# WGLab/NanoCaller

Hardware: AMD Instinct MI355X
Metric: candidate sites/sec (pileup+CNN) (higher is better)
Workload: dtype f32 (f16x3 split MFMA, f32 accumulate)

## Files before the change

### include/nanocaller_hip.h

```cpp
#ifndef NANOCALLER_HIP_H
#define NANOCALLER_HIP_H

#include <stddef.h>
#include <stdint.h>

#ifdef __cplusplus
extern "C" {
#endif

#define NC_ABI_VERSION 11

typedef struct nc_ctx nc_ctx;

enum nc_status {
    NC_OK = 0,
    NC_ERR_ARG = -1,
    NC_ERR_CAPACITY = -2,
    NC_ERR_NOMEM = -3,
    NC_ERR_HIP = -4,
    NC_ERR_STATE = -5,
    NC_ERR_SELFTEST = -6,
    NC_ERR_UNSUPPORTED = -7
};

// ... 19 lines not shown
int nc_d2h_async(nc_ctx *ctx, void *stream, void *host, const void *dev, size_t bytes);
int nc_last_kernel_ms(nc_ctx *ctx, int which, float *ms);
int nc_enable_timing(nc_ctx *ctx, int on);
int nc_timing_sums(nc_ctx *ctx, double *sum_ms, int64_t *count);

typedef struct {
    int32_t start;
    int32_t end;
    int64_t base_flag;
} nc_tile_entry;

typedef struct {
    int64_t codes_len;
    const uint8_t *codes;
    int32_t tile_size;
    int32_t tile_pos0;
    int32_t n_tiles;
    const int32_t *tile_off;
    const nc_tile_entry *tile_ent;
    int64_t n_entries;
} nc_readpack;

int nc_pack_plan(int32_t n_reads, const int32_t *start, const int32_t *end, const uint8_t *keep,
                 int32_t tile_size, int32_t pos_lo, int32_t pos_hi,
                 int64_t *codes_len, int32_t *tile_pos0, int32_t *n_tiles, int64_t *n_entries);
int nc_pack_fill(int32_t n_reads, const int32_t *start, const int32_t *end, const int64_t *off,
                 const uint8_t *codes_in, const uint8_t *strand, const uint8_t *keep,
                 int32_t tile_size, int32_t tile_pos0, int32_t n_tiles,
                 uint8_t *codes_out, int64_t codes_len, int32_t *tile_off, nc_tile_entry *tile_ent,
                 int64_t n_entries);

typedef struct nc_wire nc_wire;
typedef struct {
    int32_t n_reads;
    const int32_t *rd_start;
    const int32_t *rd_end;
    const int64_t *slot_off;
    int64_t codes_len;
    int64_t n_blocks;
    const uint32_t *blk_off;
    const int32_t *blk_read;
    const uint16_t *events;
    int64_t n_events;
    const uint32_t *blk_ev;
    const uint8_t *ev_bytes;
    int64_t n_ev_bytes;
} nc_wire_arrays;
int nc_wire_build(int32_t n_reads, const int32_t *start, const int32_t *end, const int64_t *off, const uint8_t *codes_in,
                  const uint8_t *keep, const uint8_t *ref_wire, int32_t ref_pos0, int64_t ref_len, nc_wire **out);
int nc_wire_view(const nc_wire *w, nc_wire_arrays *view);
int nc_wire_free(nc_wire *w);
int nc_wire_ref_unpack(nc_ctx *ctx, const uint8_t *d_ref_nib, int64_t ref_len, uint8_t *d_ref_wire);
int nc_wire_ins_unpack(nc_ctx *ctx, const uint8_t *d_packed, int64_t n_bases, const int32_t *d_other_idx, int32_t n_other, uint8_t *d_ins_bases);
int nc_wire_build_del(int32_t n_reads, const int32_t *start, const int32_t *end, const int64_t *off, const uint8_t *codes_in,
                      const uint8_t *keep, const uint8_t *ref_wire, int32_t ref_pos0, int64_t ref_len, const int32_t *ev_off,
                      const int32_t *ev_pos, const int32_t *ev_len, nc_wire **out);
int nc_wire_apply_deletions(nc_ctx *ctx, int32_t n_reads, const int32_t *d_rd_start, const int32_t *d_rd_end, const int64_t *d_slot_off,
                            const int32_t *d_ev_off, const int32_t *d_ev_pos, const int32_t *d_ev_len, uint8_t *d_codes);
int nc_wire_expand(nc_ctx *ctx, int32_t n_reads, const int32_t *d_rd_start, const int32_t *d_rd_end, const int64_t *d_slot_off,
                   const uint8_t *d_ref_wire, int32_t ref_pos0, int64_t ref_len, const uint32_t *d_blk_off,
                   const int32_t *d_blk_read, const uint16_t *d_events, int64_t n_blocks, uint8_t *d_codes, int64_t codes_len,
                   uint8_t *d_ref_code);
int nc_wire_build2(int32_t n_reads, const int32_t *start, const int32_t *end, const int64_t *off, const uint8_t *codes_in,
                   const uint8_t *keep, const uint8_t *ref_wire, int32_t ref_pos0, int64_t ref_len, const int32_t *ev_off,
                   const int32_t *ev_pos, const int32_t *ev_len, int32_t flags, nc_wire **out);
int nc_wire_expand2(nc_ctx *ctx, int32_t n_reads, const int32_t *d_rd_start, const int32_t *d_rd_end, const int64_t *d_slot_off,
                    const uint8_t *d_ref_wire, int32_t ref_pos0, int64_t ref_len, const uint32_t *d_blk_off,
                    const int32_t *d_blk_read, const uint8_t *d_ev_bytes, int64_t n_blocks, uint8_t *d_codes, int64_t codes_len,
                    uint8_t *d_ref_code, const uint32_t *d_blk_ev, const int32_t *d_ev_off, const int32_t *d_ev_pos,
                    const int32_t *d_ev_len);
int nc_wire_expand_del(nc_ctx *ctx, int32_t n_reads, const int32_t *d_rd_start, const int32_t *d_rd_end, const int64_t *d_slot_off,
                       const uint8_t *d_ref_wire, int32_t ref_pos0, int64_t ref_len, const uint32_t *d_blk_off,
                       const int32_t *d_blk_read, const uint16_t *d_events, int64_t n_blocks, uint8_t *d_codes, int64_t codes_len,
                       uint8_t *d_ref_code, const uint32_t *d_blk_ev, const int32_t *d_ev_off, const int32_t *d_ev_pos,
                       const int32_t *d_ev_len);

int nc_indel_events_pack(int32_t n_reads, const int32_t *rd_start, const int32_t *ev_off, const int32_t *ev_pos, const int32_t *ev_len,
                         uint16_t *d16, int8_t *l8, int32_t *read_ins_off, int64_t big_cap, int32_t *big_idx, int32_t *big_pos,
                         int32_t *big_len, int64_t *n_big);
int nc_indel_events_expand(nc_ctx *ctx, int32_t n_reads, const int32_t *d_rd_start, const int32_t *d_ev_off, const uint16_t *d_d16,
                           const int8_t *d_l8, int32_t n_big, const int32_t *d_big_idx, const int32_t *d_big_pos, const int32_t *d_big_len,
                           const int32_t *d_read_ins_off, int32_t *d_ev_pos, int32_t *d_ev_len, int32_t *d_ins_off);
int nc_indel_events_pack8(int32_t n_reads, const int32_t *rd_start, const int32_t *ev_off, const int32_t *ev_pos, const int32_t *ev_len,
                          uint8_t *b8, uint16_t *d16x, int64_t esc_cap, int32_t *read_esc_off, int32_t *read_ins_off, int64_t big_cap,
                          int32_t *big_idx, int32_t *big_pos, int32_t *big_len, int64_t *n_esc, int64_t *n_big);
int nc_indel_events_expand8(nc_ctx *ctx, int32_t n_reads, const int32_t *d_rd_start, const int32_t *d_ev_off, const uint8_t *d_b8,
                            const uint16_t *d_d16x, const int32_t *d_read_esc_off, int32_t n_big, const int32_t *d_big_idx,
                            const int32_t *d_big_pos, const int32_t *d_big_len, const int32_t *d_read_ins_off, int32_t *d_ev_pos,
                            int32_t *d_ev_len, int32_t *d_ins_off);

int nc_inflate_device(nc_ctx *ctx, int32_t n_blocks, const uint8_t *d_comp, const int64_t *d_coff, const int32_t *d_clen, uint8_t *d_out,
                      const int64_t *d_ooff, const int32_t *d_isize, int32_t *d_status, uint32_t *d_tok, int32_t *d_ntok);
int nc_inflate_device_phase(nc_ctx *ctx, int32_t phase, int32_t n_blocks, const uint8_t *d_comp, const int64_t *d_coff, const int32_t *d_clen,
                            uint8_t *d_out, const int64_t *d_ooff, const int32_t *d_isize, int32_t *d_status, uint32_t *d_tok, int32_t *d_ntok);
int nc_bgzf_crc_device(nc_ctx *ctx, int32_t n_blocks, const uint8_t *d_comp, const int64_t *d_coff, const int32_t *d_clen, const uint8_t *d_out,
                       const int64_t *d_ooff, const int32_t *d_isize, int32_t *d_status);

int nc_bam_retag_sizes(nc_ctx *ctx, const uint8_t *d_raw, int32_t n_rec, const int64_t *d_rec_off, const uint64_t *d_hash, const int32_t *d_ps,
                       int32_t n_tags, int32_t *d_new_size, int32_t *d_tag_idx, int64_t *d_out_off, int32_t *d_status);
int nc_bam_retag(nc_ctx *ctx, const uint8_t *d_raw, int32_t n_rec, const int64_t *d_rec_off, const uint8_t *d_hp, const int32_t *d_ps,
                 const int32_t *d_tag_idx, const int64_t *d_out_off, uint8_t *d_out);
int nc_bgzf_deflate_device(nc_ctx *ctx, int32_t n, const uint8_t *d_in, const int64_t *d_ioff, const int32_t *d_ilen, uint8_t *d_out,
                           const int64_t *d_ooff, int32_t *d_clen, uint32_t *d_crc, int32_t *d_status);
int nc_bgzf_crc32_device(nc_ctx *ctx, int32_t n, const uint8_t *d_in, const int64_t *d_ioff, const int32_t *d_ilen, uint32_t *d_crc);
int nc_bgzf_assemble_device(nc_ctx *ctx, int32_t n, const uint8_t *d_pay, const int64_t *d_poff, const int32_t *d_clen, const uint32_t *d_crc,
                            const int32_t *d_isize, int64_t *d_foff, uint8_t *d_file);

#define NC_BAM_META_COLS 12
int nc_bgzf_members(const uint8_t *data, int64_t n, int64_t cap, int64_t *coff, int32_t *clen, int32_t *isize, int64_t *n_members);
int nc_bgzf_scan(const uint8_t *data, int64_t n, int64_t start, int64_t cap, int64_t *coff, int32_t *clen, int32_t *isize, int64_t *n_members,
                 int64_t *next);
int nc_bam_walk(nc_ctx *ctx, const uint8_t *d_raw, int64_t raw_len, int32_t n_seeds, const int64_t *d_seed, const int32_t *d_seed_tid,
                const int64_t *d_first, int64_t *d_out, int32_t *d_status);
int nc_bam_meta(nc_ctx *ctx, const uint8_t *d_raw, int64_t n_rec, const int64_t *d_rec_off, int32_t *d_meta, int32_t *d_status);
int nc_bam_codes(nc_ctx *ctx, const uint8_t *d_raw, int32_t n_reads, const int64_t *d_rec, const int64_t *d_slot, const int32_t *d_cigd,
                 const int32_t *d_ncig, const int32_t *d_start, uint8_t *d_codes);
int nc_bam_name_groups(nc_ctx *ctx, const uint8_t *d_raw, int64_t raw_len, int64_t n_cand, const int64_t *d_rec_off, const uint64_t *d_hash,
                       int32_t *d_gid, int32_t *d_status);
int nc_bam_indel_reads(nc_ctx *ctx, const uint8_t *d_raw, int32_t n_reads, const int64_t *d_rec, const int32_t *d_cigd, const int32_t *d_ncig,
                       int32_t tail_cap, int32_t *d_counts, const int32_t *d_ev_off, const int32_t *d_ins_base, const int32_t *d_tail_off,
                       int32_t *d_ev_pos, int32_t *d_ev_len, int32_t *d_ins_off, uint8_t *d_ins_bases, uint8_t *d_tail_bases);

typedef struct {
    int32_t mincov;
    double min_allele_freq;
    double nbr_t0, nbr_t1;
    int32_t haploid;
} nc_scan_params;

int nc_snp_scan(nc_ctx *ctx, const nc_readpack *pack,
                const uint8_t *ref_code_dev, int32_t ref_pos0, int32_t ref_len,
                int32_t scan_lo, int32_t scan_hi, const nc_scan_params *params,
                int32_t n_chunks, const int32_t *chunk_start_host, const int32_t *chunk_end_host,
                int32_t *n_nbr, int32_t *n_cand, int32_t *n_sites);

int nc_snp_scan_begin(nc_ctx *ctx, const nc_readpack *pack,
                      const uint8_t *ref_code_dev, int32_t ref_pos0, int32_t ref_len,
                      int32_t scan_lo, int32_t scan_hi, const nc_scan_params *params,
                      int32_t n_chunks, const int32_t *chunk_start_host, const int32_t *chunk_end_host);
int nc_snp_scan_end(nc_ctx *ctx, int32_t *n_nbr, int32_t *n_cand, int32_t *n_sites);

int nc_snp_scan_fetch(nc_ctx *ctx, int32_t *nbr_pos, int32_t *site_pos, int32_t *site_chunk,
                      int32_t *site_n, int32_t *site_alt);

int nc_snp_scan_fetch_async(nc_ctx *ctx, void *copy_stream, int32_t *nbr_pos, int32_t *site_pos, int32_t *site_chunk,
                            int32_t *site_n, int32_t *site_alt);

int nc_snp_featurize(nc_ctx *ctx, const nc_readpack *pack,
                     const uint8_t *ref_code_dev, int32_t ref_pos0, int32_t ref_len,
                     int32_t seq_mode, int32_t maxcov, int32_t min_nbr_sites,
                     float *x_dev, int32_t *ref_code_out_dev, int32_t *fwd_dp_dev, int32_t *rev_dp_dev,
                     int32_t *site_depth_dev, uint8_t *valid_dev);

int nc_snp_set_mates(nc_ctx *ctx, int32_t n_mates, const int64_t *d_mate_key, const int32_t *d_mate_rec);

int nc_indel_set_mates(nc_ctx *ctx, int32_t n_mates, const int64_t *d_mate_key, const int32_t *d_mate_rec);

int nc_snp_scan_set_sites(nc_ctx *ctx, int32_t n_sites, const int32_t *d_pos, int32_t only);

int nc_snp_scan_set_nbr_sites(nc_ctx *ctx, int32_t n_sites, const int32_t *d_pos, int32_t only);

int nc_snp_scan_set_sampling(nc_ctx *ctx, uint32_t seed, const uint32_t *keep6_host);

typedef struct {
    int32_t c_m, c_x, c_h;
    int32_t haploid;
    int32_t n_bands;
    int32_t band[16];
} nc_refconf_params;

int nc_refconf_columns(nc_ctx *ctx, const nc_readpack *pack, const uint8_t *d_ref_code, int32_t tile_pos0, int64_t npos, uint32_t *d_words);

int nc_refconf_blocks(nc_ctx *ctx, const uint32_t *d_words, int32_t tile_pos0, int64_t npos, int32_t n_chunks, const int32_t *chunk_start_host,
                      const int32_t *chunk_end_host, int32_t n_cut, const int32_t *d_cut_start, const int32_t *d_cut_end,
                      const nc_refconf_params *params, int64_t *n_blocks);
int nc_refconf_fetch(nc_ctx *ctx, int32_t *d_or_host_out);

int nc_refconf_text(nc_ctx *ctx, int64_t n_blocks, const int32_t *d_blocks, const uint8_t *d_ref_code, int32_t tile_pos0, int64_t npos,
                    const char *chrom, const nc_refconf_params *params, int64_t *d_line_off, uint8_t *d_text, int64_t text_cap, int64_t *n_bytes);

int nc_snp_scale(nc_ctx *ctx, const int32_t *site_depth_dev, const uint8_t *valid_dev, double train_coverage,
                 int32_t mode, double *scale_dev, double *chunk_depth_host);
int nc_snp_chunk_depth_async(nc_ctx *ctx, void *copy_stream, double *chunk_depth_host_pinned);

int nc_load_weights(nc_ctx *ctx, int32_t model_kind, const float *blob_host, size_t n_floats);
int nc_set_cnn_precision(nc_ctx *ctx, int exact_fp32);
int nc_set_tensor_format(nc_ctx *ctx, int fmt);
int nc_snp_forward(nc_ctx *ctx, int32_t model_kind, int64_t n, const float *x_dev, const int32_t *ref_code_dev,
                   const double *scale_dev, int32_t scale_mode, float *probs_dev, float *gt_dev);

int nc_snp_forward_drain(nc_ctx *ctx, int32_t model_kind, int64_t n, const float *x_dev, const int32_t *ref_code_dev,
                         const double *scale_dev, int32_t scale_mode, float *probs_dev, float *gt_dev,
                         void *copy_stream, float *probs_host, float *gt_host);
int nc_cnn_x_limit(nc_ctx *ctx, int32_t model_kind, float *x_limit);
int nc_cnn_range_watch(nc_ctx *ctx, uint8_t *site_flags_dev);
int nc_snp_trunk_info(nc_ctx *ctx, int32_t *mfma_per_site, int32_t *kernel_id);
int nc_indel_forward(nc_ctx *ctx, int32_t model_kind, int64_t n, const float *x_dev, float *probs_dev);

int nc_indel_tensor(nc_ctx *ctx, int32_t n_sets, const uint8_t *rows_dev, const int64_t *row_off_dev,
                    const int32_t *n_rows_dev, const int32_t *n_cols_dev, const uint8_t *ref_rows_dev,
                    const int64_t *ref_off_dev, int32_t max_cols, float *x_dev, uint8_t *cns_dev);

typedef struct {
    int32_t n_reads;
    const int32_t *ev_off;
    const int32_t *ev_pos;
    const int32_t *ev_len;
    const uint8_t *read_hap;
} nc_indel_events;

typedef struct {
    int32_t mincov, win_size, small_win_size;
    double ins_t, del_t;
    int32_t haploid;
    int32_t impute;
} nc_indel_scan_params;

int nc_indel_scan(nc_ctx *ctx, const nc_readpack *pack, const nc_indel_events *events, const uint8_t *excl_dev,
                  int32_t start, int32_t end, const nc_indel_scan_params *params, int8_t *col_type_host);

int nc_indel_scan_batch(nc_ctx *ctx, const nc_readpack *pack, const nc_indel_events *events, const uint8_t *excl_dev,
                        int32_t n_chunks, const int32_t *starts, const int32_t *ends, const nc_indel_scan_params *params,
                        int8_t *col_type_host, const int64_t *col_off);

typedef struct nc_bam nc_bam;
typedef struct nc_decoded nc_decoded;
typedef struct {
    int32_t n_reads;
    const int32_t *start, *end, *flag;
    const int64_t *off;
    const uint8_t *codes;
    int64_t n_codes;
    const int32_t *ev_off;
    const int32_t *ev_pos, *ev_len;
    int64_t n_events;
    const uint8_t *hap;
    const int32_t *ps;
    const int64_t *seq_off;
    const uint8_t *seq;
    int64_t n_seq;
    const int32_t *name_off;
    const char *names;
    const int32_t *qstart;
} nc_decoded_arrays;

int nc_bam_open(const char *path, nc_bam **out);
int nc_bam_close(nc_bam *bam);
int nc_bam_n_refs(nc_bam *bam, int32_t *n_refs, int32_t *has_index);
int nc_bam_ref(nc_bam *bam, int32_t i, const char **name, int32_t *length);
const char *nc_bam_error(const nc_bam *bam);
int nc_bam_set_threads(nc_bam *bam, int32_t n);
int nc_bam_decode(nc_bam *bam, int32_t tid, int32_t beg1, int32_t end1, int32_t keep_seq, nc_decoded **out);
int nc_bam_decode_regions(const char *path, int32_t tid, int32_t beg1, int32_t end1, int32_t keep_seq, int32_t n_regions,
                          nc_decoded **out);
int nc_decoded_view(const nc_decoded *d, nc_decoded_arrays *view);
int nc_decoded_free(nc_decoded *d);
#define NC_FLAG_REFSKIP 0x10000
int nc_decoded_check(const nc_decoded *d, const uint8_t *keep, int64_t *n_refskip, int64_t *n_dup_overlap);
int nc_decoded_name_groups(const nc_decoded *d, const uint8_t *keep, int32_t *gid, int64_t *n_shared);

typedef struct nc_slices nc_slices;
typedef struct {
    int32_t n_anchor;
    const int32_t *anchor_off;
    const int32_t *read_idx;
    const int64_t *seq_off;
    const uint8_t *seq;
    int64_t n_slices;
} nc_slices_arrays;
int nc_indel_slices(const nc_decoded *d, int32_t n_anchor, const int32_t *anchor_pos, int32_t window_before, int32_t window_after,
                    const uint8_t *keep, nc_slices **out);
int nc_slices_view(const nc_slices *s, nc_slices_arrays *view);
int nc_slices_free(nc_slices *s);

typedef struct nc_pass2 nc_pass2;
typedef struct {
    int32_t n_kept;
    const int32_t *anchor_idx;
    const int32_t *first0;
    int32_t sets_per_anchor;
    int32_t n_sets;
    const int32_t *set_read0;
    int32_t n_alignments;
    const int32_t *read_off;
    const char *reads;
    const int32_t *ref_off;
    const char *refs;
    int32_t max_cols;
    const int32_t *al_dup;
} nc_pass2_arrays;
int nc_indel_pass2_sets(const nc_decoded *d, const uint8_t *keep, int32_t n_anchor, const int32_t *anchors, const char *contig,
                        int64_t chrom_len, int32_t ref_lo, int32_t ref_hi, int32_t window_after, int32_t mincov, int32_t maxcov,
                        int32_t haploid, const int32_t *imp_idx, const int32_t *imp_off, const int32_t *imp_reads, nc_pass2 **out);
int nc_pass2_view(const nc_pass2 *p, nc_pass2_arrays *view);
int nc_pass2_free(nc_pass2 *p);


typedef struct nc_indel_pack_h nc_indel_pack_h;
typedef struct {
    int32_t n_reads;
    const int32_t *ev_off;
    const int32_t *ev_pos, *ev_len;
    int64_t n_events;
    const int32_t *ins_off;
    const uint8_t *ins_bases;
    int64_t n_ins_bases;
// ... 199 lines not shown
```

### nanocaller_amd/_lib.py

```python
from __future__ import annotations

import ctypes as C
import os

import numpy as np

_HERE = os.path.dirname(os.path.abspath(__file__))
LIB_PATH = os.environ.get("NANOCALLER_HIP_LIB") or os.path.join(_HERE, "libnanocaller_hip.so")

NC_OK = 0
NC_ERR_ARG = -1
NC_ERR_CAPACITY = -2
NC_ERR_NOMEM = -3
NC_ERR_UNSUPPORTED = -7
FLAG_REFSKIP = 0x10000
ABI_VERSION = 11
MODEL_SNP, MODEL_SNP_HAP, MODEL_INDEL, MODEL_INDEL_HAP = 0, 1, 2, 3
SEQ_MODES = {"ont": 0, "short_ont": 1, "ul_ont": 2, "ul_ont_extreme": 3, "pacbio": 4}
CODE_ABSENT = 7
FLANK = 50000
SNP_TENSOR = 1025
STAR_SCORING = (25, 1, 20, -10)

EXPORTS = [
    "nc_abi_version", "nc_device_count", "nc_ctx_create", "nc_ctx_destroy", "nc_ctx_set_stream", "nc_ctx_sync",
    "nc_last_error", "nc_malloc", "nc_free", "nc_memcpy_h2d", "nc_memcpy_d2h", "nc_last_kernel_ms",
    "nc_enable_timing", "nc_pack_plan", "nc_pack_fill", "nc_snp_scan", "nc_snp_scan_begin", "nc_snp_scan_end", "nc_snp_scan_fetch", "nc_snp_featurize",
    "nc_snp_scale", "nc_load_weights", "nc_snp_forward", "nc_indel_forward", "nc_indel_tensor", "nc_indel_scan",
    "nc_bam_open", "nc_bam_close", "nc_bam_n_refs", "nc_bam_ref", "nc_bam_error", "nc_bam_decode", "nc_decoded_view",
    "nc_decoded_free", "nc_snp_vcf_format", "nc_set_cnn_precision", "nc_snp_scan_fetch_async", "nc_snp_forward_drain", "nc_argsort4", "nc_indel_slices", "nc_slices_view", "nc_slices_free",
    "nc_nw_cigar", "nc_allele_prediction", "nc_bgzf_compress", "nc_bam_set_threads", "nc_indel_scan_batch", "nc_timing_sums", "nc_snp_chunk_depth_async", "nc_bam_decode_regions", "nc_star_msa", "nc_star_msa_tensor", "nc_star_msa_tensor_dup", "nc_set_tensor_format", "nc_allele_prediction_batch", "nc_allele_prediction_device", "nc_bgzf_read_file", "nc_consensus_strings",
    "nc_wire_build", "nc_wire_build_del", "nc_wire_apply_deletions", "nc_wire_ref_unpack", "nc_wire_view", "nc_wire_free", "nc_wire_expand", "nc_wire_expand_del", "nc_snp_set_mates", "nc_indel_set_mates", "nc_snp_scan_set_sites", "nc_snp_scan_set_nbr_sites", "nc_snp_scan_set_sampling", "nc_decoded_name_groups", "nc_wire_ins_unpack", "nc_indel_events_pack8", "nc_indel_events_expand8", "nc_wire_build2", "nc_wire_expand2", "nc_d2h_async",
    "nc_indel_pass2_sets", "nc_pass2_view", "nc_pass2_free",
    "nc_decoded_check", "nc_indel_pack_build", "nc_indel_pack_view", "nc_indel_pack_free", "nc_indel_sites_plan", "nc_indel_sites_run",
    "nc_indel_sites_fetch", "nc_indel_sites_fetch_alt", "nc_indel_set_sites", "nc_indel_sites_fetch_src", "nc_indel_sites_stage_ms", "nc_indel_sites_band_stats", "nc_indel_sites_band", "nc_indel_events_pack", "nc_indel_events_expand", "nc_inflate_device", "nc_inflate_device_phase", "nc_bgzf_crc_device", "nc_bgzf_members", "nc_bgzf_scan", "nc_bam_walk", "nc_bam_meta", "nc_bam_codes", "nc_bam_indel_reads", "nc_bam_name_groups", "nc_indel_sites_scoring", "nc_indel_vcf_format", "nc_synth_indel_truth", "nc_synth_indel_reads", "nc_cnn_x_limit", "nc_cnn_range_watch", "nc_snp_trunk_info",
    "nc_snp_phase_gather", "nc_snp_phase_load", "nc_snp_phase_solve", "nc_haplotag_run", "nc_snp_phase_view", "nc_snp_phase_free",
    "nc_snp_phase_realign", "nc_snp_phase_solve_gt", "nc_snp_phase_genotypes",
    "nc_snp_phase_set_weights", "nc_snp_phase_weights_from_bam", "nc_snp_phase_weights",
    "nc_bam_retag_sizes", "nc_bam_retag", "nc_bgzf_deflate_device", "nc_bgzf_crc32_device", "nc_bgzf_assemble_device",
    "nc_fasta_decode",
    "nc_bamidx_candidates", "nc_bamidx_chain", "nc_bamidx_collect", "nc_bamidx_verify", "nc_bamidx_serial", "nc_bamidx_fields",
    "nc_train_create", "nc_train_free", "nc_train_set_weights", "nc_train_get_weights", "nc_train_forward", "nc_train_loss_grad", "nc_train_adam",
    "nc_train_info", "nc_train_stage_ms",
    "nc_indel_train_create", "nc_indel_train_free", "nc_indel_train_set_weights", "nc_indel_train_get_weights", "nc_indel_train_forward",
    "nc_indel_train_loss_grad", "nc_indel_train_adam", "nc_indel_train_info", "nc_indel_train_stage_ms",
    "nc_hap_train_create", "nc_hap_train_free", "nc_hap_train_set_weights", "nc_hap_train_get_weights", "nc_hap_train_forward",
    "nc_hap_train_loss_grad", "nc_hap_train_adam", "nc_hap_train_info", "nc_hap_train_stage_ms",
    "nc_hap_indel_train_create", "nc_hap_indel_train_free", "nc_hap_indel_train_set_weights", "nc_hap_indel_train_get_weights",
    "nc_hap_indel_train_forward", "nc_hap_indel_train_loss_grad", "nc_hap_indel_train_adam", "nc_hap_indel_train_info", "nc_hap_indel_train_stage_ms",
    "nc_refconf_columns", "nc_refconf_blocks", "nc_refconf_fetch", "nc_refconf_text",
]


class TileEntry(C.Structure):
    _fields_ = [("start", C.c_int32), ("end", C.c_int32), ("base_flag", C.c_int64)]


TILE_ENTRY_DTYPE = np.dtype([("start", "<i4"), ("end", "<i4"), ("base_flag", "<i8")])
assert TILE_ENTRY_DTYPE.itemsize == C.sizeof(TileEntry) == 16


class ReadPackC(C.Structure):
    _fields_ = [("codes_len", C.c_int64), ("codes", C.c_void_p), ("tile_size", C.c_int32), ("tile_pos0", C.c_int32),
                ("n_tiles", C.c_int32), ("tile_off", C.c_void_p), ("tile_ent", C.c_void_p), ("n_entries", C.c_int64)]


class ScanParamsC(C.Structure):
    _fields_ = [("mincov", C.c_int32), ("min_allele_freq", C.c_double), ("nbr_t0", C.c_double), ("nbr_t1", C.c_double),
                ("haploid", C.c_int32)]


class RefconfParamsC(C.Structure):
    _fields_ = [("c_m", C.c_int32), ("c_x", C.c_int32), ("c_h", C.c_int32), ("haploid", C.c_int32), ("n_bands", C.c_int32), ("band", C.c_int32 * 16)]


class IndelEventsC(C.Structure):
    _fields_ = [("n_reads", C.c_int32), ("ev_off", C.c_void_p), ("ev_pos", C.c_void_p), ("ev_len", C.c_void_p),
                ("read_hap", C.c_void_p)]


class IndelScanParamsC(C.Structure):
    _fields_ = [("mincov", C.c_int32), ("win_size", C.c_int32), ("small_win_size", C.c_int32), ("ins_t", C.c_double),
                ("del_t", C.c_double), ("haploid", C.c_int32), ("impute", C.c_int32)]


class DecodedArraysC(C.Structure):
    _fields_ = [("n_reads", C.c_int32), ("start", C.c_void_p), ("end", C.c_void_p), ("flag", C.c_void_p), ("off", C.c_void_p),
                ("codes", C.c_void_p), ("n_codes", C.c_int64), ("ev_off", C.c_void_p), ("ev_pos", C.c_void_p),
                ("ev_len", C.c_void_p), ("n_events", C.c_int64), ("hap", C.c_void_p), ("ps", C.c_void_p),
                ("seq_off", C.c_void_p), ("seq", C.c_void_p), ("n_seq", C.c_int64), ("name_off", C.c_void_p),
                ("names", C.c_void_p), ("qstart", C.c_void_p)]


class SlicesArraysC(C.Structure):
    _fields_ = [("n_anchor", C.c_int32), ("anchor_off", C.c_void_p), ("read_idx", C.c_void_p), ("seq_off", C.c_void_p),
                ("seq", C.c_void_p), ("n_slices", C.c_int64)]


class Pass2ArraysC(C.Structure):
    _fields_ = [("n_kept", C.c_int32), ("anchor_idx", C.c_void_p), ("first0", C.c_void_p), ("sets_per_anchor", C.c_int32),
                ("n_sets", C.c_int32), ("set_read0", C.c_void_p), ("n_alignments", C.c_int32), ("read_off", C.c_void_p),
                ("reads", C.c_void_p), ("ref_off", C.c_void_p), ("refs", C.c_void_p), ("max_cols", C.c_int32), ("al_dup", C.c_void_p)]


class IndelPackArraysC(C.Structure):
    _fields_ = [("n_reads", C.c_int32), ("ev_off", C.c_void_p), ("ev_pos", C.c_void_p), ("ev_len", C.c_void_p), ("n_events", C.c_int64),
                ("ins_off", C.c_void_p), ("ins_bases", C.c_void_p), ("n_ins_bases", C.c_int64), ("tail_off", C.c_void_p),
                ("tail_bases", C.c_void_p), ("n_tail_bases", C.c_int64), ("read_ps", C.c_void_p), ("read_hap", C.c_void_p),
                ("read_flag", C.c_void_p)]


class IndelReadsC(C.Structure):
    _fields_ = [("n_reads", C.c_int32), ("slot_off", C.c_void_p), ("rd_start", C.c_void_p), ("rd_end", C.c_void_p), ("ev_off", C.c_void_p),
                ("ev_pos", C.c_void_p), ("ev_len", C.c_void_p), ("ins_off", C.c_void_p), ("ins_bases", C.c_void_p), ("tail_off", C.c_void_p),
                ("tail_bases", C.c_void_p), ("read_ps", C.c_void_p), ("read_hap", C.c_void_p), ("read_flag", C.c_void_p)]


class WireArraysC(C.Structure):
    _fields_ = [("n_reads", C.c_int32), ("rd_start", C.c_void_p), ("rd_end", C.c_void_p), ("slot_off", C.c_void_p),
                ("codes_len", C.c_int64), ("n_blocks", C.c_int64), ("blk_off", C.c_void_p), ("blk_read", C.c_void_p), ("events", C.c_void_p),
                ("n_events", C.c_int64), ("blk_ev", C.c_void_p), ("ev_bytes", C.c_void_p), ("n_ev_bytes", C.c_int64)]


class PhaseArraysC(C.Structure):
    _fields_ = [("n_reads", C.c_int32), ("n_sites", C.c_int32), ("n_blocks", C.c_int32), ("n_groups", C.c_int32), ("n_entries", C.c_int64),
                ("entry_off", C.c_void_p), ("entry_site", C.c_void_p), ("entry_allele", C.c_void_p), ("read_side", C.c_void_p),
                ("site_block", C.c_void_p), ("site_h", C.c_void_p), ("site_phased", C.c_void_p), ("site_ps", C.c_void_p),
                ("block_first", C.c_void_p), ("block_last", C.c_void_p), ("block_ps", C.c_void_p), ("block_cost", C.c_void_p),
                ("group_hp", C.c_void_p), ("group_ps", C.c_void_p), ("ms", C.c_float * 4)]


_lib = None


class NanoCallerHipError(RuntimeError):

    def __init__(self, message, status=None):
        super().__init__(message)
        self.status = status


def lib():
    global _lib
    if _lib is None:
        if not os.path.exists(LIB_PATH):
            raise NanoCallerHipError(
                "%s not found: build it with `python -c 'import __graft_entry__ as g; g.build()'` "
                "(hipcc --offload-arch=gfx950). There is no CPU fallback." % LIB_PATH)
        try:
            import torch
        except ImportError:
            pass
        L = C.CDLL(LIB_PATH)
        vp, i32, i64, dbl = C.c_void_p, C.c_int32, C.c_int64, C.c_double
        L.nc_abi_version.restype = C.c_int
        if L.nc_abi_version() != ABI_VERSION:
            raise NanoCallerHipError("%s has ABI version %d, this binding needs %d: rebuild it" % (LIB_PATH, L.nc_abi_version(), ABI_VERSION))
        L.nc_device_count.argtypes = [C.POINTER(C.c_int)]
        L.nc_ctx_create.argtypes = [C.c_int, C.POINTER(vp)]
        L.nc_ctx_destroy.argtypes = [vp]
        L.nc_ctx_set_stream.argtypes = [vp, vp]
        L.nc_ctx_sync.argtypes = [vp]
        L.nc_last_error.argtypes = [vp]
        L.nc_last_error.restype = C.c_char_p
        L.nc_malloc.argtypes = [vp, C.c_size_t, C.POINTER(vp)]
        L.nc_free.argtypes = [vp, vp]
        L.nc_memcpy_h2d.argtypes = [vp, vp, vp, C.c_size_t]
        L.nc_memcpy_d2h.argtypes = [vp, vp, vp, C.c_size_t]
        L.nc_last_kernel_ms.argtypes = [vp, C.c_int, C.POINTER(C.c_float)]
        L.nc_timing_sums.argtypes = [vp, vp, vp]
        L.nc_enable_timing.argtypes = [vp, C.c_int]
        L.nc_set_cnn_precision.argtypes = [vp, C.c_int]
        L.nc_pack_plan.argtypes = [i32, vp, vp, vp, i32, i32, i32, C.POINTER(i64), C.POINTER(i32), C.POINTER(i32),
                                   C.POINTER(i64)]
        L.nc_pack_fill.argtypes = [i32, vp, vp, vp, vp, vp, vp, i32, i32, i32, vp, i64, vp, vp, i64]
        L.nc_snp_scan.argtypes = [vp, C.POINTER(ReadPackC), vp, i32, i32, i32, i32, C.POINTER(ScanParamsC), i32, vp, vp,
                                  C.POINTER(i32), C.POINTER(i32), C.POINTER(i32)]
        L.nc_snp_scan_begin.argtypes = [vp, C.POINTER(ReadPackC), vp, i32, i32, i32, i32, C.POINTER(ScanParamsC), i32, vp, vp]
        L.nc_snp_scan_end.argtypes = [vp, C.POINTER(i32), C.POINTER(i32), C.POINTER(i32)]
        L.nc_snp_scan_fetch.argtypes = [vp, vp, vp, vp, vp, vp]
        L.nc_snp_scan_fetch_async.argtypes = [vp, vp, vp, vp, vp, vp, vp]
        L.nc_snp_featurize.argtypes = [vp, C.POINTER(ReadPackC), vp, i32, i32, i32, i32, i32, vp, vp, vp, vp, vp, vp]
        L.nc_snp_scale.argtypes = [vp, vp, vp, dbl, i32, vp, vp]
        L.nc_snp_chunk_depth_async.argtypes = [vp, vp, vp]
        L.nc_load_weights.argtypes = [vp, i32, vp, C.c_size_t]
        L.nc_snp_forward.argtypes = [vp, i32, i64, vp, vp, vp, i32, vp, vp]
        L.nc_snp_forward_drain.argtypes = [vp, i32, i64, vp, vp, vp, i32, vp, vp, vp, vp, vp]
        L.nc_indel_forward.argtypes = [vp, i32, i64, vp, vp]
        L.nc_indel_tensor.argtypes = [vp, i32, vp, vp, vp, vp, vp, vp, i32, vp, vp]
        L.nc_indel_scan.argtypes = [vp, C.POINTER(ReadPackC), C.POINTER(IndelEventsC), vp, i32, i32, C.POINTER(IndelScanParamsC), vp]
        L.nc_indel_scan_batch.argtypes = [vp, C.POINTER(ReadPackC), C.POINTER(IndelEventsC), vp, i32, vp, vp, C.POINTER(IndelScanParamsC), vp, vp]
        L.nc_bam_open.argtypes = [C.c_char_p, C.POINTER(vp)]
        L.nc_bam_close.argtypes = [vp]
        L.nc_bam_set_threads.argtypes = [vp, i32]
        L.nc_bam_n_refs.argtypes = [vp, C.POINTER(i32), C.POINTER(i32)]
        L.nc_bam_ref.argtypes = [vp, i32, C.POINTER(C.c_char_p), C.POINTER(i32)]
        L.nc_bam_error.argtypes = [vp]
        L.nc_bam_error.restype = C.c_char_p
        L.nc_bam_decode.argtypes = [vp, i32, i32, i32, i32, C.POINTER(vp)]
        L.nc_star_msa_tensor.argtypes = [vp, i32, vp, vp, vp, vp, vp, i32, i32, i32, i32, i32, vp, vp, vp, vp, vp, vp, vp]
        L.nc_star_msa_tensor_dup.argtypes = L.nc_star_msa_tensor.argtypes + [vp]
        L.nc_consensus_strings.argtypes = [vp, i32, i32, vp, vp, vp]
        L.nc_allele_prediction_batch.argtypes = [i32, C.c_char_p, vp, C.c_char_p, vp, vp, vp, vp]
        L.nc_allele_prediction_device.argtypes = [vp, i32, C.c_char_p, vp, C.c_char_p, vp, vp, vp, vp]
        L.nc_set_tensor_format.argtypes = [vp, C.c_int]
        L.nc_star_msa.argtypes = [i32, C.c_char_p, vp, C.c_char_p, i32, i32, i32, i32, i32, i32, vp, vp, C.POINTER(i32)]
        L.nc_bam_decode_regions.argtypes = [C.c_char_p, i32, i32, i32, i32, i32, C.POINTER(vp)]
        L.nc_decoded_view.argtypes = [vp, C.POINTER(DecodedArraysC)]
        L.nc_decoded_free.argtypes = [vp]
        L.nc_indel_slices.argtypes = [vp, i32, vp, i32, i32, vp, C.POINTER(vp)]
        L.nc_slices_view.argtypes = [vp, C.POINTER(SlicesArraysC)]
        L.nc_slices_free.argtypes = [vp]
        L.nc_nw_cigar.argtypes = [C.c_char_p, i32, C.c_char_p, i32, i32, i32, i32, i32, vp, vp, i32, C.POINTER(i32)]
        L.nc_allele_prediction.argtypes = [C.c_char_p, i32, C.c_char_p, i32, i32, C.POINTER(i32), C.POINTER(i32)]
        L.nc_bgzf_compress.argtypes = [vp, i64, i32, vp, i64, C.POINTER(i64), vp, i64, C.POINTER(i64)]
        L.nc_indel_pass2_sets.argtypes = [vp, vp, i32, vp, C.c_char_p, i64, i32, i32, i32, i32, i32, i32, vp, vp, vp, C.POINTER(vp)]
        L.nc_pass2_view.argtypes = [vp, C.POINTER(Pass2ArraysC)]
        L.nc_pass2_free.argtypes = [vp]
        L.nc_d2h_async.argtypes = [vp, vp, vp, vp, C.c_size_t]
        L.nc_wire_build.argtypes = [i32, vp, vp, vp, vp, vp, vp, i32, i64, C.POINTER(vp)]
        L.nc_wire_build_del.argtypes = [i32, vp, vp, vp, vp, vp, vp, i32, i64, vp, vp, vp, C.POINTER(vp)]
        L.nc_wire_build2.argtypes = [i32, vp, vp, vp, vp, vp, vp, i32, i64, vp, vp, vp, i32, C.POINTER(vp)]
        L.nc_wire_apply_deletions.argtypes = [vp, i32, vp, vp, vp, vp, vp, vp, vp]
        L.nc_wire_ref_unpack.argtypes = [vp, vp, i64, vp]
        L.nc_wire_view.argtypes = [vp, C.POINTER(WireArraysC)]
        L.nc_wire_free.argtypes = [vp]
        L.nc_wire_expand.argtypes = [vp, i32, vp, vp, vp, vp, i32, i64, vp, vp, vp, i64, vp, i64, vp]
        L.nc_wire_expand_del.argtypes = L.nc_wire_expand.argtypes + [vp, vp, vp, vp]
        L.nc_wire_expand2.argtypes = L.nc_wire_expand.argtypes + [vp, vp, vp, vp]
        L.nc_snp_set_mates.argtypes = [vp, i32, vp, vp]
        L.nc_indel_set_mates.argtypes = [vp, i32, vp, vp]
        L.nc_snp_scan_set_sites.argtypes = [vp, i32, vp, i32]
        L.nc_snp_scan_set_nbr_sites.argtypes = [vp, i32, vp, i32]
        L.nc_snp_scan_set_sampling.argtypes = [vp, C.c_uint32, vp]
        L.nc_decoded_name_groups.argtypes = [vp, vp, vp, C.POINTER(i64)]
        L.nc_wire_ins_unpack.argtypes = [vp, vp, i64, vp, i32, vp]
        L.nc_indel_events_pack8.argtypes = [i32, vp, vp, vp, vp, vp, vp, i64, vp, vp, i64, vp, vp, vp, C.POINTER(i64), C.POINTER(i64)]
        L.nc_indel_events_expand8.argtypes = [vp, i32, vp, vp, vp, vp, vp, i32, vp, vp, vp, vp, vp, vp, vp]
        L.nc_decoded_check.argtypes = [vp, vp, C.POINTER(i64), C.POINTER(i64)]
        L.nc_indel_pack_build.argtypes = [vp, vp, i32, C.POINTER(vp)]
        L.nc_indel_pack_view.argtypes = [vp, C.POINTER(IndelPackArraysC)]
        L.nc_indel_pack_free.argtypes = [vp]
        L.nc_indel_sites_plan.argtypes = [vp, C.POINTER(ReadPackC), vp, i32, i32, i64, C.POINTER(IndelReadsC), vp, i32, vp, vp,
                                          C.POINTER(IndelScanParamsC), i32, i32, C.POINTER(i32), C.POINTER(i64)]
        L.nc_indel_sites_run.argtypes = [vp, vp]
        L.nc_indel_sites_scoring.argtypes = [vp, i32, i32, i32, i32]
        L.nc_indel_sites_fetch.argtypes = [vp, vp, vp, vp, vp, vp, vp, C.POINTER(i64)]
        L.nc_indel_sites_fetch_alt.argtypes = [vp, vp, i64]
        L.nc_indel_set_sites.argtypes = [vp, i32, vp, vp, i32]
        L.nc_indel_sites_fetch_src.argtypes = [vp, vp]
        L.nc_indel_sites_stage_ms.argtypes = [vp, vp, vp]
        L.nc_indel_sites_band_stats.argtypes = [vp, vp]
        L.nc_indel_sites_band.argtypes = [vp, i32, i32]
        L.nc_indel_events_pack.argtypes = [i32, vp, vp, vp, vp, vp, vp, vp, i64, vp, vp, vp, C.POINTER(i64)]
        L.nc_indel_events_expand.argtypes = [vp, i32, vp, vp, vp, vp, i32, vp, vp, vp, vp, vp, vp, vp]
        L.nc_inflate_device.argtypes = [vp, i32, vp, vp, vp, vp, vp, vp, vp, vp, vp]
        L.nc_inflate_device_phase.argtypes = [vp, i32, i32, vp, vp, vp, vp, vp, vp, vp, vp, vp]
        L.nc_bgzf_crc_device.argtypes = [vp, i32, vp, vp, vp, vp, vp, vp, vp]
        L.nc_bgzf_members.argtypes = [vp, i64, i64, vp, vp, vp, C.POINTER(i64)]
        L.nc_bgzf_scan.argtypes = [vp, i64, i64, i64, vp, vp, vp, C.POINTER(i64), C.POINTER(i64)]
        L.nc_bam_walk.argtypes = [vp, vp, i64, i32, vp, vp, vp, vp, vp]
        L.nc_bam_meta.argtypes = [vp, vp, i64, vp, vp, vp]
        L.nc_bam_codes.argtypes = [vp, vp, i32, vp, vp, vp, vp, vp, vp]
        L.nc_bam_indel_reads.argtypes = [vp, vp, i32, vp, vp, vp, i32, vp, vp, vp, vp, vp, vp, vp, vp, vp]
        L.nc_bam_name_groups.argtypes = [vp, vp, i64, i64, vp, vp, vp, vp]
        L.nc_indel_vcf_format.argtypes = [C.c_char_p, i64, vp, vp, i32, vp, i32, vp, vp, vp, vp, C.c_char_p, i64, i32, vp, i64, C.POINTER(i64), vp]
        L.nc_synth_indel_truth.argtypes = [vp, i64, C.c_uint64, dbl, dbl, dbl, dbl, i32, vp, vp, vp]
        L.nc_synth_indel_reads.argtypes = [vp, i64, C.c_uint64, dbl, dbl, dbl, dbl, i32, vp, vp, vp, vp, vp, vp, i32, vp, vp, vp, vp, vp, vp, vp, vp, vp]
        L.nc_cnn_x_limit.argtypes = [vp, i32, C.POINTER(C.c_float)]
        L.nc_snp_trunk_info.argtypes = [vp, C.POINTER(C.c_int32), C.POINTER(C.c_int32)]
        L.nc_cnn_range_watch.argtypes = [vp, vp]
        L.nc_argsort4.argtypes = [vp, i64, vp, C.POINTER(i64), vp, i64]
        L.nc_snp_phase_gather.argtypes = [vp, vp, i64, i32, vp, vp, vp, i32, vp, vp, C.POINTER(vp)]
        L.nc_snp_phase_load.argtypes = [vp, i32, i32, vp, vp, vp, vp, C.POINTER(vp)]
        L.nc_snp_phase_solve.argtypes = [vp, vp, i32]
        L.nc_snp_phase_solve_gt.argtypes = [vp, vp, i32, vp, i32]
        L.nc_snp_phase_genotypes.argtypes = [vp, C.POINTER(vp)]
        L.nc_snp_phase_set_weights.argtypes = [vp, vp, vp, vp]
        L.nc_snp_phase_weights_from_bam.argtypes = [vp, vp, vp, i64, vp, i32, i32, i32]
        L.nc_snp_phase_weights.argtypes = [vp, C.POINTER(vp), C.POINTER(vp), C.POINTER(vp)]
        L.nc_snp_phase_realign.argtypes = [vp, vp, i64, C.POINTER(IndelReadsC), i64, i64, vp, i32, i32, vp, vp, C.POINTER(vp)]
        L.nc_haplotag_run.argtypes = [vp, vp, i32, vp]
        L.nc_snp_phase_view.argtypes = [vp, C.POINTER(PhaseArraysC)]
        L.nc_snp_phase_free.argtypes = [vp]
        L.nc_bam_retag_sizes.argtypes = [vp, vp, i32, vp, vp, vp, i32, vp, vp, vp, vp]
        L.nc_bam_retag.argtypes = [vp, vp, i32, vp, vp, vp, vp, vp, vp]
        L.nc_bgzf_deflate_device.argtypes = [vp, i32, vp, vp, vp, vp, vp, vp, vp, vp]
        L.nc_bgzf_crc32_device.argtypes = [vp, i32, vp, vp, vp, vp]
        L.nc_bgzf_assemble_device.argtypes = [vp, i32, vp, vp, vp, vp, vp, vp, vp]
        L.nc_fasta_decode.argtypes = [vp, vp, i64, i64, i64, i64, i64, vp, vp, i64, i64, i64, i64, vp, vp]
        L.nc_bamidx_candidates.argtypes = [vp, vp, i64, i64, i32, vp, vp, vp]
        L.nc_bamidx_chain.argtypes = [vp, vp, i64, i64, vp, vp, i32, vp, vp, vp]
        L.nc_bamidx_collect.argtypes = [vp, i32, vp, vp, vp, vp]
        L.nc_bamidx_verify.argtypes = [vp, vp, i64, i64, i64, vp, i32, vp]
        L.nc_bamidx_serial.argtypes = [vp, vp, i64, i64, i32, vp, vp]
        L.nc_bamidx_fields.argtypes = [vp, vp, i64, vp, i64, vp, i32, i32, vp, vp, i32, i32, i32, i32, i32, vp, vp, vp]
        f32 = C.c_float
        for fam, snp in (("nc_train", True), ("nc_hap_train", True), ("nc_indel_train", False), ("nc_hap_indel_train", False)):
            site = [vp, i64, vp] + ([vp, vp] if snp else []) + [vp, f32]
            sig = dict(create=[vp, i32, i64] + ([] if snp else [i64]) + [C.POINTER(vp)], free=[vp], set_weights=[vp, vp, C.c_size_t],
                       get_weights=[vp, vp, C.c_size_t], forward=site + [vp] + ([vp] if fam == "nc_train" else []), loss_grad=site + [vp, f32, vp, vp],
                       adam=[vp, f32, f32, f32, f32], info=[vp, C.POINTER(i64), C.POINTER(i64), C.POINTER(i64)], stage_ms=[vp, i32, vp])
            for fn, argtypes in sig.items():
                getattr(L, "%s_%s" % (fam, fn)).argtypes = argtypes
        L.nc_refconf_columns.argtypes = [vp, C.POINTER(ReadPackC), vp, i32, i64, vp]
        L.nc_refconf_blocks.argtypes = [vp, vp, i32, i64, i32, vp, vp, i32, vp, vp, C.POINTER(RefconfParamsC), C.POINTER(i64)]
        L.nc_refconf_fetch.argtypes = [vp, vp]
        L.nc_refconf_text.argtypes = [vp, i64, vp, vp, i32, i64, C.c_char_p, C.POINTER(RefconfParamsC), vp, vp, i64, C.POINTER(i64)]
        L.nc_snp_vcf_format.argtypes = [C.c_char_p, i64, vp, vp, vp, vp, vp, vp, vp, vp, i32, vp, i64, C.POINTER(i64)]
        for name in EXPORTS:
            fn = getattr(L, name)
            if name not in ("nc_last_error", "nc_bam_error"):
                fn.restype = C.c_int
        _lib = L
    return _lib


def npp(a):
    if a is None:
        return None
    assert a.flags["C_CONTIGUOUS"]
    return a.ctypes.data_as(C.c_void_p)
```

### nanocaller_amd/csrc/nc_common.h

```cpp
#pragma once
#include <hip/hip_runtime.h>

#include <cstdarg>
#include <cstdint>
#include <cstdio>
#include <cstring>
#include <vector>

#include "../../include/nanocaller_hip.h"

__device__ __forceinline__ int32_t nc_wave_incl_scan(int32_t v)
{
    v += __builtin_amdgcn_update_dpp(0, v, 0x111, 0xf, 0xf, true);
    v += __builtin_amdgcn_update_dpp(0, v, 0x112, 0xf, 0xf, true);
    v += __builtin_amdgcn_update_dpp(0, v, 0x114, 0xf, 0xf, true);
    v += __builtin_amdgcn_update_dpp(0, v, 0x118, 0xf, 0xf, true);
    v += __builtin_amdgcn_update_dpp(0, v, 0x142, 0xa, 0xf, true);
    v += __builtin_amdgcn_update_dpp(0, v, 0x143, 0xc, 0xf, true);
    return v;
}

struct DevBuf {
    void *p = nullptr;
    size_t cap = 0;
    DevBuf() = default;
    DevBuf(const DevBuf &) = delete;
    DevBuf &operator=(const DevBuf &) = delete;
    ~DevBuf() { release(); }
    void release()
    {
        if (p) (void)hipFree(p);
        p = nullptr;
        cap = 0;
    }
};

struct nc_weights {
    float *dev = nullptr;
    size_t n = 0;
    float *packed = nullptr;
    void *packed_h = nullptr;
    float x_limit = 0.0f;
};

struct nc_ctx {
    int device = 0;
    hipStream_t own_stream = nullptr;
    hipStream_t stream = nullptr;
    char err[512] = {0};
    int timing = 0;
    bool x_i16 = false;
    bool cnn_exact_fp32 = false;
    bool k10_lds_set[2] = {false, false};
    bool huff_lds_set = false;
    bool deflate_lds_set = false;
    DevBuf deflate_tok;
    int32_t n_mates = 0;
    const int64_t *mate_key = nullptr;
    const int32_t *mate_rec = nullptr;
    int32_t n_imates = 0;
    const int64_t *imate_key = nullptr;
    const int32_t *imate_rec = nullptr;
    int32_t n_gsites = 0;
    const int32_t *gsite_pos = nullptr;
    bool gsites_only = false;
    DevBuf site_bits;
    int32_t n_nsites = 0;
    const int32_t *nsite_pos = nullptr;
    bool nsites_only = false;
    DevBuf nbr_bits;
    bool sample_on = false;
    uint32_t sample_seed = 0;
    uint32_t sample_keep[6] = {0, 0, 0, 0, 0, 0};
    int32_t n_isites = 0;
    const int32_t *isite_pos = nullptr;
    const uint8_t *isite_long = nullptr;
    bool isites_only = false;
    hipEvent_t ev0 = nullptr, ev1 = nullptr;
    float last_ms[6] = {0, 0, 0, 0, 0, 0};
    hipEvent_t kev[128] = {nullptr};
    int n_kev = 0;
    hipEvent_t tev[4][2] = {{nullptr, nullptr}, {nullptr, nullptr}, {nullptr, nullptr}, {nullptr, nullptr}};
    bool tev_pending[4] = {false, false, false, false};
    bool kev_pending = false;
    double sum_ms[6] = {0, 0, 0, 0, 0, 0};
    int64_t sum_n[6] = {0, 0, 0, 0, 0, 0};
    hipEvent_t drain_ev[4] = {nullptr};
    hipEvent_t scale_ev = nullptr;
    hipEvent_t scan_ev = nullptr;

    DevBuf stage_nbr, stage_cpos, stage_cn, stage_calt;
    DevBuf tile_cnt, tile_pre;
    DevBuf nbr_pos, cand_pos, cand_n, cand_alt;
    DevBuf chunk_start, chunk_end, chunk_lo, chunk_cnt, chunk_off;
    DevBuf site_pos, site_chunk, site_n, site_alt;
    DevBuf totals;
    DevBuf cnn_a, cnn_b, cnn_c;
    DevBuf chunk_depth;
    DevBuf nbr_idx;
    struct {
        size_t budget = 0;
        bool budget_shrunk = false;
        DevBuf ws;
        DevBuf ent_read;
        const void *ent_of = nullptr;
        int ent_spt = 0;
    } k7;
    DevBuf msa_reads, msa_read_off, msa_read_set, msa_refs, msa_ref_off;
    DevBuf msa_dup;
    DevBuf msa_rows_hf, msa_hcol, msa_tb, msa_trace, msa_cols, msa_out;
    int32_t n_nbr = 0, n_cand = 0, n_sites = 0, n_chunks = 0;
    bool have_scan = false;

    nc_weights w[4];
    struct nc_pipe_state *pipe = nullptr;
    struct nc_refconf_state *refconf = nullptr;
    uint8_t *range_sites = nullptr;

    int32_t *mbox = nullptr;
    bool scan_begun = false;
    int scan_tile = 0, scan_n_tiles = 0, scan_n_chunks = 0, scan_cap_nbr = 0, scan_cap_cand = 0;
    hipEvent_t scan_tot_ev = nullptr;
    uint8_t *stage_h = nullptr;
    int stage_turn = 0;
};

int nc_d2h(nc_ctx *ctx, void *host, const void *dev, size_t bytes, hipStream_t st);
int nc_h2d_small(nc_ctx *ctx, void *dev, const void *host, size_t bytes, hipStream_t st);
#define NC_D2H_KERNEL_MAX 65536
#define NC_STAGE_SLOT 16384
#define NC_STAGE_SLOTS 16

inline int nc_h2d_pieces(nc_ctx *ctx, void *dev, const void *host, size_t bytes, hipStream_t st)
{
    int in_flight = 0;
    for (size_t o = 0; o < bytes; o += NC_STAGE_SLOT) {
        if (++in_flight >= NC_STAGE_SLOTS - 2) {
            if (hipStreamSynchronize(st) != hipSuccess) return NC_ERR_HIP;
            in_flight = 1;
        }
        const size_t n = bytes - o < (size_t)NC_STAGE_SLOT ? bytes - o : (size_t)NC_STAGE_SLOT;
        const int rc = nc_h2d_small(ctx, (char *)dev + o, (const char *)host + o, n, st);
        if (rc != NC_OK) return rc;
    }
    return NC_OK;
}
inline int nc_d2h_pieces(nc_ctx *ctx, void *host_pinned, const void *dev, size_t bytes, hipStream_t st)
{
    for (size_t o = 0; o < bytes; o += NC_D2H_KERNEL_MAX) {
        const size_t n = bytes - o < (size_t)NC_D2H_KERNEL_MAX ? bytes - o : (size_t)NC_D2H_KERNEL_MAX;
        const int rc = nc_d2h(ctx, (char *)host_pinned + o, (const char *)dev + o, n, st);
        if (rc != NC_OK) return rc;
    }
    return NC_OK;
}

inline int nc_fail(nc_ctx *ctx, int code, const char *fmt, ...)
{
    if (ctx) {
        va_list ap;
        va_start(ap, fmt);
        vsnprintf(ctx->err, sizeof ctx->err, fmt, ap);
        va_end(ap);
    }
    return code;
}

#define NC_HIP(ctx, call)                                                                           \
    do {                                                                                            \
        hipError_t e_ = (call);                                                                     \
        if (e_ != hipSuccess)                                                                       \
            return nc_fail(ctx, NC_ERR_HIP, "%s failed: %s (%s:%d)", #call, hipGetErrorString(e_),  \
                           __FILE__, __LINE__);                                                     \
    } while (0)

inline int nc_ensure(nc_ctx *ctx, DevBuf &b, size_t bytes)
{
    if (bytes <= b.cap) return NC_OK;
    if (b.p) {
        NC_HIP(ctx, hipStreamSynchronize(ctx->stream));
        NC_HIP(ctx, hipFree(b.p));
        b.p = nullptr;
        b.cap = 0;
    }
    size_t want = bytes + bytes / 4 + 256;
    hipError_t e = hipMalloc(&b.p, want);
    if (e != hipSuccess) return nc_fail(ctx, NC_ERR_NOMEM, "hipMalloc(%zu) failed: %s", want, hipGetErrorString(e));
    b.cap = want;
    return NC_OK;
}

#define NC_TRY(x)                \
    do {                         \
        int rc_ = (x);           \
        if (rc_ != NC_OK) return rc_; \
    } while (0)

extern "C" __attribute__((visibility("hidden"))) void nc_timing_resolve(nc_ctx *ctx, int which);

struct NcTimer {
    nc_ctx *ctx;
    int which;
    NcTimer(nc_ctx *c, int w) : ctx(c), which(w)
    {
        if (ctx->timing == 1) {
            nc_timing_resolve(ctx, which);
            for (int e = 0; e < 2; e++)
                if (!ctx->tev[which][e]) (void)hipEventCreate(&ctx->tev[which][e]);
            (void)hipEventRecord(ctx->tev[which][0], ctx->stream);
        }
    }
    void stop()
    {
        if (ctx->timing == 1) {
            (void)hipEventRecord(ctx->tev[which][1], ctx->stream);
            ctx->tev_pending[which] = true;
        }
    }
};

int nc_selftest_device(nc_ctx *ctx);
void nc_pipe_destroy(nc_ctx *ctx);
void nc_refconf_destroy(nc_ctx *ctx);
```

### nanocaller_amd/csrc/nc_featurize.hip

```cpp
#include <type_traits>

#include "nc_common.h"

namespace {

constexpr int MAXCOV_CAP = 1024;
constexpr int MAXCOV_SMALL = 256;
constexpr int NBR = 20;

struct Bucket { int32_t dlo, dhi, k, far; };
struct ModeTab { int32_t nb, W; Bucket b[7]; };

constexpr ModeTab MODE_TABLES[5] = {
    {5, 50000, {{0, 2000, 2, 1}, {2000, 5000, 3, 0}, {5000, 10000, 4, 0}, {10000, 20000, 5, 0}, {20000, 1 << 30, 6, 0}, {0, 0, 0, 0}, {0, 0, 0, 0}}},
    {3, 50000, {{0, 2000, 5, 0}, {2000, 5000, 10, 0}, {5000, 1 << 30, 5, 0}, {0, 0, 0, 0}, {0, 0, 0, 0}, {0, 0, 0, 0}, {0, 0, 0, 0}}},
    {7, 100000, {{0, 2000, 2, 1}, {2000, 5000, 2, 0}, {5000, 10000, 3, 0}, {10000, 20000, 3, 0}, {20000, 40000, 4, 0}, {40000, 50000, 3, 0}, {50000, 1 << 30, 3, 0}}},
    {7, 300000, {{0, 10000, 2, 1}, {10000, 20000, 2, 0}, {20000, 50000, 3, 0}, {50000, 75000, 3, 0}, {75000, 100000, 4, 0}, {100000, 200000, 4, 0}, {200000, 1 << 30, 2, 0}}},
    {4, 20000, {{0, 2000, 4, 1}, {2000, 5000, 5, 0}, {5000, 10000, 5, 0}, {10000, 20000, 6, 0}, {0, 0, 0, 0}, {0, 0, 0, 0}, {0, 0, 0, 0}}},
};
__constant__ ModeTab MODES[5] = {MODE_TABLES[0], MODE_TABLES[1], MODE_TABLES[2], MODE_TABLES[3], MODE_TABLES[4]};

constexpr bool buckets_contiguous()
{
    for (int m = 0; m < 5; m++)
        for (int i = 0; i < MODE_TABLES[m].nb; i++)
            if (MODE_TABLES[m].b[i].dlo != (i ? MODE_TABLES[m].b[i - 1].dhi : 0) || MODE_TABLES[m].b[i].dhi <= MODE_TABLES[m].b[i].dlo) return false;
    return true;
}
static_assert(buckets_contiguous(), "a bucket must begin where the one before it ends (the first at 0): k_featurize_pairs shares the buckets' edges");

constexpr int NBR_IDX_SHIFT = 10;

__device__ __forceinline__ int lower_bound_i32(const int32_t *a, int n, int64_t key, const int32_t *cidx, int32_t cidx_pos0, int n_cidx)
{
    int lo = 0, hi = n;
    const int64_t rel = key - cidx_pos0;
    if (rel <= 0) hi = cidx[0];
    else {
        const int64_t b = rel >> NBR_IDX_SHIFT;
        if (b >= n_cidx - 1) lo = cidx[n_cidx - 1];
        else { lo = cidx[b]; hi = cidx[b + 1]; }
    }
    while (lo < hi) {
        const int mid = (lo + hi) >> 1;
        if ((int64_t)a[mid] < key) lo = mid + 1; else hi = mid;
    }
    return lo;
}

struct FeatArgs {
    const uint8_t *codes;
    const int32_t *tile_off;
    const nc_tile_entry *tile_ent;
    int32_t tile_pos0, tile_shift;
    const uint8_t *ref_code;
    int32_t ref_pos0;
    const int32_t *nbr_pos;
    int32_t n_nbr;
    const int32_t *cidx;
    int32_t cidx_pos0, n_cidx;
    const int32_t *site_pos, *site_chunk;
    const int32_t *chunk_start, *chunk_end;
    int32_t n_sites, mode, maxcov, min_nbr_sites;
    float *x;
    int32_t *ref_out, *fwd, *rev, *depth;
    uint8_t *valid;
    int32_t x_i16;
    const int64_t *mate_key;
    const int4 *mate_rec;
    int32_t n_mates;
};

__device__ __forceinline__ int named_member(const FeatArgs &a, int64_t key, int32_t p, int *self)
{
    int lo = 0, hi = a.n_mates;
    while (lo < hi) { const int mid = (lo + hi) >> 1; if (a.mate_key[mid] < key) lo = mid + 1; else hi = mid; }
    if (self) *self = lo;
    if (lo >= a.n_mates || a.mate_key[lo] != key) { if (self) *self = -2; return -1; }
    int best = -1, i = lo;
    for (int guard = 0; guard < 64; guard++) {
        const int4 r = a.mate_rec[i];
        if (r.x <= p && p < r.y && i > best) best = i;
        i = r.z;
        if (i == lo || i < 0 || i >= a.n_mates) break;
    }
    return best;
}
__device__ __forceinline__ int named_code(const FeatArgs &a, int64_t key, int32_t p)
{
    const int m = named_member(a, key, p, nullptr);
    if (m < 0) return 4;
    return a.codes[a.mate_key[m] - (a.mate_rec[m].x & ~15) + p];
}

template <int CAP, bool I16>
__global__ __launch_bounds__(256) void k_featurize(FeatArgs a)
{
    __shared__ __attribute__((aligned(16))) float sm[I16 ? 1 : 4][I16 ? 4 : NC_SNP_TENSOR + 3];
    __shared__ int32_t nlist[4][64];
    const int lane = threadIdx.x & 63, wv = __builtin_amdgcn_readfirstlane(threadIdx.x >> 6);
    const int nblk = (int)gridDim.x, q8 = nblk >> 3, r8 = nblk & 7, xcd = blockIdx.x & 7, within = blockIdx.x >> 3;
    const int blk = (xcd < r8 ? xcd * (q8 + 1) : r8 * (q8 + 1) + (xcd - r8) * q8) + within;
    const int s = blk * 4 + wv;
    float *X = sm[I16 ? 0 : wv];
    if constexpr (!I16)
        for (int i = lane; i < NC_SNP_TENSOR; i += 64) X[i] = 0.0f;

    if (s < a.n_sites) {
        const int32_t v = __builtin_amdgcn_readfirstlane(a.site_pos[s]);
        const int32_t ch = __builtin_amdgcn_readfirstlane(a.site_chunk[s]);
        const int64_t win_lo = max((int64_t)1, (int64_t)a.chunk_start[ch] - NC_FLANK);
        const int64_t win_hi = (int64_t)a.chunk_end[ch] + NC_FLANK;
        const ModeTab &M = MODES[a.mode];
        const int nb = M.nb;

        int take = 0, idx0 = 0;
        if (lane < 2 * nb) {
            const bool left = lane < nb;
            const Bucket B = M.b[left ? nb - 1 - lane : lane - nb];
            const int64_t dhi = min((int64_t)B.dhi, (int64_t)M.W - 1);
            int64_t pmin = left ? (int64_t)v - dhi : (int64_t)v + B.dlo + 1;
            int64_t pmax = left ? (int64_t)v - B.dlo - 1 : (int64_t)v + dhi;
            pmin = max(pmin, win_lo);
            pmax = min(pmax, win_hi);
            if (pmin <= pmax) {
                const int lo = lower_bound_i32(a.nbr_pos, a.n_nbr, pmin, a.cidx, a.cidx_pos0, a.n_cidx);
                const int hi = lower_bound_i32(a.nbr_pos, a.n_nbr, pmax + 1, a.cidx, a.cidx_pos0, a.n_cidx);
                const int m = hi - lo;
                take = min(m, B.k);
                const bool first = left ? (B.far != 0) : (B.far == 0);
                idx0 = first ? lo : hi - take;
            }
        }
        int incl = take;
#pragma unroll
        for (int o = 1; o < 16; o <<= 1) {
            const int y = __shfl_up(incl, o, 64);
            if (lane >= o) incl += y;
        }
        const int excl = incl - take;
        const int nl = __builtin_amdgcn_readlane(incl, nb - 1);
        const int ntot = __builtin_amdgcn_readlane(incl, 2 * nb - 1);
        const int nr = ntot - nl;
        const int ncols = ntot + 1;

        int32_t col = v;
        {
            for (int i = 0; i < take; i++) nlist[wv][excl + i] = idx0 + i;
            __builtin_amdgcn_fence(__ATOMIC_ACQ_REL, "wavefront");
            __builtin_amdgcn_wave_barrier();
            const int jj = lane < nl ? lane : lane - 1;
            if (lane != nl && lane < ncols) col = a.nbr_pos[nlist[wv][jj]];
        }
        const bool active = lane < ncols;
        const int rc_col = active ? a.ref_code[(int64_t)col - a.ref_pos0] : 4;
        const int rc_centre = a.ref_code[(int64_t)v - a.ref_pos0];

        const int t = (v - a.tile_pos0) >> a.tile_shift;
        const int e0 = __builtin_amdgcn_readfirstlane(a.tile_off[t]), e1 = __builtin_amdgcn_readfirstlane(a.tile_off[t + 1]);
        const bool ok = ncols >= a.min_nbr_sites;
        constexpr bool BYTE_CNT = CAP == MAXCOV_SMALL;
        using cnt_t = typename std::conditional<BYTE_CNT, uint32_t, unsigned long long>::type;
        constexpr int FIELD = BYTE_CNT ? 8 : 16;
        cnt_t cnt[4] = {0, 0, 0, 0};
        int n_all = 0;
        int fw[4] = {0, 0, 0, 0}, rv[4] = {0, 0, 0, 0};
        for (int eb = e0; eb < e1; eb += 64) {
            const int e = eb + lane;
            bool cov = false;
            int code = 4, strand = 0;
            int32_t estart = 0;
            uint32_t elen = 0, erow_lo = 0, erow_hi = 0;
            if (e < e1) {
                const nc_tile_entry ent = a.tile_ent[e];
                cov = ent.start <= v && v < ent.end;
                const uint64_t row = (uint64_t)(uintptr_t)a.codes + (uint64_t)((ent.base_flag & ~int64_t(15)) + ent.start);
                estart = ent.start;
                elen = (uint32_t)(ent.end - ent.start);
                erow_lo = (uint32_t)row;
                erow_hi = (uint32_t)(row >> 32);
                if (cov) {
                    code = a.codes[(ent.base_flag & ~int64_t(15)) + v];
                    strand = (int)(ent.base_flag & 1);
                }
            }
            unsigned long long m = __ballot(cov);
            unsigned long long mb[4];
#pragma unroll
            for (int b = 0; b < 4; b++) {
                mb[b] = __ballot(cov && code == b);
                const unsigned long long f = __ballot(cov && code == b && strand == 0);
                fw[b] += __popcll(f);
                rv[b] += __popcll(mb[b] & ~f);
            }
            const int room = a.maxcov - n_all;
            n_all += __popcll(m);
            if (!ok || room <= 0) continue;
            while (__popcll(m) > room) m &= ~(1ull << (63 - __builtin_clzll(m)));
#pragma unroll
            for (int k = 0; k < 4; k++) {
                unsigned long long mk = mb[k] & m;
                while (mk != 0ull) {
                    constexpr int RND = 16;
                    typedef const uint8_t __attribute__((address_space(1))) *gbyte_ptr;
                    int bcode[RND];
                    int nu = 0;
#pragma unroll
                    for (int u = 0; u < RND; u++) {
                        bcode[u] = 4;
                        if (mk != 0ull) {
                            const int idx = __builtin_ctzll(mk);
                            mk &= mk - 1ull;
                            nu = u + 1;
                            const int32_t rstart = __builtin_amdgcn_readlane(estart, idx);
                            const uint32_t rlen = (uint32_t)__builtin_amdgcn_readlane((int)elen, idx);
                            const gbyte_ptr rrow = (gbyte_ptr)(uintptr_t)(((uint64_t)(uint32_t)__builtin_amdgcn_readlane((int)erow_hi, idx) << 32) |
                                                                         (uint32_t)__builtin_amdgcn_readlane((int)erow_lo, idx));
                            const uint32_t off = (uint32_t)(col - rstart);
                            if (active && off < rlen) bcode[u] = rrow[off];
                        }
                    }
#pragma unroll
                    for (int u = 0; u < RND; u++) {
                        const cnt_t inc = BYTE_CNT ? (cnt_t)(uint32_t)(1ull << (8 * bcode[u]))
                                                   : (bcode[u] < 4 ? ((cnt_t)1 << (16 * bcode[u])) : (cnt_t)0);
                        if (u < nu) cnt[k] += inc;
                    }
                }
            }
        }
        const int ns = min(n_all, a.maxcov);
        if constexpr (I16) {
            const int o = NBR - nl;
            const int src = lane - o;
            const bool have = ok && lane < 41 && src >= 0 && src < ncols;
            const int sl = have ? src : lane;
            const int rc_s = __shfl(rc_col, sl, 64);
            cnt_t cs[4];
#pragma unroll
            for (int i = 0; i < 4; i++) {
                if constexpr (BYTE_CNT) cs[i] = (cnt_t)__shfl((int)cnt[i], sl, 64);
                else cs[i] = ((cnt_t)(uint32_t)__shfl((int)(cnt[i] >> 32), sl, 64) << 32) | (uint32_t)__shfl((int)(uint32_t)cnt[i], sl, 64);
            }
            if (lane < 41) {
                int16_t *dst = reinterpret_cast<int16_t *>(a.x) + (int64_t)s * NC_SNP_TENSOR + lane * 5;
                typedef uint32_t __attribute__((aligned(2))) u32_a2;
                auto put_row = [&](int row, int v0, int v1, int v2, int v3, int v4) {
                    int16_t *d = dst + row * (41 * 5);
                    *reinterpret_cast<u32_a2 *>(d) = (uint32_t)(v0 & 0xffff) | ((uint32_t)v1 << 16);
                    *reinterpret_cast<u32_a2 *>(d + 2) = (uint32_t)(v2 & 0xffff) | ((uint32_t)v3 << 16);
                    d[4] = (int16_t)v4;
                };
                const int rcs = have ? rc_s : 4;
                put_row(0, rcs == 0, rcs == 1, rcs == 2, rcs == 3, 0);
#pragma unroll
                for (int i = 0; i < 4; i++) {
                    int v[4];
#pragma unroll
                    for (int b = 0; b < 4; b++) {
                        const int val = have ? (int)((cs[i] >> (FIELD * b)) & ((1 << FIELD) - 1)) : 0;
                        v[b] = b == rcs ? -val : val;
                    }
                    put_row(1 + i, v[0], v[1], v[2], v[3], (have && i == rc_centre) ? 1 : 0);
                }
            }
        } else if (ok) {
            if (active) {
                const int o = NBR - nl;
                float *Xc = X + (o + lane) * 5;
                if (rc_col < 4) Xc[rc_col] = 1.0f;
#pragma unroll
                for (int i = 0; i < 4; i++) {
#pragma unroll
                    for (int b = 0; b < 4; b++) {
                        const int val = (int)((cnt[i] >> (FIELD * b)) & ((1 << FIELD) - 1));
                        Xc[(1 + i) * 41 * 5 + b] = (float)(b == rc_col ? -val : val);
                    }
                    Xc[(1 + i) * 41 * 5 + 4] = (i == rc_centre) ? 1.0f : 0.0f;
                }
            }
        }
        if (lane == 0) {
            a.ref_out[s] = rc_centre;
            a.depth[s] = ns;
            a.valid[s] = ok ? 1 : 0;
        }
        if (lane < 4) {
            a.fwd[s * 4 + lane] = fw[lane];
            a.rev[s * 4 + lane] = rv[lane];
        }
        (void)nr;
    }
    if constexpr (I16) return;
    __syncthreads();
    const int s0 = blk * 4;
    const int nsite = min(4, a.n_sites - s0);
    if (a.x_i16) {
        int16_t *d16 = reinterpret_cast<int16_t *>(a.x) + (int64_t)s0 * NC_SNP_TENSOR;
        const int total = nsite * NC_SNP_TENSOR;
        for (int i = threadIdx.x * 8; i < total; i += 256 * 8) {
            if (i + 8 <= total) {
                union { int16_t h[8]; uint4 u; } o;
#pragma unroll
                for (int q = 0; q < 8; q++) o.h[q] = (int16_t)sm[(i + q) / NC_SNP_TENSOR][(i + q) % NC_SNP_TENSOR];
                *reinterpret_cast<uint4 *>(d16 + i) = o.u;
            } else {
                for (int q = i; q < total; q++) d16[q] = (int16_t)sm[q / NC_SNP_TENSOR][q % NC_SNP_TENSOR];
            }
        }
        return;
    }
    float *dst = a.x + (int64_t)s0 * NC_SNP_TENSOR;
    if (nsite == 4) {
        float4 *d4 = reinterpret_cast<float4 *>(dst);
        for (int i = threadIdx.x; i < NC_SNP_TENSOR; i += 256) {
            const int f = i * 4;
            float4 o;
            o.x = sm[(f + 0) / NC_SNP_TENSOR][(f + 0) % NC_SNP_TENSOR];
            o.y = sm[(f + 1) / NC_SNP_TENSOR][(f + 1) % NC_SNP_TENSOR];
            o.z = sm[(f + 2) / NC_SNP_TENSOR][(f + 2) % NC_SNP_TENSOR];
            o.w = sm[(f + 3) / NC_SNP_TENSOR][(f + 3) % NC_SNP_TENSOR];
            d4[i] = o;
        }
    } else {
        for (int i = threadIdx.x; i < nsite * NC_SNP_TENSOR; i += 256) dst[i] = sm[i / NC_SNP_TENSOR][i % NC_SNP_TENSOR];
    }
}

template <bool MATES>
__global__ __launch_bounds__(256) void k_featurize_pairs(FeatArgs a)
{
    __shared__ int32_t nlist[4][64];
    union alignas(16) RecBuf { uint4 r[MAXCOV_SMALL]; int16_t h[MAXCOV_SMALL * 8]; uint32_t w[MAXCOV_SMALL * 4]; };
    static_assert((NC_SNP_TENSOR + 1) * 2 <= (int)sizeof(uint4) * MAXCOV_SMALL, "the tensor (one int16 further in for odd sites) must fit the read list");
    __shared__ RecBuf rec[4];
    __shared__ int32_t colL[4][64];
    __shared__ uint32_t cntL[4][41 * 4 + 4];
    __shared__ uint32_t endL[4][2 * 41];
    const int lane = threadIdx.x & 63, wv = __builtin_amdgcn_readfirstlane(threadIdx.x >> 6);
    const int nblk = (int)gridDim.x, q8 = nblk >> 3, r8 = nblk & 7, xcd = blockIdx.x & 7, within = blockIdx.x >> 3;
    const int blk = (xcd < r8 ? xcd * (q8 + 1) : r8 * (q8 + 1) + (xcd - r8) * q8) + within;
    const int s = blk * 4 + wv;
    if (s >= a.n_sites) return;
    const int32_t v = __builtin_amdgcn_readfirstlane(a.site_pos[s]);
    const int32_t ch = __builtin_amdgcn_readfirstlane(a.site_chunk[s]);
    const int64_t win_lo = max((int64_t)1, (int64_t)a.chunk_start[ch] - NC_FLANK);
    const int64_t win_hi = (int64_t)a.chunk_end[ch] + NC_FLANK;
    const ModeTab &M = MODES[a.mode];
    const int nb = M.nb;
    const int t = (v - a.tile_pos0) >> a.tile_shift;
    const int e0 = __builtin_amdgcn_readfirstlane(a.tile_off[t]), e1 = __builtin_amdgcn_readfirstlane(a.tile_off[t + 1]);
    nc_tile_entry pf_ent;
    pf_ent.start = 0; pf_ent.end = 0; pf_ent.base_flag = 0;
    int pf_code = 4;
    if (e0 + lane < e1) {
        pf_ent = a.tile_ent[e0 + lane];
        if (pf_ent.start <= v && v < pf_ent.end) pf_code = a.codes[(pf_ent.base_flag & ~int64_t(15)) + v];
    }
    const int rc_centre = a.ref_code[(int64_t)v - a.ref_pos0];
    int edge = 0;
    if (lane < 2 * nb + 2) {
        const bool left = lane <= nb;
        const int bi = left ? nb - 1 - lane : lane - nb - 2;
        const int64_t D = bi < 0 ? (int64_t)0 : min((int64_t)M.b[max(bi, 0)].dhi, (int64_t)M.W - 1);
        const int64_t key = min(max(left ? (int64_t)v - D : (int64_t)v + 1 + D, win_lo), win_hi + 1);
        edge = lower_bound_i32(a.nbr_pos, a.n_nbr, key, a.cidx, a.cidx_pos0, a.n_cidx);
    }
    int take = 0, idx0 = 0;
    {
        const bool left = lane < nb;
        const int lo = __shfl(edge, left ? lane : lane + 1, 64), hi = __shfl(edge, left ? lane + 1 : lane + 2, 64);
        if (lane < 2 * nb) {
            const Bucket B = M.b[left ? nb - 1 - lane : lane - nb];
            take = min(max(hi - lo, 0), B.k);
            const bool first = left ? (B.far != 0) : (B.far == 0);
            idx0 = first ? lo : hi - take;
        }
    }
    int incl = take;
#pragma unroll
    for (int o = 1; o < 16; o <<= 1) {
        const int y = __shfl_up(incl, o, 64);
        if (lane >= o) incl += y;
    }
    const int excl = incl - take;
    const int nl = __builtin_amdgcn_readlane(incl, nb - 1);
    const int ntot = __builtin_amdgcn_readlane(incl, 2 * nb - 1);
    const int ncols = ntot + 1;
    int32_t col = v;
    for (int i = 0; i < take; i++) nlist[wv][excl + i] = idx0 + i;
    for (int i = lane; i < 41 * 4; i += 64) cntL[wv][i] = 0;
    __builtin_amdgcn_fence(__ATOMIC_ACQ_REL, "wavefront");
    __builtin_amdgcn_wave_barrier();
    {
        const int jj = lane < nl ? lane : lane - 1;
        if (lane != nl && lane < ncols) col = a.nbr_pos[nlist[wv][jj]];
    }
    const bool active = lane < ncols;
    colL[wv][lane] = active ? col : INT32_MAX;
    const int rc_col = active ? a.ref_code[(int64_t)col - a.ref_pos0] : 4;
    const bool ok = ncols >= a.min_nbr_sites;
    int n_all = 0, nsel = 0;
    int fw[4] = {0, 0, 0, 0}, rv[4] = {0, 0, 0, 0};
    for (int eb = e0; eb < e1; eb += 64) {
        const int e = eb + lane;
        bool cov = false;
        int code = 4, strand = 0;
        uint4 rr = make_uint4(0, 0, 0, 0);
        if (e < e1) {
            nc_tile_entry ent = pf_ent;
            if (eb != e0) ent = a.tile_ent[e];
            cov = ent.start <= v && v < ent.end;
            const uint64_t row = (uint64_t)(uintptr_t)a.codes + (uint64_t)((ent.base_flag & ~int64_t(15)) + ent.start);
            rr = make_uint4((uint32_t)row, (uint32_t)(row >> 32), (uint32_t)ent.start, (uint32_t)(ent.end - ent.start));
            if constexpr (MATES) {
                if (cov && (ent.base_flag & 8)) {
                    int self;
                    const int m = named_member(a, (ent.base_flag & ~int64_t(15)) + (ent.start & ~15), v, &self);
                    if (self >= 0) { cov = m == self; rr.w |= 0x80000000u; }
                }
            }
            if (cov) {
                code = eb == e0 ? pf_code : (int)a.codes[(ent.base_flag & ~int64_t(15)) + v];
                strand = (int)(ent.base_flag & 1);
            }
        }
        unsigned long long m = __ballot(cov);
#pragma unroll
        for (int b = 0; b < 4; b++) {
            const unsigned long long mb = __ballot(cov && code == b), f = __ballot(cov && code == b && strand == 0);
            fw[b] += __popcll(f);
            rv[b] += __popcll(mb & ~f);
        }
        const int room = a.maxcov - n_all;
        n_all += __popcll(m);
        if (!ok || room <= 0) continue;
        while (__popcll(m) > room) m &= ~(1ull << (63 - __builtin_clzll(m)));
        const bool sel = ((m >> lane) & 1ull) && code < 4;
        const unsigned long long ms = __ballot(sel);
        if (sel) {
            rr.w |= (uint32_t)code << 28;
            rec[wv].r[nsel + __popcll(ms & ((1ull << lane) - 1ull))] = rr;
        }
        nsel += __popcll(ms);
    }
    __builtin_amdgcn_fence(__ATOMIC_ACQ_REL, "wavefront");
    __builtin_amdgcn_wave_barrier();
    {
        typedef const uint8_t __attribute__((address_space(1))) *gbyte_ptr;
        constexpr int U = 8;
        for (int g0 = 0; g0 < nsel; g0 += 64) {
            const int ng = min(64, nsel - g0);
            int len = 0, jlo = 0;
            if (lane < ng) {
                const uint4 rr = rec[wv].r[g0 + lane];
                int jhi = 0;
                const int32_t st = (int32_t)rr.z;
                const int64_t en = (int64_t)st + (int64_t)(rr.w & 0x0fffffffu);
#pragma unroll
                for (int w = 32; w > 0; w >>= 1) {
                    const int32_t cl = colL[wv][jlo + w - 1], ch2 = colL[wv][jhi + w - 1];
                    if (cl < st) jlo += w;
                    if ((int64_t)ch2 < en) jhi += w;
                }
                if (MATES && (rr.w >> 31)) { jlo = 0; jhi = ncols; }
                len = jhi - jlo;
            }
            int pin = len;
#pragma unroll
            for (int o = 1; o < 64; o <<= 1) {
                const int y = __shfl_up(pin, o, 64);
                if (lane >= o) pin += y;
            }
            const int Pc = __builtin_amdgcn_readlane(pin, 63);
            const int dj = jlo - (pin - len);
            if (lane < 41) endL[wv][2 * lane] = endL[wv][2 * lane + 1] = 0u;
            __builtin_amdgcn_fence(__ATOMIC_ACQ_REL, "wavefront");
            __builtin_amdgcn_wave_barrier();
            if (len > 0) atomicOr(&endL[wv][(pin - 1) >> 5], 1u << ((pin - 1) & 31));
            __builtin_amdgcn_fence(__ATOMIC_ACQ_REL, "wavefront");
            __builtin_amdgcn_wave_barrier();
            const int ew_lo = lane < 41 ? (int)endL[wv][2 * lane] : 0, ew_hi = lane < 41 ? (int)endL[wv][2 * lane + 1] : 0;
            int base = 0;
            for (int q0 = 0; q0 < Pc; q0 += 64 * U) {
                int jk[U];
                uint32_t bc[U];
#pragma unroll
                for (int u = 0; u < U; u++) {
                    bc[u] = 4;
                    jk[u] = 0;
                    const int qs = q0 + u * 64;
                    if (qs < Pc) {
                        const uint32_t wlo = (uint32_t)__builtin_amdgcn_readlane(ew_lo, qs >> 6), whi = (uint32_t)__builtin_amdgcn_readlane(ew_hi, qs >> 6);
                        const int q = qs + lane;
                        const bool valid = q < Pc;
                        const int r = valid ? base + (int)__builtin_amdgcn_mbcnt_hi(whi, __builtin_amdgcn_mbcnt_lo(wlo, 0u)) : 0;
                        base += __builtin_popcount(wlo) + __builtin_popcount(whi);
                        const uint4 rr = rec[wv].r[g0 + r];
                        const int djr = __shfl(dj, r, 64);
                        const int j = valid ? q + djr : 0;
                        const int32_t cj = colL[wv][j];
                        const uint32_t off = (uint32_t)(cj - (int32_t)rr.z);
                        jk[u] = j * 4 + (int)((rr.w >> 28) & 7u);
                        if (MATES && valid && (rr.w >> 31)) {
                            const int64_t key = (int64_t)((((uint64_t)rr.y << 32) | rr.x) - (uint64_t)(uintptr_t)a.codes) - (int64_t)(int32_t)rr.z + ((int32_t)rr.z & ~15);
                            bc[u] = (uint32_t)named_code(a, key, cj);
                        } else if (valid && j == nl) bc[u] = (rr.w >> 28) & 7u;
                        else if (valid && off < (rr.w & 0x0fffffffu)) bc[u] = ((gbyte_ptr)(uintptr_t)(((uint64_t)rr.y << 32) | rr.x))[off];
                    }
                }
#pragma unroll
                for (int u = 0; u < U; u++)
                    if (bc[u] < 4) atomicAdd(&cntL[wv][jk[u]], 1u << (8 * bc[u]));
            }
        }
    }
    __builtin_amdgcn_fence(__ATOMIC_ACQ_REL, "wavefront");
    __builtin_amdgcn_wave_barrier();
    const int ns = min(n_all, a.maxcov);
    {
        const int o = NBR - nl;
        const int src = lane - o;
        const bool have = ok && lane < 41 && src >= 0 && src < ncols;
        const int sl = have ? src : 0;
        const int rc_s = __shfl(rc_col, have ? src : lane, 64);
        const int odd = s & 1;
        int16_t *T = rec[wv].h + odd;
        if (lane < 41) {
            auto put_row = [&](int row, int v0, int v1, int v2, int v3, int v4) {
                int16_t *d = T + row * (41 * 5) + lane * 5;
                d[0] = (int16_t)v0; d[1] = (int16_t)v1; d[2] = (int16_t)v2; d[3] = (int16_t)v3; d[4] = (int16_t)v4;
            };
            const int rcs = have ? rc_s : 4;
            put_row(0, rcs == 0, rcs == 1, rcs == 2, rcs == 3, 0);
#pragma unroll
            for (int i = 0; i < 4; i++) {
                const uint32_t cs = have ? cntL[wv][sl * 4 + i] : 0u;
                int vv[4];
#pragma unroll
                for (int b = 0; b < 4; b++) {
                    const int val = (int)((cs >> (8 * b)) & 0xffu);
                    vv[b] = b == rcs ? -val : val;
                }
                put_row(1 + i, vv[0], vv[1], vv[2], vv[3], (have && i == rc_centre) ? 1 : 0);
            }
        }
        __builtin_amdgcn_fence(__ATOMIC_ACQ_REL, "wavefront");
        __builtin_amdgcn_wave_barrier();
        int16_t *dst = reinterpret_cast<int16_t *>(a.x) + (int64_t)s * NC_SNP_TENSOR;
        uint32_t *d32 = reinterpret_cast<uint32_t *>(dst + odd);
        const uint32_t *t32 = rec[wv].w + odd;
#pragma unroll
        for (int i = 0; i < (NC_SNP_TENSOR - 1) / 2; i += 64) d32[i + lane] = t32[i + lane];
        if (lane == 0) dst[odd ? 0 : NC_SNP_TENSOR - 1] = T[odd ? 0 : NC_SNP_TENSOR - 1];
    }
    if (lane == 0) {
        a.ref_out[s] = rc_centre;
        a.depth[s] = ns;
        a.valid[s] = ok ? 1 : 0;
    }
    if (lane < 4) {
        a.fwd[s * 4 + lane] = fw[lane];
        a.rev[s * 4 + lane] = rv[lane];
    }
}

__global__ void k_nbr_index(const int32_t *__restrict__ nbr_pos, int n_nbr, int32_t pos0, int n_cidx, int32_t *__restrict__ cidx)
{
    const int b = blockIdx.x * blockDim.x + threadIdx.x;
    if (b >= n_cidx) return;
    const int64_t key = (int64_t)pos0 + ((int64_t)b << NBR_IDX_SHIFT);
    int lo = 0, hi = n_nbr;
    while (lo < hi) {
        const int mid = (lo + hi) >> 1;
        if ((int64_t)nbr_pos[mid] < key) lo = mid + 1; else hi = mid;
    }
    cidx[b] = lo;
}

__global__ __launch_bounds__(256) void k_chunk_scale(const int32_t *__restrict__ chunk_off, const int32_t *__restrict__ depth,
                                                     const uint8_t *__restrict__ valid, const int32_t *__restrict__ site_n,
                                                     double train_cov, int mode, double *__restrict__ scale,
                                                     double *__restrict__ chunk_depth)
{
    const int c = blockIdx.x;
    const int s0 = chunk_off[c], s1 = chunk_off[c + 1];
    long long sum = 0, cntv = 0;
    for (int s = s0 + threadIdx.x; s < s1; s += 256)
        if (valid[s]) { sum += depth[s]; cntv++; }
    __shared__ long long ssum[256], scnt[256];
    ssum[threadIdx.x] = sum;
    scnt[threadIdx.x] = cntv;
    __syncthreads();
    for (int o = 128; o > 0; o >>= 1) {
        if (threadIdx.x < o) { ssum[threadIdx.x] += ssum[threadIdx.x + o]; scnt[threadIdx.x] += scnt[threadIdx.x + o]; }
        __syncthreads();
    }
    const double mean = scnt[0] ? (double)ssum[0] / (double)scnt[0] : 0.0;
    if (threadIdx.x == 0) chunk_depth[c] = mean;
    for (int s = s0 + threadIdx.x; s < s1; s += 256)
        scale[s] = mode == 0 ? train_cov / mean : train_cov / (double)site_n[s];
}

}

extern "C" {

int nc_snp_featurize(nc_ctx *ctx, const nc_readpack *pack, const uint8_t *ref_code_dev, int32_t ref_pos0, int32_t ref_len,
                     int32_t seq_mode, int32_t maxcov, int32_t min_nbr_sites, float *x_dev, int32_t *ref_code_out_dev,
                     int32_t *fwd_dp_dev, int32_t *rev_dp_dev, int32_t *site_depth_dev, uint8_t *valid_dev)
{
    if (!ctx) return NC_ERR_ARG;
    if (!ctx->have_scan) return nc_fail(ctx, NC_ERR_STATE, "nc_snp_featurize: call nc_snp_scan first");
    if (!pack || !ref_code_dev || seq_mode < 0 || seq_mode > 4)
        return nc_fail(ctx, NC_ERR_ARG, "nc_snp_featurize: bad argument");
    if (maxcov < 1 || maxcov > MAXCOV_CAP)
        return nc_fail(ctx, NC_ERR_ARG, "nc_snp_featurize: maxcov %d outside [1,%d]", maxcov, MAXCOV_CAP);
    if (ctx->n_sites == 0) return NC_OK;
    if (!x_dev || !ref_code_out_dev || !fwd_dp_dev || !rev_dp_dev || !site_depth_dev || !valid_dev)
        return nc_fail(ctx, NC_ERR_ARG, "nc_snp_featurize: null output");
    if (((uintptr_t)x_dev) & 15) return nc_fail(ctx, NC_ERR_ARG, "nc_snp_featurize: x_dev must be 16-byte aligned");
    if (ref_pos0 != pack->tile_pos0 || (int64_t)ref_len < (int64_t)pack->n_tiles * pack->tile_size)
        return nc_fail(ctx, NC_ERR_ARG, "nc_snp_featurize: ref_code must cover the pack's tile grid");
    NC_HIP(ctx, hipSetDevice(ctx->device));
    FeatArgs a;
    a.codes = pack->codes;
    a.tile_off = pack->tile_off;
    a.tile_ent = pack->tile_ent;
    a.tile_pos0 = pack->tile_pos0;
    a.tile_shift = pack->tile_size == 1024 ? 10 : pack->tile_size == 2048 ? 11 : 12;
    a.ref_code = ref_code_dev;
    a.ref_pos0 = ref_pos0;
    a.nbr_pos = (const int32_t *)ctx->nbr_pos.p;
    a.n_nbr = ctx->n_nbr;
    const int n_cidx = (int)(((int64_t)pack->n_tiles * pack->tile_size) >> NBR_IDX_SHIFT) + 2;
    NC_TRY(nc_ensure(ctx, ctx->nbr_idx, (size_t)n_cidx * 4));
    a.cidx = (const int32_t *)ctx->nbr_idx.p;
    a.cidx_pos0 = pack->tile_pos0;
    a.n_cidx = n_cidx;
    a.site_pos = (const int32_t *)ctx->site_pos.p;
    a.site_chunk = (const int32_t *)ctx->site_chunk.p;
    a.chunk_start = (const int32_t *)ctx->chunk_start.p;
    a.chunk_end = (const int32_t *)ctx->chunk_end.p;
    a.n_sites = ctx->n_sites;
    a.mode = seq_mode;
    a.maxcov = maxcov;
    a.min_nbr_sites = min_nbr_sites;
    a.x = x_dev;
    a.ref_out = ref_code_out_dev;
    a.fwd = fwd_dp_dev;
    a.rev = rev_dp_dev;
    a.depth = site_depth_dev;
    a.valid = valid_dev;
    a.x_i16 = ctx->x_i16 ? 1 : 0;
    a.mate_key = (const int64_t *)ctx->mate_key;
    a.mate_rec = (const int4 *)ctx->mate_rec;
    a.n_mates = ctx->n_mates;
    const char *fp = getenv("NC_FEAT_PAIRS");
    const bool pairs = maxcov < MAXCOV_SMALL && a.x_i16 && !(fp && atoi(fp) == 0);
    if (a.n_mates > 0 && !pairs)
        return nc_fail(ctx, NC_ERR_UNSUPPORTED, "nc_snp_featurize: alignments that share read names (nc_snp_set_mates) need the int16 tensor format and maxcov < %d", MAXCOV_SMALL);
    NcTimer tm(ctx, 1);
    hipLaunchKernelGGL(k_nbr_index, dim3((n_cidx + 255) / 256), dim3(256), 0, ctx->stream, a.nbr_pos, a.n_nbr, a.cidx_pos0, n_cidx,
                       (int32_t *)ctx->nbr_idx.p);
    const dim3 grid((ctx->n_sites + 3) / 4);
    if (maxcov < MAXCOV_SMALL) {
        if (pairs && a.n_mates > 0) hipLaunchKernelGGL(k_featurize_pairs<true>, grid, dim3(256), 0, ctx->stream, a);
        else if (pairs) hipLaunchKernelGGL(k_featurize_pairs<false>, grid, dim3(256), 0, ctx->stream, a);
        else if (a.x_i16) hipLaunchKernelGGL((k_featurize<MAXCOV_SMALL, true>), grid, dim3(256), 0, ctx->stream, a);
        else hipLaunchKernelGGL((k_featurize<MAXCOV_SMALL, false>), grid, dim3(256), 0, ctx->stream, a);
    } else {
        if (a.x_i16) hipLaunchKernelGGL((k_featurize<MAXCOV_CAP, true>), grid, dim3(256), 0, ctx->stream, a);
        else hipLaunchKernelGGL((k_featurize<MAXCOV_CAP, false>), grid, dim3(256), 0, ctx->stream, a);
    }
    NC_HIP(ctx, hipGetLastError());
    tm.stop();
    return NC_OK;
}

int nc_snp_set_mates(nc_ctx *ctx, int32_t n_mates, const int64_t *d_mate_key, const int32_t *d_mate_rec)
{
    if (!ctx) return NC_ERR_ARG;
    if (n_mates < 0 || (n_mates > 0 && (!d_mate_key || !d_mate_rec || ((uintptr_t)d_mate_rec & 15))))
        return nc_fail(ctx, NC_ERR_ARG, "nc_snp_set_mates: bad argument");
    ctx->n_mates = n_mates;
    ctx->mate_key = n_mates ? d_mate_key : nullptr;
    ctx->mate_rec = n_mates ? d_mate_rec : nullptr;
    return NC_OK;
}

int nc_snp_scale(nc_ctx *ctx, const int32_t *site_depth_dev, const uint8_t *valid_dev, double train_coverage, int32_t mode,
                 double *scale_dev, double *chunk_depth_host)
{
    if (!ctx) return NC_ERR_ARG;
    if (!ctx->have_scan) return nc_fail(ctx, NC_ERR_STATE, "nc_snp_scale: call nc_snp_scan first");
    if (mode != 0 && mode != 1) return nc_fail(ctx, NC_ERR_ARG, "nc_snp_scale: mode must be 0 or 1");
    NC_TRY(nc_ensure(ctx, ctx->chunk_depth, (size_t)ctx->n_chunks * 8));
    if (ctx->n_sites > 0) {
        if (!site_depth_dev || !valid_dev || !scale_dev) return nc_fail(ctx, NC_ERR_ARG, "nc_snp_scale: null argument");
        hipLaunchKernelGGL(k_chunk_scale, dim3(ctx->n_chunks), dim3(256), 0, ctx->stream, (const int32_t *)ctx->chunk_off.p,
                           site_depth_dev, valid_dev, (const int32_t *)ctx->site_n.p, train_coverage, mode, scale_dev,
                           (double *)ctx->chunk_depth.p);
        NC_HIP(ctx, hipGetLastError());
    } else {
        NC_HIP(ctx, hipMemsetAsync(ctx->chunk_depth.p, 0, (size_t)ctx->n_chunks * 8, ctx->stream));
    }
    if (chunk_depth_host) {
        NC_HIP(ctx, hipMemcpyAsync(chunk_depth_host, ctx->chunk_depth.p, (size_t)ctx->n_chunks * 8, hipMemcpyDeviceToHost,
                                   ctx->stream));
        NC_HIP(ctx, hipStreamSynchronize(ctx->stream));
    }
    return NC_OK;
}

int nc_snp_chunk_depth_async(nc_ctx *ctx, void *copy_stream, double *chunk_depth_host_pinned)
{
    if (!ctx) return NC_ERR_ARG;
    if (!copy_stream || !chunk_depth_host_pinned) return nc_fail(ctx, NC_ERR_ARG, "nc_snp_chunk_depth_async: null argument");
    if (!ctx->have_scan || !ctx->chunk_depth.p) return nc_fail(ctx, NC_ERR_STATE, "nc_snp_chunk_depth_async: call nc_snp_scale first");
    if (!ctx->scale_ev) NC_HIP(ctx, hipEventCreateWithFlags(&ctx->scale_ev, hipEventDisableTiming));
    NC_HIP(ctx, hipEventRecord(ctx->scale_ev, ctx->stream));
    NC_HIP(ctx, hipStreamWaitEvent((hipStream_t)copy_stream, ctx->scale_ev, 0));
    NC_TRY(nc_d2h(ctx, chunk_depth_host_pinned, ctx->chunk_depth.p, (size_t)ctx->n_chunks * 8, (hipStream_t)copy_stream));
    return NC_OK;
}

}
```

### nanocaller_amd/csrc/nc_scan.hip

```cpp
#include <algorithm>

#include "nc_common.h"

namespace {

__device__ __forceinline__ uint32_t lut8(uint32_t x, uint32_t lo, uint32_t hi) { return __builtin_amdgcn_perm(hi, lo, x); }

constexpr uint32_t LUT_LO[5] = {0x00000001u, 0x00000100u, 0x00010000u, 0x01000000u, 0x01010101u};
constexpr uint32_t LUT_HI[5] = {0u, 0u, 0u, 0u, 0x00000001u};

struct ScanP {
    int32_t mincov;
    int32_t haploid;
    double min_af, t0, t1;
    int32_t scan_lo, scan_hi;
};

struct ScanX {
    int32_t sample;
    uint32_t seed;
    uint32_t keep[6];
};

__device__ __forceinline__ uint32_t mix32(int32_t p, uint32_t seed)
// ... 111 lines not shown
    __syncthreads();
    uint32_t wpre = 0, total = 0;
#pragma unroll
    for (int i = 0; i < BLOCK / 64; i++) {
        const uint32_t s = wsum[i];
        if (i < wv) wpre += s;
        total += s;
    }
    const uint32_t excl = wpre + incl - mine;
    int on = excl & 0xFFFF, oc = excl >> 16;
    const int64_t sbase = (int64_t)t * TILE;
#pragma unroll
    for (int i = 0; i < 16; i++) {
        if (nbr_mask & (1u << i)) stage_nbr[sbase + on++] = P0 + i;
        if (cand_mask & (1u << i)) {
            const int d = i >> 2, k = i & 3;
            const int wi = 2 * d + (k & 1), sh = (k >> 1) * 16;
            const int r = (rw[d] >> (8 * k)) & 0xFF;
            uint32_t alt = 0;
#pragma unroll
            for (int b = 0; b < 4; b++) {
                const uint32_t cb = (wide[b][wi] >> sh) & 0xFFFF;
                if (b != r && cb > alt) alt = cb;
            }
            stage_cpos[sbase + oc] = P0 + i;
            stage_cn[sbase + oc] = (int32_t)((wide[4][wi] >> sh) & 0xFFFF);
            stage_calt[sbase + oc] = (int32_t)alt;
            oc++;
        }
    }
    if (threadIdx.x == 0) tile_cnt[t] = make_int2((int)(total & 0xFFFF), (int)(total >> 16));
}

__global__ __launch_bounds__(256) void k_site_bits(int32_t n, const int32_t *__restrict__ pos, int32_t tile_pos0, int64_t npos,
                                                   uint32_t *__restrict__ bits)
{
    const int64_t i = (int64_t)blockIdx.x * 256 + threadIdx.x;
    if (i >= n) return;
    const int64_t g = (int64_t)pos[i] - tile_pos0;
    if (g < 0 || g >= npos) return;
    atomicOr(&bits[g >> 5], 1u << (g & 31));
}

__global__ __launch_bounds__(1024) void k_tile_prefix(const int2 *__restrict__ cnt, int2 *__restrict__ pre, int n,
                                                      int32_t *__restrict__ totals)
{
    __shared__ int2 wsum[16];
    const int lane = threadIdx.x & 63, wv = threadIdx.x >> 6;
    const int per = ((n + 15) / 16 + 63) & ~63;
    const int b0 = min(n, wv * per), b1 = min(n, b0 + per);
    int2 sum = make_int2(0, 0);
#pragma unroll 4
    for (int i = b0 + lane; i < b1; i += 64) {
        const int2 v = cnt[i];
        sum.x += v.x; sum.y += v.y;
    }
    const int2 winc = make_int2(nc_wave_incl_scan(sum.x), nc_wave_incl_scan(sum.y));
    if (lane == 63) wsum[wv] = winc;
    __syncthreads();
    int cx = 0, cy = 0, tx = 0, ty = 0;
    for (int w = 0; w < 16; w++) {
        const int2 t = wsum[w];
        if (w < wv) { cx += t.x; cy += t.y; }
        tx += t.x; ty += t.y;
    }
#pragma unroll 4
    for (int base = b0; base < b1; base += 64) {
        const int i = base + lane;
        const int2 v = i < b1 ? cnt[i] : make_int2(0, 0);
        const int ix = nc_wave_incl_scan(v.x), iy = nc_wave_incl_scan(v.y);
        if (i < b1) pre[i] = make_int2(cx + ix - v.x, cy + iy - v.y);
        cx += __builtin_amdgcn_readlane(ix, 63);
        cy += __builtin_amdgcn_readlane(iy, 63);
    }
    if (threadIdx.x == 0) { totals[0] = tx; totals[1] = ty; }
}

__global__ __launch_bounds__(256) void k_compact(int tile, const int2 *__restrict__ cnt, const int2 *__restrict__ pre,
                                                 const int32_t *__restrict__ stage_nbr, const int32_t *__restrict__ stage_cpos,
                                                 const int32_t *__restrict__ stage_cn, const int32_t *__restrict__ stage_calt,
                                                 int32_t *__restrict__ nbr_pos, int32_t *__restrict__ cand_pos,
                                                 int32_t *__restrict__ cand_n, int32_t *__restrict__ cand_alt, int cap_nbr, int cap_cand)
{
    const int t = blockIdx.x;
    const int2 c = cnt[t], p = pre[t];
    const int64_t sb = (int64_t)t * tile;
    for (int i = threadIdx.x; i < c.x; i += 256)
        if (p.x + i < cap_nbr) nbr_pos[p.x + i] = stage_nbr[sb + i];
    for (int i = threadIdx.x; i < c.y; i += 256) {
        if (p.y + i >= cap_cand) continue;
        cand_pos[p.y + i] = stage_cpos[sb + i];
        cand_n[p.y + i] = stage_cn[sb + i];
        cand_alt[p.y + i] = stage_calt[sb + i];
    }
}

__device__ __forceinline__ int lower_bound_dev(const int32_t *a, int n, int32_t key)
{
    int lo = 0, hi = n;
    while (lo < hi) {
        const int mid = (lo + hi) >> 1;
        if (a[mid] < key) lo = mid + 1; else hi = mid;
    }
    return lo;
}

__device__ __forceinline__ int chunk_range(const int32_t *__restrict__ cand_pos, int n, int32_t cs, int32_t ce, int32_t *lo_out)
{
    const int lo = lower_bound_dev(cand_pos, n, cs);
    const int hi = ce == INT32_MAX ? n : lower_bound_dev(cand_pos, n, ce + 1);
    *lo_out = lo;
    return hi > lo ? hi - lo : 0;
}

__global__ __launch_bounds__(1024) void k_chunk_prefix(const int32_t *__restrict__ cand_pos, int cap_cand, const int32_t *__restrict__ cs,
                                                       const int32_t *__restrict__ ce, int32_t *__restrict__ chunk_lo,
                                                       int32_t *__restrict__ chunk_cnt, int32_t *__restrict__ off, int n,
                                                       int32_t *__restrict__ totals)
{
    __shared__ int wsum[16];
    __shared__ int carry;
    if (threadIdx.x == 0) carry = 0;
    __syncthreads();
    const int lane = threadIdx.x & 63, wv = threadIdx.x >> 6;
    const int n_cand = totals[1] < cap_cand ? totals[1] : cap_cand;
    for (int base = 0; base < n; base += 1024) {
        const int i = base + threadIdx.x;
        int v = 0;
        if (i < n) {
            int32_t lo;
            v = chunk_range(cand_pos, n_cand, cs[i], ce[i], &lo);
            chunk_lo[i] = lo;
            chunk_cnt[i] = v;
        }
        int inc = v;
        inc = (decltype(inc))nc_wave_incl_scan((int32_t)inc);
        if (lane == 63) wsum[wv] = inc;
        __syncthreads();
        int wp = 0, tot = 0;
        for (int w = 0; w < 16; w++) {
            const int s = wsum[w];
            if (w < wv) wp += s;
            tot += s;
        }
        const int c = carry;
        if (i < n) off[i] = c + wp + inc - v;
        __syncthreads();
        if (threadIdx.x == 0) carry = c + tot;
        __syncthreads();
    }
    if (threadIdx.x == 0) { off[n] = carry; totals[2] = carry; }
}

__global__ void k_sites(int n_sites, int n_chunks, const int32_t *__restrict__ chunk_off, const int32_t *__restrict__ chunk_lo,
                        const int32_t *__restrict__ cand_pos, const int32_t *__restrict__ cand_n,
                        const int32_t *__restrict__ cand_alt, int32_t *__restrict__ site_pos,
                        int32_t *__restrict__ site_chunk, int32_t *__restrict__ site_n, int32_t *__restrict__ site_alt)
{
    const int s = blockIdx.x * blockDim.x + threadIdx.x;
    if (s >= n_sites) return;
    int lo = 0, hi = n_chunks;
    while (lo < hi) {
        const int mid = (lo + hi) >> 1;
        if (chunk_off[mid + 1] <= s) lo = mid + 1; else hi = mid;
    }
    const int c = lo;
    const int ci = chunk_lo[c] + (s - chunk_off[c]);
    site_pos[s] = cand_pos[ci];
    site_chunk[s] = c;
    site_n[s] = cand_n[ci];
    site_alt[s] = cand_alt[ci];
}

__global__ void k_selftest(uint32_t *out)
{
    const uint32_t x = 0x07040300u | (threadIdx.x & 3);
    uint32_t r = 0;
    for (int c = 0; c < 5; c++) r |= lut8(x, LUT_LO[c], LUT_HI[c]) << c;
    out[threadIdx.x] = r;
}

}

int nc_selftest_device(nc_ctx *ctx)
{
    uint32_t *d = nullptr, h[64];
    NC_HIP(ctx, hipMalloc(&d, sizeof h));
    hipLaunchKernelGGL(k_selftest, dim3(1), dim3(64), 0, ctx->stream, d);
    NC_HIP(ctx, hipGetLastError());
    NC_HIP(ctx, hipMemcpyAsync(h, d, sizeof h, hipMemcpyDeviceToHost, ctx->stream));
    NC_HIP(ctx, hipStreamSynchronize(ctx->stream));
    NC_HIP(ctx, hipFree(d));
    for (int l = 0; l < 64; l++) {
        uint32_t exp = 0;
        const int c0 = l & 3;
        exp |= (1u << c0) | (1u << 4);
        exp |= ((1u << 3) | (1u << 4)) << 8;
        exp |= (1u << 4) << 16;
        if (h[l] != exp)
            return nc_fail(ctx, NC_ERR_SELFTEST, "v_perm_b32 byte-LUT self-test: lane %d got %08x expected %08x", l, h[l], exp);
    }
    return NC_OK;
}

template <bool SITES, bool EXT>
static void launch_scan(nc_ctx *ctx, const nc_readpack *pack, const uint8_t *ref_code_dev, const ScanP &sp, const uint16_t *sb, const uint16_t *nb,
                        const ScanX &sx)
{
    auto *sn = (int32_t *)ctx->stage_nbr.p;
    auto *sc = (int32_t *)ctx->stage_cpos.p;
    auto *scn = (int32_t *)ctx->stage_cn.p;
    auto *sca = (int32_t *)ctx->stage_calt.p;
    auto *tc = (int2 *)ctx->tile_cnt.p;
    if (pack->tile_size == 1024)
        hipLaunchKernelGGL((k_scan<64, SITES, EXT>), dim3(pack->n_tiles), dim3(64), 0, ctx->stream, pack->codes, pack->tile_off,
                           pack->tile_ent, pack->tile_pos0, ref_code_dev, sp, sn, sc, scn, sca, tc, sb, nb, sx);
    else if (pack->tile_size == 2048)
        hipLaunchKernelGGL((k_scan<128, SITES, EXT>), dim3(pack->n_tiles), dim3(128), 0, ctx->stream, pack->codes, pack->tile_off,
                           pack->tile_ent, pack->tile_pos0, ref_code_dev, sp, sn, sc, scn, sca, tc, sb, nb, sx);
    else
        hipLaunchKernelGGL((k_scan<256, SITES, EXT>), dim3(pack->n_tiles), dim3(256), 0, ctx->stream, pack->codes, pack->tile_off,
                           pack->tile_ent, pack->tile_pos0, ref_code_dev, sp, sn, sc, scn, sca, tc, sb, nb, sx);
}

static int build_bits(nc_ctx *ctx, DevBuf &bits, int32_t n, const int32_t *d_pos, int32_t tile_pos0, int64_t npos)
{
    NC_HIP(ctx, hipMemsetAsync(bits.p, 0, (size_t)(npos / 8), ctx->stream));
    hipLaunchKernelGGL(k_site_bits, dim3((n + 255) / 256), dim3(256), 0, ctx->stream, n, d_pos, tile_pos0, npos, (uint32_t *)bits.p);
    NC_HIP(ctx, hipGetLastError());
    return NC_OK;
}

extern "C" {

static int scan_compact(nc_ctx *ctx, int cap_nbr, int cap_cand)
{
    const int tile = ctx->scan_tile, n_tiles = ctx->scan_n_tiles, n_chunks = ctx->scan_n_chunks;
    hipLaunchKernelGGL(k_compact, dim3(n_tiles), dim3(256), 0, ctx->stream, tile, (int2 *)ctx->tile_cnt.p, (const int2 *)ctx->tile_pre.p,
                       (int32_t *)ctx->stage_nbr.p, (int32_t *)ctx->stage_cpos.p, (int32_t *)ctx->stage_cn.p, (int32_t *)ctx->stage_calt.p,
                       (int32_t *)ctx->nbr_pos.p, (int32_t *)ctx->cand_pos.p, (int32_t *)ctx->cand_n.p, (int32_t *)ctx->cand_alt.p, cap_nbr, cap_cand);
    NC_HIP(ctx, hipGetLastError());
    hipLaunchKernelGGL(k_chunk_prefix, dim3(1), dim3(1024), 0, ctx->stream, (const int32_t *)ctx->cand_pos.p, cap_cand,
                       (const int32_t *)ctx->chunk_start.p, (const int32_t *)ctx->chunk_end.p, (int32_t *)ctx->chunk_lo.p,
                       (int32_t *)ctx->chunk_cnt.p, (int32_t *)ctx->chunk_off.p, n_chunks, (int32_t *)ctx->totals.p);
    NC_HIP(ctx, hipGetLastError());
    NC_TRY(nc_d2h(ctx, ctx->mbox, ctx->totals.p, 16, ctx->stream));
    if (!ctx->scan_tot_ev) NC_HIP(ctx, hipEventCreateWithFlags(&ctx->scan_tot_ev, hipEventDisableTiming));
    NC_HIP(ctx, hipEventRecord(ctx->scan_tot_ev, ctx->stream));
    return NC_OK;
}
static int cap_of(const DevBuf &b) { return (int)std::min<size_t>(b.cap / 4, (size_t)INT32_MAX); }

int nc_snp_scan_begin(nc_ctx *ctx, const nc_readpack *pack, const uint8_t *ref_code_dev, int32_t ref_pos0, int32_t ref_len,
                      int32_t scan_lo, int32_t scan_hi, const nc_scan_params *params, int32_t n_chunks,
                      const int32_t *chunk_start_host, const int32_t *chunk_end_host)
{
    if (!ctx) return NC_ERR_ARG;
    if (!pack || !ref_code_dev || !params || n_chunks <= 0 || !chunk_start_host || !chunk_end_host)
        return nc_fail(ctx, NC_ERR_ARG, "nc_snp_scan: null argument");
    const int tile = pack->tile_size;
    if (!(tile == 1024 || tile == 2048 || tile == 4096) || pack->n_tiles <= 0 || !pack->codes || !pack->tile_off ||
        (pack->n_entries && !pack->tile_ent) || (pack->tile_pos0 & 15))
        return nc_fail(ctx, NC_ERR_ARG, "nc_snp_scan: malformed read pack");
    if (ref_pos0 != pack->tile_pos0 || (int64_t)ref_len < (int64_t)pack->n_tiles * tile)
        return nc_fail(ctx, NC_ERR_ARG, "nc_snp_scan: ref_code must start at tile_pos0 (%d) and cover %lld positions",
                       pack->tile_pos0, (long long)pack->n_tiles * tile);
    if (scan_hi < scan_lo) return nc_fail(ctx, NC_ERR_ARG, "nc_snp_scan: empty scan range");
    NC_HIP(ctx, hipSetDevice(ctx->device));
    ctx->have_scan = false;
    ctx->scan_begun = false;
    const int64_t npos = (int64_t)pack->n_tiles * tile;
    NC_TRY(nc_ensure(ctx, ctx->stage_nbr, npos * 4));
    NC_TRY(nc_ensure(ctx, ctx->stage_cpos, npos * 4));
    NC_TRY(nc_ensure(ctx, ctx->stage_cn, npos * 4));
    NC_TRY(nc_ensure(ctx, ctx->stage_calt, npos * 4));
    NC_TRY(nc_ensure(ctx, ctx->tile_cnt, (size_t)pack->n_tiles * 8));
    NC_TRY(nc_ensure(ctx, ctx->tile_pre, (size_t)pack->n_tiles * 8));
    NC_TRY(nc_ensure(ctx, ctx->totals, 16));
    NC_TRY(nc_ensure(ctx, ctx->chunk_start, (size_t)n_chunks * 4));
    NC_TRY(nc_ensure(ctx, ctx->chunk_end, (size_t)n_chunks * 4));
    NC_TRY(nc_ensure(ctx, ctx->chunk_lo, (size_t)n_chunks * 4));
    NC_TRY(nc_ensure(ctx, ctx->chunk_cnt, (size_t)n_chunks * 4));
    NC_TRY(nc_ensure(ctx, ctx->chunk_off, ((size_t)n_chunks + 1) * 4));
    NC_TRY(nc_h2d_small(ctx, ctx->chunk_start.p, chunk_start_host, (size_t)n_chunks * 4, ctx->stream));
    NC_TRY(nc_h2d_small(ctx, ctx->chunk_end.p, chunk_end_host, (size_t)n_chunks * 4, ctx->stream));

    ScanP sp;
    sp.mincov = params->mincov;
    sp.haploid = params->haploid;
    sp.min_af = params->min_allele_freq;
    sp.t0 = params->nbr_t0;
    sp.t1 = params->nbr_t1;
    sp.scan_lo = scan_lo;
    sp.scan_hi = scan_hi;

    const bool listed = ctx->n_gsites > 0;
    const bool listed_nbr = ctx->n_nsites > 0;
    const bool ext = listed_nbr || ctx->sample_on;
    if (listed) {
        NC_TRY(nc_ensure(ctx, ctx->site_bits, (size_t)(npos / 8)));
        if (ctx->gsites_only) sp.min_af = 2.0;
    }
    if (listed_nbr) {
        NC_TRY(nc_ensure(ctx, ctx->nbr_bits, (size_t)(npos / 8)));
        if (ctx->nsites_only) sp.t0 = 2.0;
    }
    NcTimer tm(ctx, 0);
    auto *tc = (int2 *)ctx->tile_cnt.p;
    ScanX sx;
    sx.sample = ctx->sample_on ? 1 : 0;
    sx.seed = ctx->sample_seed;
    for (int b = 0; b < 6; b++) sx.keep[b] = ctx->sample_on ? ctx->sample_keep[b] : 0u;
    const auto *sb = listed ? (const uint16_t *)ctx->site_bits.p : nullptr;
    const auto *nb = listed_nbr ? (const uint16_t *)ctx->nbr_bits.p : nullptr;
    if (listed) NC_TRY(build_bits(ctx, ctx->site_bits, ctx->n_gsites, ctx->gsite_pos, pack->tile_pos0, npos));
    if (listed_nbr) NC_TRY(build_bits(ctx, ctx->nbr_bits, ctx->n_nsites, ctx->nsite_pos, pack->tile_pos0, npos));
    if (ext) launch_scan<false, true>(ctx, pack, ref_code_dev, sp, sb, nb, sx);
    else if (listed) launch_scan<true, false>(ctx, pack, ref_code_dev, sp, sb, nb, sx);
    else launch_scan<false, false>(ctx, pack, ref_code_dev, sp, sb, nb, sx);
    NC_HIP(ctx, hipGetLastError());
    tm.stop();
    hipLaunchKernelGGL(k_tile_prefix, dim3(1), dim3(1024), 0, ctx->stream, tc, (int2 *)ctx->tile_pre.p, pack->n_tiles,
                       (int32_t *)ctx->totals.p);
    NC_HIP(ctx, hipGetLastError());
    ctx->scan_tile = tile;
    ctx->scan_n_tiles = pack->n_tiles;
    ctx->scan_n_chunks = n_chunks;
    volatile int32_t *tot = ctx->mbox;
    ctx->scan_cap_nbr = cap_of(ctx->nbr_pos);
    ctx->scan_cap_cand = std::min(cap_of(ctx->cand_pos), std::min(cap_of(ctx->cand_n), cap_of(ctx->cand_alt)));
    if (ctx->scan_cap_nbr == 0 || ctx->scan_cap_cand == 0) {
        NC_TRY(nc_d2h(ctx, ctx->mbox, ctx->totals.p, 16, ctx->stream));
        NC_HIP(ctx, hipStreamSynchronize(ctx->stream));
        NC_TRY(nc_ensure(ctx, ctx->nbr_pos, (size_t)(tot[0] + 1) * 4));
        NC_TRY(nc_ensure(ctx, ctx->cand_pos, (size_t)(tot[1] + 1) * 4));
        NC_TRY(nc_ensure(ctx, ctx->cand_n, (size_t)(tot[1] + 1) * 4));
        NC_TRY(nc_ensure(ctx, ctx->cand_alt, (size_t)(tot[1] + 1) * 4));
        ctx->scan_cap_nbr = cap_of(ctx->nbr_pos);
        ctx->scan_cap_cand = std::min(cap_of(ctx->cand_pos), std::min(cap_of(ctx->cand_n), cap_of(ctx->cand_alt)));
    }
    NC_TRY(scan_compact(ctx, ctx->scan_cap_nbr, ctx->scan_cap_cand));
    ctx->scan_begun = true;
    return NC_OK;
}

int nc_snp_scan_end(nc_ctx *ctx, int32_t *n_nbr, int32_t *n_cand, int32_t *n_sites)
{
    if (!ctx) return NC_ERR_ARG;
    if (!ctx->scan_begun) return nc_fail(ctx, NC_ERR_STATE, "nc_snp_scan_end: no nc_snp_scan_begin on this context");
    ctx->scan_begun = false;
    NC_HIP(ctx, hipSetDevice(ctx->device));
    volatile int32_t *tot = ctx->mbox;
    NC_HIP(ctx, hipEventSynchronize(ctx->scan_tot_ev));
    if (!(tot[0] <= ctx->scan_cap_nbr && tot[1] <= ctx->scan_cap_cand)) {
        NC_TRY(nc_ensure(ctx, ctx->nbr_pos, (size_t)(tot[0] + 1) * 4));
        NC_TRY(nc_ensure(ctx, ctx->cand_pos, (size_t)(tot[1] + 1) * 4));
        NC_TRY(nc_ensure(ctx, ctx->cand_n, (size_t)(tot[1] + 1) * 4));
        NC_TRY(nc_ensure(ctx, ctx->cand_alt, (size_t)(tot[1] + 1) * 4));
        ctx->scan_cap_nbr = cap_of(ctx->nbr_pos);
        ctx->scan_cap_cand = std::min(cap_of(ctx->cand_pos), std::min(cap_of(ctx->cand_n), cap_of(ctx->cand_alt)));
        NC_TRY(scan_compact(ctx, ctx->scan_cap_nbr, ctx->scan_cap_cand));
        NC_HIP(ctx, hipEventSynchronize(ctx->scan_tot_ev));
        if (!(tot[0] <= ctx->scan_cap_nbr && tot[1] <= ctx->scan_cap_cand)) return nc_fail(ctx, NC_ERR_STATE, "nc_snp_scan: outputs still too small after regrowth");
    }
    const int32_t n_chunks = ctx->scan_n_chunks;
    ctx->n_nbr = tot[0];
    ctx->n_cand = tot[1];
    ctx->n_sites = tot[2];
    ctx->n_chunks = n_chunks;
    const size_t ns = (size_t)tot[2] + 1;
    NC_TRY(nc_ensure(ctx, ctx->site_pos, ns * 4));
    NC_TRY(nc_ensure(ctx, ctx->site_chunk, ns * 4));
    NC_TRY(nc_ensure(ctx, ctx->site_n, ns * 4));
    NC_TRY(nc_ensure(ctx, ctx->site_alt, ns * 4));
    if (tot[2] > 0) {
        hipLaunchKernelGGL(k_sites, dim3((tot[2] + 255) / 256), dim3(256), 0, ctx->stream, tot[2], n_chunks,
                           (const int32_t *)ctx->chunk_off.p, (const int32_t *)ctx->chunk_lo.p,
                           (const int32_t *)ctx->cand_pos.p, (const int32_t *)ctx->cand_n.p, (const int32_t *)ctx->cand_alt.p,
                           (int32_t *)ctx->site_pos.p, (int32_t *)ctx->site_chunk.p, (int32_t *)ctx->site_n.p,
                           (int32_t *)ctx->site_alt.p);
        NC_HIP(ctx, hipGetLastError());
    }
    if (!ctx->scan_ev) NC_HIP(ctx, hipEventCreateWithFlags(&ctx->scan_ev, hipEventDisableTiming));
    NC_HIP(ctx, hipEventRecord(ctx->scan_ev, ctx->stream));
    ctx->have_scan = true;
    if (n_nbr) *n_nbr = tot[0];
    if (n_cand) *n_cand = tot[1];
    if (n_sites) *n_sites = tot[2];
    return NC_OK;
}

int nc_snp_scan(nc_ctx *ctx, const nc_readpack *pack, const uint8_t *ref_code_dev, int32_t ref_pos0, int32_t ref_len,
                int32_t scan_lo, int32_t scan_hi, const nc_scan_params *params, int32_t n_chunks,
                const int32_t *chunk_start_host, const int32_t *chunk_end_host, int32_t *n_nbr, int32_t *n_cand,
                int32_t *n_sites)
{
    const int rc = nc_snp_scan_begin(ctx, pack, ref_code_dev, ref_pos0, ref_len, scan_lo, scan_hi, params, n_chunks, chunk_start_host, chunk_end_host);
    return rc != NC_OK ? rc : nc_snp_scan_end(ctx, n_nbr, n_cand, n_sites);
}

int nc_snp_scan_set_sites(nc_ctx *ctx, int32_t n_sites, const int32_t *d_pos, int32_t only)
{
    if (!ctx) return NC_ERR_ARG;
    if (n_sites < 0 || (n_sites > 0 && !d_pos)) return nc_fail(ctx, NC_ERR_ARG, "nc_snp_scan_set_sites: bad argument");
    ctx->n_gsites = n_sites;
    ctx->gsite_pos = n_sites ? d_pos : nullptr;
    ctx->gsites_only = n_sites > 0 && only != 0;
    return NC_OK;
}

int nc_snp_scan_set_nbr_sites(nc_ctx *ctx, int32_t n_sites, const int32_t *d_pos, int32_t only)
{
    if (!ctx) return NC_ERR_ARG;
    if (n_sites < 0 || (n_sites > 0 && !d_pos)) return nc_fail(ctx, NC_ERR_ARG, "nc_snp_scan_set_nbr_sites: bad argument");
    ctx->n_nsites = n_sites;
    ctx->nsite_pos = n_sites ? d_pos : nullptr;
    ctx->nsites_only = n_sites > 0 && only != 0;
    return NC_OK;
}

int nc_snp_scan_set_sampling(nc_ctx *ctx, uint32_t seed, const uint32_t *keep6_host)
{
    if (!ctx) return NC_ERR_ARG;
    ctx->sample_on = keep6_host != nullptr;
    ctx->sample_seed = keep6_host ? seed : 0u;
    for (int b = 0; b < 6; b++) ctx->sample_keep[b] = keep6_host ? keep6_host[b] : 0u;
    return NC_OK;
}

static int scan_fetch(nc_ctx *ctx, hipStream_t st, bool wait, int32_t *nbr_pos, int32_t *site_pos, int32_t *site_chunk, int32_t *site_n,
                      int32_t *site_alt)
{
    if (!ctx) return NC_ERR_ARG;
    if (!ctx->have_scan) return nc_fail(ctx, NC_ERR_STATE, "nc_snp_scan_fetch: no scan on this context");
    const size_t nb = (size_t)ctx->n_nbr * 4, ns = (size_t)ctx->n_sites * 4;
    if (nbr_pos && nb) NC_TRY(nc_d2h(ctx, nbr_pos, ctx->nbr_pos.p, nb, st));
    if (site_pos && ns) NC_TRY(nc_d2h(ctx, site_pos, ctx->site_pos.p, ns, st));
    if (site_chunk && ns) NC_TRY(nc_d2h(ctx, site_chunk, ctx->site_chunk.p, ns, st));
    if (site_n && ns) NC_TRY(nc_d2h(ctx, site_n, ctx->site_n.p, ns, st));
    if (site_alt && ns) NC_TRY(nc_d2h(ctx, site_alt, ctx->site_alt.p, ns, st));
    if (wait) NC_HIP(ctx, hipStreamSynchronize(st));
    return NC_OK;
}

int nc_snp_scan_fetch(nc_ctx *ctx, int32_t *nbr_pos, int32_t *site_pos, int32_t *site_chunk, int32_t *site_n,
                      int32_t *site_alt)
{
    if (!ctx) return NC_ERR_ARG;
    return scan_fetch(ctx, ctx->stream, true, nbr_pos, site_pos, site_chunk, site_n, site_alt);
}

int nc_snp_scan_fetch_async(nc_ctx *ctx, void *copy_stream, int32_t *nbr_pos, int32_t *site_pos, int32_t *site_chunk,
                            int32_t *site_n, int32_t *site_alt)
{
    if (!ctx) return NC_ERR_ARG;
    if (copy_stream && (hipStream_t)copy_stream != ctx->stream && ctx->have_scan && ctx->scan_ev)
        NC_HIP(ctx, hipStreamWaitEvent((hipStream_t)copy_stream, ctx->scan_ev, 0));
    return scan_fetch(ctx, copy_stream ? (hipStream_t)copy_stream : ctx->stream, false, nbr_pos, site_pos, site_chunk, site_n, site_alt);
}

}
```

### nanocaller_amd/engine.py

```python
from __future__ import annotations

import ctypes as C
import os
import weakref
from contextlib import contextmanager
from dataclasses import dataclass

import numpy as np
import torch

from . import _lib
from .pack import HostPack
from .weights import Weights


def _ptr(t):
    return C.c_void_p(t.data_ptr()) if t is not None else None


def sample_thresholds(keep):
    return np.floor(np.asarray(keep, np.float64) * 4294967296.0).astype(np.uint32)


@dataclass
# ... 39 lines not shown
    depth: torch.Tensor | None = None
    valid: torch.Tensor | None = None
    nbr_only: bool = False


class _PinnedPool:

    def __init__(self):
        self.blocks = []

    def get(self, shape, dtype):
        shape = tuple(int(v) for v in (shape if isinstance(shape, (tuple, list, torch.Size)) else (shape,)))
        nbytes = int(np.prod(shape, dtype=np.int64)) * torch.empty(0, dtype=dtype).element_size()
        best = None
        for b in self.blocks:
            if (b[1] is None or b[1]() is None) and b[0].numel() >= nbytes and (best is None or b[0].numel() < best[0].numel()):
                best = b
        if best is None:
            cap = max(4096, nbytes + nbytes // 4)
            best = [torch.empty(cap, dtype=torch.uint8, pin_memory=True), None]
            self.blocks.append(best)
        t = best[0][:nbytes].view(dtype).view(shape)
        arr = t.numpy()
        best[1] = weakref.ref(arr)
        return t, arr


class Engine:

    def __init__(self, device: int = 0):
        if not torch.cuda.is_available():
            raise _lib.NanoCallerHipError("no ROCm device visible: the NanoCaller HIP path has no CPU fallback")
        self.L = _lib.lib()
        self.device = torch.device("cuda", device)
        torch.cuda.set_device(self.device)
        ctx = C.c_void_p()
        rc = self.L.nc_ctx_create(device, C.byref(ctx))
        if rc != _lib.NC_OK:
            raise _lib.NanoCallerHipError("nc_ctx_create(device=%d) failed with status %d" % (device, rc))
        self.ctx = ctx
        self._loaded = {}
        self._pinned = _PinnedPool()
        self.x_int16 = self.exact_fp32 = False
        self.use_torch_stream()

    def close(self):
        if getattr(self, "ctx", None):
            self.L.nc_ctx_destroy(self.ctx)
            self.ctx = None

    def __del__(self):
        try:
            self.close()
        except Exception:
            pass

    def _check(self, rc, what):
        if rc != _lib.NC_OK:
            msg = self.L.nc_last_error(self.ctx)
            raise _lib.NanoCallerHipError("%s failed (%d): %s" % (what, rc, msg.decode() if msg else ""), status=rc)

    def use_torch_stream(self):
        s = torch.cuda.current_stream(self.device)
        if s.cuda_stream == 0 and os.environ.get("NC_ONE_QUEUE", "1") != "0":
            if getattr(self, "_tstream", None) is None:
                self._tstream = torch.cuda.Stream(device=self.device)
            self._tstream.wait_stream(s)
            torch.cuda.set_stream(self._tstream)
            s = self._tstream
        self._check(self.L.nc_ctx_set_stream(self.ctx, C.c_void_p(s.cuda_stream)), "nc_ctx_set_stream")

    def _adopt_thread(self):
        s = torch.cuda.current_stream(self.device)
        if s.cuda_stream == 0 and os.environ.get("NC_ONE_QUEUE", "1") != "0" and getattr(self, "_tstream", None) is not None:
            self._tstream.wait_stream(s)
            torch.cuda.set_stream(self._tstream)

    def set_cnn_precision(self, exact_fp32: bool):
        self._check(self.L.nc_set_cnn_precision(self.ctx, 1 if exact_fp32 else 0), "nc_set_cnn_precision")
        self.exact_fp32 = bool(exact_fp32)

    def set_tensor_format(self, int16: bool):
        self._check(self.L.nc_set_tensor_format(self.ctx, 1 if int16 else 0), "nc_set_tensor_format")
        self.x_int16 = bool(int16)

    @contextmanager
    def _snp_state(self, int16=None, exact_fp32=None, range_flags=None):
        was_i16, was_exact = self.x_int16, self.exact_fp32
        try:
            if int16 is not None and bool(int16) != was_i16:
                self.set_tensor_format(int16)
            if exact_fp32 is not None and bool(exact_fp32) != was_exact:
                self.set_cnn_precision(exact_fp32)
            if range_flags is not None:
                self._check(self.L.nc_cnn_range_watch(self.ctx, C.c_void_p(range_flags.data_ptr())), "nc_cnn_range_watch")
            yield
        finally:
            if range_flags is not None:
                self.L.nc_cnn_range_watch(self.ctx, None)
            if self.exact_fp32 != was_exact:
                self.set_cnn_precision(was_exact)
            if self.x_int16 != was_i16:
                self.set_tensor_format(was_i16)

    TRUNK_KERNELS = {0: "k4_conv12", 2: "k5_trunk_p3", 3: "k5_trunk_lin"}

    def trunk_info(self, int16=None):
        n, k = C.c_int32(), C.c_int32()
        with self._snp_state(int16=int16):
            self._check(self.L.nc_snp_trunk_info(self.ctx, C.byref(n), C.byref(k)), "nc_snp_trunk_info")
        return int(n.value), self.TRUNK_KERNELS[int(k.value)]

    def trunk_mfma_per_site(self) -> int:
        return self.trunk_info()[0]

    def enable_timing(self, on=True, trunk_only=False):
        self._check(self.L.nc_enable_timing(self.ctx, (2 if trunk_only else 1) if on else 0), "nc_enable_timing")

    def last_ms(self, which):
        ms = C.c_float()
        self._check(self.L.nc_last_kernel_ms(self.ctx, which, C.byref(ms)), "nc_last_kernel_ms")
        return float(ms.value)

    def timing_sums(self):
        sums, cnt = np.zeros(6, np.float64), np.zeros(6, np.int64)
        self._check(self.L.nc_timing_sums(self.ctx, _lib.npp(sums), _lib.npp(cnt)), "nc_timing_sums")
        return sums, cnt

    def upload(self, hp: HostPack) -> DevicePack:
        dev = self.device
        ent_bytes = np.frombuffer(hp.tile_ent.tobytes(), np.uint8) if hp.tile_ent.size else np.zeros(16, np.uint8)
        dp = DevicePack(codes=torch.from_numpy(hp.codes).to(dev), tile_off=torch.from_numpy(hp.tile_off).to(dev),
                        tile_ent=torch.from_numpy(ent_bytes.copy()).to(dev), ref_code=torch.from_numpy(hp.ref_code).to(dev),
                        tile_size=hp.tile_size, tile_pos0=hp.tile_pos0, n_tiles=hp.n_tiles,
                        n_entries=int(hp.tile_ent.shape[0]), pos_lo=hp.pos_lo, pos_hi=hp.pos_hi)
        if hp.mates is not None:
            dp.mates = (torch.from_numpy(hp.mates[0]).to(dev), torch.from_numpy(hp.mates[1]).to(dev))
        if hp.ev_off is not None:
            z = lambda a, dt: torch.from_numpy(np.ascontiguousarray(a, dt) if a.size else np.zeros(1, dt)).to(dev)
            dp.events = dict(n_reads=int(hp.read_hap.shape[0]), ev_off=z(hp.ev_off, np.int32), ev_pos=z(hp.ev_pos, np.int32),
                             ev_len=z(hp.ev_len, np.int32), read_hap=z(hp.read_hap, np.uint8))
        return dp

    def load_weights(self, kind: int, w: Weights):
        if self._loaded.get(kind) == w.path:
            return
        if w.kind != kind:
            raise ValueError("weights %s are of kind %d, expected %d" % (w.path, w.kind, kind))
        flat = np.ascontiguousarray(w.flat, np.float32)
        self._check(self.L.nc_load_weights(self.ctx, kind, _lib.npp(flat), flat.size), "nc_load_weights")
        self._loaded[kind] = w.path

    def snp_scan(self, dp: DevicePack, chunks, *, mincov, min_allele_freq, threshold, haploid=False, async_fetch=False, sites=None,
                 sites_only=False, nbr_sites=None, nbr_only=False, sample=None) -> SnpSites:
        def on_device(s):
            if isinstance(s, torch.Tensor):
                d = s.to(device=self.device, dtype=torch.int32).contiguous()
            else:
                a = np.asarray(s).astype(np.int64, copy=False).ravel()
                a = a[(a >= 1) & (a <= np.iinfo(np.int32).max)]
                d = torch.from_numpy(np.ascontiguousarray(a, np.int32)).to(self.device)
            d.record_stream(torch.cuda.current_stream(self.device))
            return d
        d_sites = on_device(sites) if sites is not None else None
        d_nbr = on_device(nbr_sites) if nbr_sites is not None else None
        threshold = [float(threshold[0]), float(threshold[1])]
        if sites_only and (d_sites is None or d_sites.numel() == 0):
            min_allele_freq = 2.0
        if nbr_only and (d_nbr is None or d_nbr.numel() == 0):
            threshold[0] = 2.0
        keep6 = None
        if sample is not None:
            seed, keep = sample
            keep = np.asarray(keep, np.float64).ravel()
            if keep.size != 6 or not np.all((keep >= 0.0) & (keep < 1.0)):
                raise ValueError("snp_scan: sample = (seed, keep) needs six probabilities in [0, 1)")
            keep6 = np.ascontiguousarray(sample_thresholds(keep))
            seed = int(seed) & 0xFFFFFFFF
        cs = np.ascontiguousarray([c[0] for c in chunks], np.int32)
        ce = np.ascontiguousarray([c[1] for c in chunks], np.int32)
        scan_lo = max(1, int(cs.min()) - _lib.FLANK)
        scan_hi = int(ce.max()) + _lib.FLANK
        if scan_lo < dp.pos_lo or min(scan_hi, dp.pos_hi) < scan_lo:
            pass
        params = _lib.ScanParamsC(mincov=int(mincov), min_allele_freq=float(min_allele_freq), nbr_t0=float(threshold[0]),
                                  nbr_t1=float(threshold[1]), haploid=1 if haploid else 0)
        pc = dp.c_struct()
        listed = d_sites is not None and d_sites.numel() > 0
        listed_nbr = d_nbr is not None and d_nbr.numel() > 0
        try:
            if listed:
                self._check(self.L.nc_snp_scan_set_sites(self.ctx, int(d_sites.numel()), _ptr(d_sites), 1 if sites_only else 0), "nc_snp_scan_set_sites")
            if listed_nbr:
                self._check(self.L.nc_snp_scan_set_nbr_sites(self.ctx, int(d_nbr.numel()), _ptr(d_nbr), 1 if nbr_only else 0), "nc_snp_scan_set_nbr_sites")
            if keep6 is not None:
                self._check(self.L.nc_snp_scan_set_sampling(self.ctx, seed, _lib.npp(keep6)), "nc_snp_scan_set_sampling")
            self._check(self.L.nc_snp_scan_begin(self.ctx, C.byref(pc), _ptr(dp.ref_code), dp.tile_pos0, dp.ref_code.numel(), scan_lo,
                                                 scan_hi, C.byref(params), len(chunks), _lib.npp(cs), _lib.npp(ce)), "nc_snp_scan_begin")
        finally:
            if listed:
                self.L.nc_snp_scan_set_sites(self.ctx, 0, None, 0)
            if listed_nbr:
                self.L.nc_snp_scan_set_nbr_sites(self.ctx, 0, None, 0)
            if keep6 is not None:
                self.L.nc_snp_scan_set_sampling(self.ctx, 0, None)
        n_nbr, n_cand, n_sites = C.c_int32(), C.c_int32(), C.c_int32()
        self._check(self.L.nc_snp_scan_end(self.ctx, C.byref(n_nbr), C.byref(n_cand), C.byref(n_sites)), "nc_snp_scan_end")
        N = n_sites.value
        hb, h = self._pinned.get((4, max(N, 1)), torch.int32)
        ptr = [C.c_void_p(hb[i].data_ptr()) for i in range(4)]
        if async_fetch:
            self._check(self.L.nc_snp_scan_fetch_async(self.ctx, self._copy_stream_ptr(), None, ptr[0], ptr[1], ptr[2], ptr[3]),
                        "nc_snp_scan_fetch_async")
        else:
            self._check(self.L.nc_snp_scan_fetch(self.ctx, None, ptr[0], ptr[1], ptr[2], ptr[3]), "nc_snp_scan_fetch")
        return SnpSites(n_sites=N, n_nbr=n_nbr.value, pos=h[0, :N], chunk=h[1, :N], dp=h[2, :N], alt=h[3, :N], nbr_only=bool(nbr_only))

    def fetch_nbr_sites(self, n_nbr) -> np.ndarray:
        out = np.empty(n_nbr, np.int32)
        self._check(self.L.nc_snp_scan_fetch(self.ctx, _lib.npp(out), None, None, None, None), "nc_snp_scan_fetch")
        return out

    REFCONF_TILE = 4096

    @staticmethod
    def _refconf_params(error, bands, haploid):
        from . import gvcf
        c_m, c_x, c_h = gvcf.constants(error)
        b = gvcf.gq_bands(bands)
        prm = _lib.RefconfParamsC(c_m=c_m, c_x=c_x, c_h=c_h, haploid=1 if haploid else 0, n_bands=len(b))
        for k, v in enumerate(b):
            prm.band[k] = v
        return prm

    def refconf_columns(self, dp: DevicePack):
        npos = dp.n_tiles * dp.tile_size
        if dp.ref_code.numel() < npos:
            raise ValueError("refconf_columns: the pack's reference codes hold %d columns, its tile grid %d" % (dp.ref_code.numel(), npos))
        words = torch.empty(npos, dtype=torch.int32, device=self.device)
        pc = dp.c_struct()
        self._check(self.L.nc_refconf_columns(self.ctx, C.byref(pc), _ptr(dp.ref_code), dp.tile_pos0, npos, _ptr(words)), "nc_refconf_columns")
        return words, dp.ref_code[:npos].clone(), dp.tile_pos0

    def refconf_blocks(self, words, dpk, chunks, cuts, *, error, bands, haploid=False, device_out=False):
        tile_pos0 = int(getattr(dpk, "tile_pos0", dpk))
        prm = self._refconf_params(error, bands, haploid)
        cs = np.ascontiguousarray([c[0] for c in chunks], np.int32)
        ce = np.ascontiguousarray([c[1] for c in chunks], np.int32)
        d_cs = d_ce = None
        n_cut = 0
        if cuts is not None and len(cuts):
            d_cuts = cuts if isinstance(cuts, torch.Tensor) else torch.from_numpy(np.ascontiguousarray(cuts, np.int32).reshape(-1, 2))
            d_cuts = d_cuts.to(device=self.device, dtype=torch.int32)
            d_cs, d_ce = d_cuts[:, 0].contiguous(), d_cuts[:, 1].contiguous()
            n_cut = int(d_cs.numel())
        nb = C.c_int64()
        self._check(self.L.nc_refconf_blocks(self.ctx, _ptr(words), tile_pos0, int(words.numel()), len(chunks), _lib.npp(cs), _lib.npp(ce), n_cut,
                                             _ptr(d_cs), _ptr(d_ce), C.byref(prm), C.byref(nb)), "nc_refconf_blocks")
        n = int(nb.value)
        if device_out:
            out = torch.empty((n, 6), dtype=torch.int32, device=self.device)
            self._check(self.L.nc_refconf_fetch(self.ctx, _ptr(out) if n else None), "nc_refconf_fetch")
            return out
        out = np.empty((n, 6), np.int32)
        self._check(self.L.nc_refconf_fetch(self.ctx, _lib.npp(out) if n else None), "nc_refconf_fetch")
        return out

    def refconf_text(self, blocks, ref_code, tile_pos0, chrom, *, error, haploid=False):
        prm = self._refconf_params(error, None, haploid)
        d_blocks = blocks if isinstance(blocks, torch.Tensor) else torch.from_numpy(np.ascontiguousarray(blocks, np.int32).reshape(-1, 6))
        d_blocks = d_blocks.to(device=self.device, dtype=torch.int32).contiguous()
        n = int(d_blocks.shape[0])
        off = torch.empty(n + 1, dtype=torch.int64, device=self.device)
        nbytes = C.c_int64()
        args = (self.ctx, n, _ptr(d_blocks) if n else None, _ptr(ref_code), int(tile_pos0), int(ref_code.numel()), str(chrom).encode(), C.byref(prm), _ptr(off))
        self._check(self.L.nc_refconf_text(*args, None, 0, C.byref(nbytes)), "nc_refconf_text")
        text = torch.empty(max(int(nbytes.value), 1), dtype=torch.uint8, device=self.device)
        self._check(self.L.nc_refconf_text(*args, _ptr(text), int(nbytes.value), None), "nc_refconf_text")
        return text[:int(nbytes.value)].cpu().numpy(), off.cpu().numpy()

    def snp_featurize(self, dp: DevicePack, sites: SnpSites, *, seq, maxcov, min_nbr_sites=1, int16=None) -> SnpSites:
        if sites.nbr_only:
            min_nbr_sites = int(min_nbr_sites) + 1
        N = sites.n_sites
        dev = self.device
        want16 = self.x_int16 if int16 is None else bool(int16)
        i16 = want16 or dp.mates is not None
        xb = N * 1025 * (2 if i16 else 4)
        a16 = lambda v: (v + 15) & ~15
        o_ref = a16(xb); o_fwd = a16(o_ref + 4 * N); o_rev = a16(o_fwd + 16 * N); o_dep = a16(o_rev + 16 * N); o_val = a16(o_dep + 4 * N)
        buf = torch.empty(o_val + N + 16, dtype=torch.uint8, device=dev)
        sites.x = buf[:xb].view(torch.int16 if i16 else torch.float32).view(N, 5, 41, 5)
        sites.ref_code = buf[o_ref:o_ref + 4 * N].view(torch.int32)
        sites.fwd_dp = buf[o_fwd:o_fwd + 16 * N].view(torch.int32).view(N, 4)
        sites.rev_dp = buf[o_rev:o_rev + 16 * N].view(torch.int32).view(N, 4)
        sites.depth = buf[o_dep:o_dep + 4 * N].view(torch.int32)
        sites.valid = buf[o_val:o_val + N]
        pc = dp.c_struct()
        if dp.mates is not None:
            self._check(self.L.nc_snp_set_mates(self.ctx, int(dp.mates[0].numel()), _ptr(dp.mates[0]), _ptr(dp.mates[1])), "nc_snp_set_mates")
        try:
            with self._snp_state(int16=i16):
                self._check(self.L.nc_snp_featurize(self.ctx, C.byref(pc), _ptr(dp.ref_code), dp.tile_pos0, dp.ref_code.numel(),
                                                    _lib.SEQ_MODES[seq], int(maxcov), int(min_nbr_sites), _ptr(sites.x),
                                                    _ptr(sites.ref_code), _ptr(sites.fwd_dp), _ptr(sites.rev_dp), _ptr(sites.depth),
                                                    _ptr(sites.valid)), "nc_snp_featurize")
        finally:
            if dp.mates is not None:
                self.L.nc_snp_set_mates(self.ctx, 0, None, None)
        if not want16 and i16:
            sites.x = sites.x.to(torch.float32)
        return sites

    def snp_scale(self, sites: SnpSites, n_chunks, train_coverage, per_site=False, async_fetch=False):
        scale = torch.empty(sites.n_sites, dtype=torch.float64, device=self.device)
        if not async_fetch:
            cd = np.zeros(n_chunks, np.float64)
            self._check(self.L.nc_snp_scale(self.ctx, _ptr(sites.depth), _ptr(sites.valid), float(train_coverage),
                                            1 if per_site else 0, _ptr(scale), _lib.npp(cd)), "nc_snp_scale")
            return scale, cd
        hb, cd = self._pinned.get((max(int(n_chunks), 1),), torch.float64)
        self._check(self.L.nc_snp_scale(self.ctx, _ptr(sites.depth), _ptr(sites.valid), float(train_coverage),
                                        1 if per_site else 0, _ptr(scale), None), "nc_snp_scale")
        self._check(self.L.nc_snp_chunk_depth_async(self.ctx, self._copy_stream_ptr(), C.c_void_p(hb.data_ptr())), "nc_snp_chunk_depth_async")
        return scale, cd[:int(n_chunks)]

    def x_limit(self, kind) -> float:
        v = C.c_float()
        self._check(self.L.nc_cnn_x_limit(self.ctx, kind, C.byref(v)), "nc_cnn_x_limit")
        return float(v.value)

    def snp_forward_guarded(self, kind, x, ref_code, scale, scale_mode=0):
        n = int(x.shape[0])
        flags = torch.zeros(max(n, 1), dtype=torch.uint8, device=self.device)
        probs, gt = self.snp_forward(kind, x, ref_code, scale, scale_mode, range_flags=flags)
        idx = torch.nonzero(flags[:n]).squeeze(1)
        if idx.numel():
            self.range_rerun(kind, x, ref_code, scale, scale_mode, idx, probs, gt)
        return probs, gt, int(idx.numel())

    def range_rerun(self, kind, x, ref_code, scale, scale_mode, idx, probs, gt):
        xs = x[idx].to(torch.float32).contiguous()
        with self._snp_state(exact_fp32=True):
            p2, g2 = self.snp_forward(kind, xs, ref_code[idx].contiguous(), scale[idx].contiguous() if scale is not None else None, scale_mode,
                                      want_gt=gt is not None)
        probs[idx] = p2
        if gt is not None and g2 is not None:
            gt[idx] = g2

    def snp_forward(self, kind, x, ref_code, scale, scale_mode=0, want_gt=True, drain=False, range_flags=None):
        if x.dtype not in (torch.int16, torch.float32):
            raise ValueError("snp_forward: tensors of dtype %s (int16 or float32 expected)" % x.dtype)
        n = int(x.shape[0])
        probs = torch.empty((n, 4), dtype=torch.float32, device=self.device)
        gt = torch.empty((n, 2), dtype=torch.float32, device=self.device) if (want_gt and kind == _lib.MODEL_SNP) else None
        with self._snp_state(int16=x.dtype == torch.int16, range_flags=range_flags):
            if not drain:
                self._check(self.L.nc_snp_forward(self.ctx, kind, n, _ptr(x), _ptr(ref_code), _ptr(scale), int(scale_mode),
                                                  _ptr(probs), _ptr(gt)), "nc_snp_forward")
                return probs, gt
            hp, hp_np = self._pinned.get((n, 4), torch.float32)
            hg, hg_np = self._pinned.get((n, 2), torch.float32) if gt is not None else (None, None)
            self._check(self.L.nc_snp_forward_drain(self.ctx, kind, n, _ptr(x), _ptr(ref_code), _ptr(scale), int(scale_mode),
                                                    _ptr(probs), _ptr(gt), self._copy_stream_ptr(), C.c_void_p(hp.data_ptr()),
                                                    C.c_void_p(hg.data_ptr()) if hg is not None else None), "nc_snp_forward_drain")
            return probs, gt, hp_np, hg_np

    def indel_forward(self, kind, x):
        n = int(x.shape[0])
        nout = 4 if kind == _lib.MODEL_INDEL else 1
        probs = torch.empty((n, nout), dtype=torch.float32, device=self.device)
        self._check(self.L.nc_indel_forward(self.ctx, kind, n, _ptr(x), _ptr(probs)), "nc_indel_forward")
        return probs

    def snp_phase(self, site_pos, site_alleles, read_group, n_groups, *, max_cov=15, reads=None, csr=None, realign=None, site_gt=None,
                  distrust_cost=1, weights=None, bam_quals=None) -> dict:
        pos = np.ascontiguousarray(site_pos, np.int32)
        h = self._phase_open(pos, site_alleles, reads, csr, realign)
        try:
            self._phase_weigh(h, weights, bam_quals)
            if site_gt is None:
                self._check(self.L.nc_snp_phase_solve(self.ctx, h, int(max_cov)), "nc_snp_phase_solve")
            else:
                gt = np.ascontiguousarray(site_gt, np.uint8)
                if gt.shape != pos.shape:
                    raise ValueError("snp_phase: site_gt holds %d classes for %d sites" % (gt.size, pos.size))
                self._check(self.L.nc_snp_phase_solve_gt(self.ctx, h, int(max_cov), _lib.npp(gt), int(distrust_cost)), "nc_snp_phase_solve_gt")
            grp = np.ascontiguousarray(read_group, np.int32)
            self._check(self.L.nc_haplotag_run(self.ctx, h, int(n_groups), _lib.npp(grp)), "nc_haplotag_run")
            return self._phase_result(h, with_gt=site_gt is not None, with_weights=weights is not None or bam_quals is not None)
        finally:
            self.L.nc_snp_phase_free(h)

    def _phase_open(self, pos, site_alleles, reads, csr, realign):
        L, h = self.L, C.c_void_p()
        if realign is not None or reads is not None:
            al = np.ascontiguousarray(site_alleles, np.uint8).reshape(-1, 2)
            torch.cuda.current_stream(self.device).synchronize()
        if realign is not None:
            codes, reads_c, n_events, n_ins, ref_code = realign
            rc = L.nc_snp_phase_realign(self.ctx, _ptr(codes), codes.numel(), C.byref(reads_c), int(n_events), int(n_ins), _ptr(ref_code),
                                        int(ref_code.numel()), pos.size, _lib.npp(pos), _lib.npp(al), C.byref(h))
            self._check(rc, "nc_snp_phase_realign")
        elif reads is not None:
            codes, rs, re_, so = reads
            rc = L.nc_snp_phase_gather(self.ctx, _ptr(codes), codes.numel(), int(rs.numel()), _ptr(rs), _ptr(re_), _ptr(so), pos.size, _lib.npp(pos),
                                       _lib.npp(al), C.byref(h))
            self._check(rc, "nc_snp_phase_gather")
        else:
            off, site, allele = (np.ascontiguousarray(a, t) for a, t in zip(csr, (np.int64, np.int32, np.uint8)))
            self._check(L.nc_snp_phase_load(self.ctx, off.size - 1, pos.size, _lib.npp(pos), _lib.npp(off), _lib.npp(site), _lib.npp(allele),
                                            C.byref(h)), "nc_snp_phase_load")
        return h

    def _phase_view(self, h):
        v = _lib.PhaseArraysC()
        self.L.nc_snp_phase_view(h, C.byref(v))
        return v

    def _phase_weigh(self, h, weights, bam_quals):
        if weights is not None and bam_quals is not None:
            raise ValueError("snp_phase: weights= and bam_quals= are two sources of the same weights")
        if weights is None and bam_quals is None:
            return
        v = self._phase_view(h)
        if weights is not None:
            ew, ok = (None if a is None else np.ascontiguousarray(a, np.uint8) for a in weights)
            if (ew is not None and ew.size != v.n_entries) or (ok is not None and ok.size != v.n_reads):
                raise ValueError("snp_phase: weights= holds %s weights / %s flags for %d entries / %d reads"
                                 % (None if ew is None else ew.size, None if ok is None else ok.size, v.n_entries, v.n_reads))
            self._check(self.L.nc_snp_phase_set_weights(self.ctx, h, None if ew is None else _lib.npp(ew), None if ok is None else _lib.npp(ok)),
                        "nc_snp_phase_set_weights")
        else:
            raw, rec_off, mapq_min, default_weight, w_max = bam_quals
            if rec_off.dtype != torch.int64 or rec_off.numel() != v.n_reads or raw.dtype != torch.uint8:
                raise ValueError("snp_phase: bam_quals= needs a uint8 record stream and %d int64 record offsets, one per read" % v.n_reads)
            torch.cuda.current_stream(self.device).synchronize()
            self._check(self.L.nc_snp_phase_weights_from_bam(self.ctx, h, _ptr(raw), int(raw.numel()), _ptr(rec_off), int(mapq_min), int(default_weight),
                                                             int(w_max)), "nc_snp_phase_weights_from_bam")

    def _phase_result(self, h, with_gt, with_weights) -> dict:
        L, v = self.L, self._phase_view(h)

        def a(ptr, n, dt):
            return np.ctypeslib.as_array(C.cast(ptr, C.POINTER(np.ctypeslib.as_ctypes_type(dt))), (n,)).copy() if n and ptr else np.zeros(0, dt)
        R, S, nb, ng = v.n_reads, v.n_sites, v.n_blocks, v.n_groups
        extra = {}
        if with_gt:
            g = C.c_void_p()
            L.nc_snp_phase_genotypes(h, C.byref(g))
            extra = dict(site_gt=a(g, S, np.uint8))
        if with_weights:
            pw, pm, po = C.c_void_p(), C.c_void_p(), C.c_void_p()
            L.nc_snp_phase_weights(h, C.byref(pw), C.byref(pm), C.byref(po))
            extra.update(entry_weight=a(pw, v.n_entries, np.uint8), read_mapq=a(pm, R, np.uint8), read_ok=a(po, R, np.uint8))
        return dict(entry_off=a(v.entry_off, R + 1, np.int64), entry_site=a(v.entry_site, v.n_entries, np.int32),
                    entry_allele=a(v.entry_allele, v.n_entries, np.uint8), side=a(v.read_side, R, np.int8),
                    site_block=a(v.site_block, S, np.int32), site_h=a(v.site_h, S, np.uint8), site_phased=a(v.site_phased, S, np.uint8).astype(bool),
                    site_ps=a(v.site_ps, S, np.int32), block_first=a(v.block_first, nb, np.int32), block_last=a(v.block_last, nb, np.int32),
                    block_ps=a(v.block_ps, nb, np.int32), block_cost=a(v.block_cost, nb, np.int64), group_hp=a(v.group_hp, ng, np.uint8),
                    group_ps=a(v.group_ps, ng, np.int32), ms=dict(zip(("gather", "select", "dp", "haplotag"), list(v.ms))), **extra)

# ... 225 lines not shown
```

### nanocaller_amd/snpCaller.py

```python
from __future__ import annotations

import datetime
import os
import queue
import shutil
import struct
import sys
import zlib

import numpy as np
import torch

from . import _lib
from .engine import get_engine
from .generate_SNP_pileups import device_pack_for, release_contig
from .weights import Weights, get_haploid_SNP_model, get_SNP_model

num_to_base_map = {0: 'A', 1: 'G', 2: 'T', 3: 'C'}
_B = "AGTC"


def _qual(p, cap=99.0, mult=-10.0):
    return min(cap, mult * np.log10(1e-10 + 1 - float(p)))

# ... 15 lines not shown
        if k[j] >= 2:
            if p1 == r:
                a = (fwd_dp[j][p2], rev_dp[j][p2])
                out.append(head + '%s\t%.3f\t%s\t%s\t%s\t%s:%d:%.4f:%d,%d:%d,%d:%d,%d\n' % (
                    _B[p2], _qual(pr[p2]), 'PASS', info, fmt, '0/1', d, sum(a) / d, sum(ref_dp), sum(a), ref_dp[0], a[0],
                    ref_dp[1], a[1]))
            elif p2 == r and pr[p2] >= 0.5:
                a = (fwd_dp[j][p1], rev_dp[j][p1])
                out.append(head + '%s\t%.3f\t%s\t%s\t%s\t%s:%d:%.4f:%d,%d:%d,%d:%d,%d\n' % (
                    _B[p1], _qual(pr[p2]), 'PASS', info, fmt, '0/1', d, sum(a) / d, sum(ref_dp), sum(a), ref_dp[0], a[0],
                    ref_dp[1], a[1]))
            elif p2 != r and p1 != r and pr[p2] >= 0.5:
                a1 = (fwd_dp[j][p1], rev_dp[j][p1])
                a2 = (fwd_dp[j][p2], rev_dp[j][p2])
                out.append(head + '%s,%s\t%.3f\t%s\t%s\t%s\t%s:%d:%.4f,%.4f:%d,%d,%d:%d,%d,%d:%d,%d,%d\n' % (
                    _B[p1], _B[p2], _qual(pr[p2]), 'PASS', info, fmt, '1/2', d, sum(a1) / d, sum(a2) / d, sum(ref_dp),
                    sum(a1), sum(a2), ref_dp[0], a1[0], a2[0], ref_dp[1], a1[1], a2[1]))
        elif k[j] == 1 and r != p1 and pr[p1] >= 0.5:
            a = (fwd_dp[j][p1], rev_dp[j][p1])
            out.append(head + '%s\t%.3f\t%s\t%s\t%s\t%s:%d:%.4f:%d,%d:%d,%d:%d,%d\n' % (
                _B[p1], _qual(pr[p1]), 'PASS', info, fmt, '1/1', d, sum(a) / d, sum(ref_dp), sum(a), ref_dp[0], a[0],
                ref_dp[1], a[1]))
        elif k[j] == 1 and r == p1:
            out.append(head + '%s\t%.3f\t%s\t%s\t%s\t%s:%d:.:.:.:.\n' % ('.', _qual(pr[p1]), 'REF', info, fmt, './.', d))
        else:
            out.append(head + '%s\t%.3f\t%s\t%s\t%s\t%s:%d:.:.:.:.\n' % ('.', 0, 'LOW', info, fmt, './.', d))
    return out


def snp_vcf_lines_haploid(chrom, pos, ref_idx, probs, dp, freq):
    probs = np.asarray(probs, np.float32)
    pred = np.argmax(probs, 1)
    out = []
    for j in range(len(pos)):
        pr = probs[j]
        p = int(pred[j])
        r = int(ref_idx[j])
        info = 'PR=' + ','.join("{:.4f}".format(x) for x in pr[[0, 3, 1, 2]]) + ";FQ={:.4f}".format(freq[j])
        out.append('%s\t%d\t.\t%s\t%s\t%.3f\t%s\t%s\tGT:DP:VF:AD:ADF:ADR\t%s:%d:%.4f:.:.:.\n' % (
            chrom, pos[j], _B[r], _B[p], _qual(pr[p], 999.0, -100.0), 'PASS' if p != r else 'REF', info, '1/1', int(dp[j]),
            freq[j]))
    return out


def argsort4(probs):
    import ctypes as C
    L = _lib.lib()
    probs = np.ascontiguousarray(probs, np.float32)
    n = probs.shape[0]
    order = np.empty((n, 4), np.int32)
    ties = np.empty(max(n, 1), np.int64)
    nt = C.c_int64()
    rc = L.nc_argsort4(_lib.npp(probs), n, _lib.npp(order), C.byref(nt), _lib.npp(ties), ties.size)
    if rc != _lib.NC_OK:
        raise _lib.NanoCallerHipError("nc_argsort4 failed (%d)" % rc)
    if nt.value:
        t = ties[:nt.value]
        order[t] = np.argsort(probs[t], axis=1)
    return order


def snp_vcf_text(chrom, pos, ref_idx, probs, dp, freq, fwd_dp=None, rev_dp=None, haploid=False, as_array=False, out=None):
    import ctypes as C
    L = _lib.lib()
    n = len(pos)
    i32 = lambda a: np.ascontiguousarray(a, np.int32)
    probs = np.ascontiguousarray(probs, np.float32)
    order = None if haploid else argsort4(probs)
    pos_, ref_, dp_ = i32(pos), i32(ref_idx), i32(dp)
    freq_ = np.ascontiguousarray(freq, np.float64)
    fwd_ = None if haploid else i32(fwd_dp)
    rev_ = None if haploid else i32(rev_dp)
    cap = (400 + len(chrom)) * max(n, 1) + 1024
    if out is None or out.size < cap:
        out = np.empty(cap, np.uint8)
    cap = out.size
    nb = C.c_int64()
    rc = L.nc_snp_vcf_format(chrom.encode(), n, _lib.npp(pos_), _lib.npp(ref_), _lib.npp(probs), _lib.npp(order),
                             _lib.npp(dp_), _lib.npp(freq_), _lib.npp(fwd_), _lib.npp(rev_), 1 if haploid else 0,
                             _lib.npp(out), cap, C.byref(nb))
    if rc != _lib.NC_OK:
        raise _lib.NanoCallerHipError("nc_snp_vcf_format failed (%d)" % rc)
    return out[:nb.value] if as_array else out[:nb.value].tobytes()


VCF_HEADER = (
    '##fileformat=VCFv4.2\n'
    '##FILTER=<ID=PASS,Description="All filters passed">\n'
    '##FILTER=<ID=LOW,Description="All alleles have probability less than 50%.">\n'
    '##FILTER=<ID=REF,Description="Homozygous Reference. Only reference allele has greater than 50% probability. '
    'All alternative alleles having probability less than 50%.">\n'
    '{contigs}'
    '##FORMAT=<ID=GT,Number=1,Type=String,Description="Genotype">\n'
    '##FORMAT=<ID=DP,Number=1,Type=Integer,Description="Depth">\n'
    '##FORMAT=<ID=AD,Number=R,Type=Integer,Description="Allelic depths for the ref and alt alleles in the order listed">\n'
    '##FORMAT=<ID=ADF,Number=R,Type=Integer,Description="Allelic depths on forward strand for the ref and alt alleles in the order listed">\n'
    '##FORMAT=<ID=ADR,Number=R,Type=Integer,Description="Allelic depths on reverse strand for the ref and alt alleles in the order listed">\n'
    '##FORMAT=<ID=VF,Number=A,Type=Float,Description="Alternative allele frequency in the order listed">\n'
    '##INFO=<ID=PR,Number=4,Type=Float,Description="Probability of presence of alleles A, C, G and T, in the given order. '
    'Probability of each base is out of 1, independent of each other.">\n'
    '##INFO=<ID=FQ,Number=1,Type=Float,Description="Maximum frequency of non-reference base.">\n'
    '#CHROM\tPOS\tID\tREF\tALT\tQUAL\tFILTER\tINFO\tFORMAT\t{sample}\n')


PARAM_KEYS = frozenset(['chunks_list', 'regions_list', 'sam_path', 'fasta_path', 'mincov', 'maxcov', 'min_allele_freq', 'min_nbr_sites',
                        'threshold', 'snp_model', 'vcf_path', 'prefix', 'sample', 'seq', 'supplementary', 'exclude_bed',
                        'suppress_progress', 'disable_coverage_normalization'])

_WEIGHTS = {}


def _weights(path):
    if path not in _WEIGHTS:
        _WEIGHTS[path] = Weights(path)
    return _WEIGHTS[path]


class PendingCall:

    def __init__(self, finish):
        self._finish, self._res = finish, None

    def result(self):
        if self._finish is not None:
            self._res, self._finish = self._finish(), None
        return self._res


def call_chunks(params, chunks, device=0, dpk=None, defer=False, pipeline=None):
    if pipeline:
        raise ValueError("call_chunks(pipeline=True): the pipelined-CNN path (NC_PIPE_CNN=1) was removed")
    chrom = chunks[0]['chrom']
    ploidy = chunks[0]['ploidy']
    assert all(c['chrom'] == chrom and c['ploidy'] == ploidy for c in chunks)
    eng = get_engine(device)
    eng.use_torch_stream()
    if ploidy == 'diploid':
        path, train_cov = get_SNP_model(params['snp_model'])
        if path is None:
            print('Invalid SNP model name or path', flush=True)
            sys.exit(1)
        kind = _lib.MODEL_SNP
    else:
        path, train_cov = get_haploid_SNP_model(params)
        kind = _lib.MODEL_SNP_HAP
    eng.load_weights(kind, _weights(path))
    if dpk is None:
        from .generate_SNP_pileups import contig_span
        dpk = device_pack_for(params, chrom, device, span=contig_span(params['sam_path'], chrom, chunks))
    from .genotype_sites import count_listed, neighbor_sites_for, sites_for
    listed, only = sites_for(params, chrom)
    nbr_listed, nbr_only = neighbor_sites_for(params, chrom)
    spans = [(c['start'], c['end']) for c in chunks]
    sites = eng.snp_scan(dpk, spans, mincov=params['mincov'],
                         min_allele_freq=params['min_allele_freq'], threshold=params['threshold'],
                         haploid=(ploidy == 'haploid'), async_fetch=True, sites=listed, sites_only=only,
                         nbr_sites=nbr_listed, nbr_only=nbr_only)
    res = dict(chrom=chrom, ploidy=ploidy, n=0, genotype_listed=count_listed(listed, spans, ())[0], genotype_emitted=0)
    from . import gvcf
    if gvcf.enabled(params):
        res['gvcf'] = eng.refconf_columns(dpk)
    if sites.n_sites == 0:
        eng.wait_copies()
        return PendingCall(lambda: res) if defer else res
    exact = eng.exact_fp32
    eng.snp_featurize(dpk, sites, seq=params['seq'], maxcov=params['maxcov'], min_nbr_sites=params['min_nbr_sites'], int16=not exact)
    all_valid = bool(sites.valid.all().item()) if params['min_nbr_sites'] > 1 or sites.nbr_only else True
    per_site = bool(params.get('disable_coverage_normalization'))
    scale, chunk_depth = eng.snp_scale(sites, len(chunks), train_cov, per_site=per_site, async_fetch=True)
    scan_copied = eng.copy_event()
    h_ref, h_fwd, h_rev, h_valid = eng.to_host_async([sites.ref_code, sites.fwd_dp, sites.rev_dp, None if all_valid else sites.valid])
    flags = None if exact else torch.zeros(sites.n_sites, dtype=torch.uint8, device=eng.device)
    d_probs, d_gt, h_probs, h_gt = eng.snp_forward(kind, sites.x, sites.ref_code, scale, scale_mode=1 if per_site else 0, drain=True, range_flags=flags)
    h_nflag = None if exact else eng.to_host_async([flags.sum(dtype=torch.int32).reshape(1)])[0]
    drained = eng.copy_event()
    scan_copied.synchronize()
    freq = sites.alt.astype(np.float64) / sites.dp.astype(np.float64)

    def finish():
        drained.synchronize()
        n_rerun = int(h_nflag[0]) if h_nflag is not None else 0
        if n_rerun:
            idx = torch.nonzero(flags).squeeze(1)
            eng.use_torch_stream()
            eng.range_rerun(kind, sites.x, sites.ref_code, scale, 1 if per_site else 0, idx, d_probs, d_gt)
            ih = idx.cpu().numpy()
            h_probs[ih] = d_probs[idx].cpu().numpy()
            if h_gt is not None and d_gt is not None:
                h_gt[ih] = d_gt[idx].cpu().numpy()
        res['range_reruns'] = n_rerun
        out = dict(pos=sites.pos, chunk=sites.chunk, ref=h_ref, probs=h_probs, gt=h_gt, dp=sites.dp, alt=sites.alt,
                   fwd_dp=h_fwd, rev_dp=h_rev, freq=freq)
        if not all_valid:
            m = h_valid.astype(bool)
            out = {k: (v[m] if v is not None else None) for k, v in out.items()}
        res.update(out, n=int(out['pos'].shape[0]), chunk_depth=chunk_depth)
        res['genotype_listed'], res['genotype_emitted'] = count_listed(listed, spans, out['pos'])
        return res
    return PendingCall(finish) if defer else finish()


def _prepare_wire(params, chrom, grp):
    from .generate_SNP_pileups import _check_supported, _exclude_rows, _resolve, contig_span
    from .wire import build_wire_from_world
    span = contig_span(params['sam_path'], chrom, grp)
    world = _resolve(params['sam_path'], chrom, params.get('fasta_path'), span)
    _check_supported(world, params['sam_path'], chrom, bool(params.get('supplementary')), by_name=True)
    kw = dict(pos_lo=span[0], pos_hi=span[1]) if span else {}
    return build_wire_from_world(world, supplementary=bool(params.get('supplementary')), exclude=_exclude_rows(params, chrom), **kw)


def _prepare_device(dbam, params, chrom, grp, ref=None):
    from .device_fasta import reference_for
    from .generate_SNP_pileups import _exclude_rows, span_of
    span = span_of(grp, dbam.ref_lengths[dbam.ref_names.index(chrom)] if chrom in dbam.ref_names else 0)
    ref = ref.result() if ref is not None else reference_for(params['fasta_path'], chrom, dbam.device, params)
    return dbam.prepare(chrom, ref, supplementary=bool(params.get('supplementary')), exclude=_exclude_rows(params, chrom), span=span, by_name=True)


def _plan_runs(params, keys, device):
    from .device_bam import DeviceIngestUnavailable, plan_shares
    run_end, run_dev = [len(keys)] * len(keys), [None] * len(keys)
    try:
        lim = os.environ.get('NC_DEVICE_INGEST_SHARE_GB')
        order = list(dict.fromkeys(k[0] for k in keys))
        share_of = {}
        for n_sh, (cs, fits) in enumerate(plan_shares(params['sam_path'], order, None if lim is None else int(float(lim) * (1 << 30)), device=device)):
            for c in cs:
                share_of[c] = (n_sh, tuple(cs) if fits else None)
        a0 = 0
        for j in range(1, len(keys) + 1):
            if j == len(keys) or share_of[keys[j][0]][0] != share_of[keys[a0][0]][0]:
                for q in range(a0, j):
                    run_end[q], run_dev[q] = j, share_of[keys[a0][0]][1]
                a0 = j
    except DeviceIngestUnavailable:
        pass
    return run_end, run_dev


class _Ingest:

    def __init__(self, params, keys, groups, device):
        from concurrent.futures import ThreadPoolExecutor
        self.params, self.keys, self.groups, self.device = params, keys, groups, device
        self.run_end, self.run_dev = [len(keys)] * len(keys), [None] * len(keys)
        if params.get('device_ingest', os.environ.get('NC_DEVICE_INGEST', '1') != '0') and params.get('fasta_path'):
            from .device_bam import ensure_index
            ensure_index(params['sam_path'], params, device)
            self.run_end, self.run_dev = _plan_runs(params, keys, device)
        self.ahead = max(1, int(os.environ.get('NC_INGEST_AHEAD', 2)))
        self.pool = ThreadPoolExecutor(max_workers=self.ahead)
        self.dbam = self.prepare = self.uploader = self.codes = None
        self.preps, self.refs, self.nxt = [], {}, 0

    def _prepare_next(self, run_end):
        if self.nxt < run_end:
            k = self.keys[self.nxt]
            self.preps.append(self.pool.submit(self.prepare, k[0], self.groups[k]))
            self.nxt += 1

    def enter_run(self, i):
        from concurrent.futures import ThreadPoolExecutor
        from .device_bam import DeviceIngestUnavailable, open_device_bam, release as release_device_bam
        from .device_fasta import reference_for
        params, device, refs = self.params, self.device, self.refs
        self.dbam = self.prepare = None
        if i > 0 and self.run_dev[i - 1] is not None:
            get_engine(device).sync()
            release_device_bam(params['sam_path'])
        if self.run_dev[i] is not None:
            ref_pool = ThreadPoolExecutor(max_workers=2)
            for k in self.keys[i:min(self.run_end[i], i + 3)]:
                refs.setdefault(k[0], ref_pool.submit(reference_for, params['fasta_path'], k[0], device, params))
            try:
                self.dbam = open_device_bam(params['sam_path'], device, contigs=list(self.run_dev[i]))
            except DeviceIngestUnavailable:
                pass
            ref_pool.shutdown(wait=False)
        if self.dbam is not None:
            db = self.dbam
            self.prepare = lambda chrom, grp: _prepare_device(db, params, chrom, grp, refs.pop(chrom, None))
        else:
            self.prepare = lambda chrom, grp: _prepare_wire(params, chrom, grp)
            if self.uploader is None:
                from .wire import WireUploader
                self.uploader = WireUploader(get_engine(device))
        self.nxt = i
        while self.nxt < self.run_end[i] and len(self.preps) < self.ahead:
            self._prepare_next(self.run_end[i])

    def pack_for(self, i):
        if i == 0 or self.run_end[i - 1] == i:
            self.enter_run(i)
        wp = self.preps.pop(0).result()
        self._prepare_next(self.run_end[i])
        if self.dbam is not None:
            if self.codes is None or self.codes.numel() < wp['codes_len']:
                self.codes = torch.empty(wp['codes_len'] + wp['codes_len'] // 8, dtype=torch.uint8, device=get_engine(self.device).device)
            return self.dbam.pack(wp, codes=self.codes), lambda: None
        tk = self.uploader.submit(wp)
        return self.uploader.expand(tk), lambda: self.uploader.release(tk)

    def close(self):
        self.pool.shutdown(wait=True)
        if self.dbam is not None:
            from .device_bam import release as release_device_bam
            from .device_fasta import release as release_device_fasta
            self.dbam = self.prepare = None
            release_device_bam(self.params['sam_path'])
            release_device_fasta(self.params['fasta_path'])


class _Records:

    def __init__(self, f, pool, counter_Q, gvcf_f=None):
        self.f, self.pool, self.counter_Q, self.scratch, self.pending, self.gvcf_f = f, pool, counter_Q, None, None, gvcf_f

    def emit(self, chrom, ploidy, r, grp, blocks=None):
# ... 168 lines not shown
```

Measured before the change: 62.45 million.

## Launch SNP featurization before scan completes using device-side site counts

Adds an early featurize path that is enqueued right after the scan begins. The kernels size the grid from capacity and read the actual neighbor and site counts from device totals, so they no longer wait for a host round trip to learn n_sites. This removes the host sync and launch gap between scan and featurize. In exchange it allocates outputs at candidate capacity and launches blocks that exit early, and it falls back to the old featurize path when the early result is not valid.

```diff
diff --git a/include/nanocaller_hip.h b/include/nanocaller_hip.h
--- a/include/nanocaller_hip.h
+++ b/include/nanocaller_hip.h
@@ -195,6 +195,14 @@
                      float *x_dev, int32_t *ref_code_out_dev, int32_t *fwd_dp_dev, int32_t *rev_dp_dev,
                      int32_t *site_depth_dev, uint8_t *valid_dev);
 
+int nc_snp_scan_caps(nc_ctx *ctx, int32_t *cap_nbr, int32_t *cap_cand);
+int nc_snp_featurize_early(nc_ctx *ctx, const nc_readpack *pack,
+                           const uint8_t *ref_code_dev, int32_t ref_pos0, int32_t ref_len,
+                           int32_t seq_mode, int32_t maxcov, int32_t min_nbr_sites,
+                           float *x_dev, int32_t *ref_code_out_dev, int32_t *fwd_dp_dev, int32_t *rev_dp_dev,
+                           int32_t *site_depth_dev, uint8_t *valid_dev, int32_t row_cap);
+int nc_snp_featurize_early_ok(nc_ctx *ctx, int32_t *ok);
+
 int nc_snp_set_mates(nc_ctx *ctx, int32_t n_mates, const int64_t *d_mate_key, const int32_t *d_mate_rec);
 
 int nc_indel_set_mates(nc_ctx *ctx, int32_t n_mates, const int64_t *d_mate_key, const int32_t *d_mate_rec);
diff --git a/nanocaller_amd/_lib.py b/nanocaller_amd/_lib.py
--- a/nanocaller_amd/_lib.py
+++ b/nanocaller_amd/_lib.py
@@ -39,6 +39,7 @@
     "nc_snp_phase_set_weights", "nc_snp_phase_weights_from_bam", "nc_snp_phase_weights",
     "nc_bam_retag_sizes", "nc_bam_retag", "nc_bgzf_deflate_device", "nc_bgzf_crc32_device", "nc_bgzf_assemble_device",
     "nc_fasta_decode",
+    "nc_snp_scan_caps", "nc_snp_featurize_early", "nc_snp_featurize_early_ok",
     "nc_bamidx_candidates", "nc_bamidx_chain", "nc_bamidx_collect", "nc_bamidx_verify", "nc_bamidx_serial", "nc_bamidx_fields",
     "nc_train_create", "nc_train_free", "nc_train_set_weights", "nc_train_get_weights", "nc_train_forward", "nc_train_loss_grad", "nc_train_adam",
     "nc_train_info", "nc_train_stage_ms",
@@ -181,6 +182,9 @@
         L.nc_snp_scan_fetch.argtypes = [vp, vp, vp, vp, vp, vp]
         L.nc_snp_scan_fetch_async.argtypes = [vp, vp, vp, vp, vp, vp, vp]
         L.nc_snp_featurize.argtypes = [vp, C.POINTER(ReadPackC), vp, i32, i32, i32, i32, i32, vp, vp, vp, vp, vp, vp]
+        L.nc_snp_featurize_early.argtypes = [vp, C.POINTER(ReadPackC), vp, i32, i32, i32, i32, i32, vp, vp, vp, vp, vp, vp, i32]
+        L.nc_snp_scan_caps.argtypes = [vp, C.POINTER(i32), C.POINTER(i32)]
+        L.nc_snp_featurize_early_ok.argtypes = [vp, C.POINTER(i32)]
         L.nc_snp_scale.argtypes = [vp, vp, vp, dbl, i32, vp, vp]
         L.nc_snp_chunk_depth_async.argtypes = [vp, vp, vp]
         L.nc_load_weights.argtypes = [vp, i32, vp, C.c_size_t]
diff --git a/nanocaller_amd/csrc/nc_common.h b/nanocaller_amd/csrc/nc_common.h
--- a/nanocaller_amd/csrc/nc_common.h
+++ b/nanocaller_amd/csrc/nc_common.h
@@ -121,6 +121,8 @@
     bool scan_begun = false;
     int scan_tile = 0, scan_n_tiles = 0, scan_n_chunks = 0, scan_cap_nbr = 0, scan_cap_cand = 0;
     hipEvent_t scan_tot_ev = nullptr;
+    bool early_sites = false, early_ok = false;
+    int32_t early_rows = 0;
     uint8_t *stage_h = nullptr;
     int stage_turn = 0;
 };
@@ -219,6 +221,10 @@
     }
 };
 
+constexpr int NBR_IDX_SHIFT = 10;
+inline int nc_nbr_index_len(const nc_readpack *pack) { return (int)(((int64_t)pack->n_tiles * pack->tile_size) >> NBR_IDX_SHIFT) + 2; }
+
+extern "C" __attribute__((visibility("hidden"))) int nc_scan_sites_early(nc_ctx *ctx);
 int nc_selftest_device(nc_ctx *ctx);
 void nc_pipe_destroy(nc_ctx *ctx);
 void nc_refconf_destroy(nc_ctx *ctx);
diff --git a/nanocaller_amd/csrc/nc_featurize.hip b/nanocaller_amd/csrc/nc_featurize.hip
--- a/nanocaller_amd/csrc/nc_featurize.hip
+++ b/nanocaller_amd/csrc/nc_featurize.hip
@@ -1,3 +1,4 @@
+#include <algorithm>
 #include <type_traits>
 
 #include "nc_common.h"
@@ -29,8 +30,6 @@
 }
 static_assert(buckets_contiguous(), "a bucket must begin where the one before it ends (the first at 0): k_featurize_pairs shares the buckets' edges");
 
-constexpr int NBR_IDX_SHIFT = 10;
-
 __device__ __forceinline__ int lower_bound_i32(const int32_t *a, int n, int64_t key, const int32_t *cidx, int32_t cidx_pos0, int n_cidx)
 {
     int lo = 0, hi = n;
@@ -56,12 +55,13 @@
     const uint8_t *ref_code;
     int32_t ref_pos0;
     const int32_t *nbr_pos;
-    int32_t n_nbr;
+    const int32_t *totals;
+    int32_t max_nbr, max_sites;
     const int32_t *cidx;
     int32_t cidx_pos0, n_cidx;
     const int32_t *site_pos, *site_chunk;
     const int32_t *chunk_start, *chunk_end;
-    int32_t n_sites, mode, maxcov, min_nbr_sites;
+    int32_t mode, maxcov, min_nbr_sites;
     float *x;
     int32_t *ref_out, *fwd, *rev, *depth;
     uint8_t *valid;
@@ -99,14 +99,17 @@
     __shared__ __attribute__((aligned(16))) float sm[I16 ? 1 : 4][I16 ? 4 : NC_SNP_TENSOR + 3];
     __shared__ int32_t nlist[4][64];
     const int lane = threadIdx.x & 63, wv = __builtin_amdgcn_readfirstlane(threadIdx.x >> 6);
-    const int nblk = (int)gridDim.x, q8 = nblk >> 3, r8 = nblk & 7, xcd = blockIdx.x & 7, within = blockIdx.x >> 3;
+    const int n_sites = min(a.totals[2], a.max_sites), n_nbr = min(a.totals[0], a.max_nbr);
+    const int nblk = (n_sites + 3) >> 2;
+    if ((int)blockIdx.x >= nblk) return;
+    const int q8 = nblk >> 3, r8 = nblk & 7, xcd = blockIdx.x & 7, within = blockIdx.x >> 3;
     const int blk = (xcd < r8 ? xcd * (q8 + 1) : r8 * (q8 + 1) + (xcd - r8) * q8) + within;
     const int s = blk * 4 + wv;
     float *X = sm[I16 ? 0 : wv];
     if constexpr (!I16)
         for (int i = lane; i < NC_SNP_TENSOR; i += 64) X[i] = 0.0f;
 
-    if (s < a.n_sites) {
+    if (s < n_sites) {
         const int32_t v = __builtin_amdgcn_readfirstlane(a.site_pos[s]);
         const int32_t ch = __builtin_amdgcn_readfirstlane(a.site_chunk[s]);
         const int64_t win_lo = max((int64_t)1, (int64_t)a.chunk_start[ch] - NC_FLANK);
@@ -124,8 +127,8 @@
             pmin = max(pmin, win_lo);
             pmax = min(pmax, win_hi);
             if (pmin <= pmax) {
-                const int lo = lower_bound_i32(a.nbr_pos, a.n_nbr, pmin, a.cidx, a.cidx_pos0, a.n_cidx);
-                const int hi = lower_bound_i32(a.nbr_pos, a.n_nbr, pmax + 1, a.cidx, a.cidx_pos0, a.n_cidx);
+                const int lo = lower_bound_i32(a.nbr_pos, n_nbr, pmin, a.cidx, a.cidx_pos0, a.n_cidx);
+                const int hi = lower_bound_i32(a.nbr_pos, n_nbr, pmax + 1, a.cidx, a.cidx_pos0, a.n_cidx);
                 const int m = hi - lo;
                 take = min(m, B.k);
                 const bool first = left ? (B.far != 0) : (B.far == 0);
@@ -294,7 +297,7 @@
     if constexpr (I16) return;
     __syncthreads();
     const int s0 = blk * 4;
-    const int nsite = min(4, a.n_sites - s0);
+    const int nsite = min(4, n_sites - s0);
     if (a.x_i16) {
         int16_t *d16 = reinterpret_cast<int16_t *>(a.x) + (int64_t)s0 * NC_SNP_TENSOR;
         const int total = nsite * NC_SNP_TENSOR;
@@ -338,10 +341,13 @@
     __shared__ uint32_t cntL[4][41 * 4 + 4];
     __shared__ uint32_t endL[4][2 * 41];
     const int lane = threadIdx.x & 63, wv = __builtin_amdgcn_readfirstlane(threadIdx.x >> 6);
-    const int nblk = (int)gridDim.x, q8 = nblk >> 3, r8 = nblk & 7, xcd = blockIdx.x & 7, within = blockIdx.x >> 3;
+    const int n_sites = min(a.totals[2], a.max_sites), n_nbr = min(a.totals[0], a.max_nbr);
+    const int nblk = (n_sites + 3) >> 2;
+    if ((int)blockIdx.x >= nblk) return;
+    const int q8 = nblk >> 3, r8 = nblk & 7, xcd = blockIdx.x & 7, within = blockIdx.x >> 3;
     const int blk = (xcd < r8 ? xcd * (q8 + 1) : r8 * (q8 + 1) + (xcd - r8) * q8) + within;
     const int s = blk * 4 + wv;
-    if (s >= a.n_sites) return;
+    if (s >= n_sites) return;
     const int32_t v = __builtin_amdgcn_readfirstlane(a.site_pos[s]);
     const int32_t ch = __builtin_amdgcn_readfirstlane(a.site_chunk[s]);
     const int64_t win_lo = max((int64_t)1, (int64_t)a.chunk_start[ch] - NC_FLANK);
@@ -364,7 +370,7 @@
         const int bi = left ? nb - 1 - lane : lane - nb - 2;
         const int64_t D = bi < 0 ? (int64_t)0 : min((int64_t)M.b[max(bi, 0)].dhi, (int64_t)M.W - 1);
         const int64_t key = min(max(left ? (int64_t)v - D : (int64_t)v + 1 + D, win_lo), win_hi + 1);
-        edge = lower_bound_i32(a.nbr_pos, a.n_nbr, key, a.cidx, a.cidx_pos0, a.n_cidx);
+        edge = lower_bound_i32(a.nbr_pos, n_nbr, key, a.cidx, a.cidx_pos0, a.n_cidx);
     }
     int take = 0, idx0 = 0;
     {
@@ -565,10 +571,12 @@
     }
 }
 
-__global__ void k_nbr_index(const int32_t *__restrict__ nbr_pos, int n_nbr, int32_t pos0, int n_cidx, int32_t *__restrict__ cidx)
+__global__ void k_nbr_index(const int32_t *__restrict__ nbr_pos, const int32_t *__restrict__ totals, int max_nbr, int32_t pos0, int n_cidx,
+                            int32_t *__restrict__ cidx)
 {
     const int b = blockIdx.x * blockDim.x + threadIdx.x;
     if (b >= n_cidx) return;
+    const int n_nbr = min(totals[0], max_nbr);
     const int64_t key = (int64_t)pos0 + ((int64_t)b << NBR_IDX_SHIFT);
     int lo = 0, hi = n_nbr;
     while (lo < hi) {
@@ -602,26 +610,15 @@
         scale[s] = mode == 0 ? train_cov / mean : train_cov / (double)site_n[s];
 }
 
-}
-
-extern "C" {
-
-int nc_snp_featurize(nc_ctx *ctx, const nc_readpack *pack, const uint8_t *ref_code_dev, int32_t ref_pos0, int32_t ref_len,
-                     int32_t seq_mode, int32_t maxcov, int32_t min_nbr_sites, float *x_dev, int32_t *ref_code_out_dev,
-                     int32_t *fwd_dp_dev, int32_t *rev_dp_dev, int32_t *site_depth_dev, uint8_t *valid_dev)
-{
-    if (!ctx) return NC_ERR_ARG;
-    if (!ctx->have_scan) return nc_fail(ctx, NC_ERR_STATE, "nc_snp_featurize: call nc_snp_scan first");
-    if (!pack || !ref_code_dev || seq_mode < 0 || seq_mode > 4)
-        return nc_fail(ctx, NC_ERR_ARG, "nc_snp_featurize: bad argument");
-    if (maxcov < 1 || maxcov > MAXCOV_CAP)
-        return nc_fail(ctx, NC_ERR_ARG, "nc_snp_featurize: maxcov %d outside [1,%d]", maxcov, MAXCOV_CAP);
-    if (ctx->n_sites == 0) return NC_OK;
+int featurize_launch(nc_ctx *ctx, const char *who, const nc_readpack *pack, const uint8_t *ref_code_dev, int32_t ref_pos0, int32_t ref_len,
+                     int32_t seq_mode, int32_t maxcov, int32_t min_nbr_sites, float *x_dev, int32_t *ref_code_out_dev, int32_t *fwd_dp_dev,
+                     int32_t *rev_dp_dev, int32_t *site_depth_dev, uint8_t *valid_dev, int32_t max_nbr, int32_t max_sites, int (*before)(nc_ctx *))
+{
     if (!x_dev || !ref_code_out_dev || !fwd_dp_dev || !rev_dp_dev || !site_depth_dev || !valid_dev)
-        return nc_fail(ctx, NC_ERR_ARG, "nc_snp_featurize: null output");
-    if (((uintptr_t)x_dev) & 15) return nc_fail(ctx, NC_ERR_ARG, "nc_snp_featurize: x_dev must be 16-byte aligned");
+        return nc_fail(ctx, NC_ERR_ARG, "%s: null output", who);
+    if (((uintptr_t)x_dev) & 15) return nc_fail(ctx, NC_ERR_ARG, "%s: x_dev must be 16-byte aligned", who);
     if (ref_pos0 != pack->tile_pos0 || (int64_t)ref_len < (int64_t)pack->n_tiles * pack->tile_size)
-        return nc_fail(ctx, NC_ERR_ARG, "nc_snp_featurize: ref_code must cover the pack's tile grid");
+        return nc_fail(ctx, NC_ERR_ARG, "%s: ref_code must cover the pack's tile grid", who);
     NC_HIP(ctx, hipSetDevice(ctx->device));
     FeatArgs a;
     a.codes = pack->codes;
@@ -632,8 +629,10 @@
     a.ref_code = ref_code_dev;
     a.ref_pos0 = ref_pos0;
     a.nbr_pos = (const int32_t *)ctx->nbr_pos.p;
-    a.n_nbr = ctx->n_nbr;
-    const int n_cidx = (int)(((int64_t)pack->n_tiles * pack->tile_size) >> NBR_IDX_SHIFT) + 2;
+    a.totals = (const int32_t *)ctx->totals.p;
+    a.max_nbr = max_nbr;
+    a.max_sites = max_sites;
+    const int n_cidx = nc_nbr_index_len(pack);
     NC_TRY(nc_ensure(ctx, ctx->nbr_idx, (size_t)n_cidx * 4));
     a.cidx = (const int32_t *)ctx->nbr_idx.p;
     a.cidx_pos0 = pack->tile_pos0;
@@ -642,7 +641,6 @@
     a.site_chunk = (const int32_t *)ctx->site_chunk.p;
     a.chunk_start = (const int32_t *)ctx->chunk_start.p;
     a.chunk_end = (const int32_t *)ctx->chunk_end.p;
-    a.n_sites = ctx->n_sites;
     a.mode = seq_mode;
     a.maxcov = maxcov;
     a.min_nbr_sites = min_nbr_sites;
@@ -659,11 +657,12 @@
     const char *fp = getenv("NC_FEAT_PAIRS");
     const bool pairs = maxcov < MAXCOV_SMALL && a.x_i16 && !(fp && atoi(fp) == 0);
     if (a.n_mates > 0 && !pairs)
-        return nc_fail(ctx, NC_ERR_UNSUPPORTED, "nc_snp_featurize: alignments that share read names (nc_snp_set_mates) need the int16 tensor format and maxcov < %d", MAXCOV_SMALL);
+        return nc_fail(ctx, NC_ERR_UNSUPPORTED, "%s: alignments that share read names (nc_snp_set_mates) need the int16 tensor format and maxcov < %d", who, MAXCOV_SMALL);
+    if (before) NC_TRY(before(ctx));
     NcTimer tm(ctx, 1);
-    hipLaunchKernelGGL(k_nbr_index, dim3((n_cidx + 255) / 256), dim3(256), 0, ctx->stream, a.nbr_pos, a.n_nbr, a.cidx_pos0, n_cidx,
+    hipLaunchKernelGGL(k_nbr_index, dim3((n_cidx + 255) / 256), dim3(256), 0, ctx->stream, a.nbr_pos, a.totals, a.max_nbr, a.cidx_pos0, n_cidx,
                        (int32_t *)ctx->nbr_idx.p);
-    const dim3 grid((ctx->n_sites + 3) / 4);
+    const dim3 grid((max_sites + 3) / 4);
     if (maxcov < MAXCOV_SMALL) {
         if (pairs && a.n_mates > 0) hipLaunchKernelGGL(k_featurize_pairs<true>, grid, dim3(256), 0, ctx->stream, a);
         else if (pairs) hipLaunchKernelGGL(k_featurize_pairs<false>, grid, dim3(256), 0, ctx->stream, a);
@@ -675,6 +674,45 @@
     }
     NC_HIP(ctx, hipGetLastError());
     tm.stop();
+    return NC_OK;
+}
+
+}
+
+extern "C" {
+
+int nc_snp_featurize(nc_ctx *ctx, const nc_readpack *pack, const uint8_t *ref_code_dev, int32_t ref_pos0, int32_t ref_len,
+                     int32_t seq_mode, int32_t maxcov, int32_t min_nbr_sites, float *x_dev, int32_t *ref_code_out_dev,
+                     int32_t *fwd_dp_dev, int32_t *rev_dp_dev, int32_t *site_depth_dev, uint8_t *valid_dev)
+{
+    if (!ctx) return NC_ERR_ARG;
+    if (!ctx->have_scan) return nc_fail(ctx, NC_ERR_STATE, "nc_snp_featurize: call nc_snp_scan first");
+    if (!pack || !ref_code_dev || seq_mode < 0 || seq_mode > 4)
+        return nc_fail(ctx, NC_ERR_ARG, "nc_snp_featurize: bad argument");
+    if (maxcov < 1 || maxcov > MAXCOV_CAP)
+        return nc_fail(ctx, NC_ERR_ARG, "nc_snp_featurize: maxcov %d outside [1,%d]", maxcov, MAXCOV_CAP);
+    if (ctx->n_sites == 0) return NC_OK;
+    return featurize_launch(ctx, "nc_snp_featurize", pack, ref_code_dev, ref_pos0, ref_len, seq_mode, maxcov, min_nbr_sites, x_dev, ref_code_out_dev,
+                            fwd_dp_dev, rev_dp_dev, site_depth_dev, valid_dev, ctx->n_nbr, ctx->n_sites, nullptr);
+}
+
+int nc_snp_featurize_early(nc_ctx *ctx, const nc_readpack *pack, const uint8_t *ref_code_dev, int32_t ref_pos0, int32_t ref_len,
+                           int32_t seq_mode, int32_t maxcov, int32_t min_nbr_sites, float *x_dev, int32_t *ref_code_out_dev,
+                           int32_t *fwd_dp_dev, int32_t *rev_dp_dev, int32_t *site_depth_dev, uint8_t *valid_dev, int32_t row_cap)
+{
+    if (!ctx) return NC_ERR_ARG;
+    if (!ctx->scan_begun) return nc_fail(ctx, NC_ERR_STATE, "nc_snp_featurize_early: no open nc_snp_scan_begin on this context");
+    if (ctx->early_rows) return nc_fail(ctx, NC_ERR_STATE, "nc_snp_featurize_early: called twice for one scan");
+    if (!pack || !ref_code_dev || seq_mode < 0 || seq_mode > 4 || row_cap < 1)
+        return nc_fail(ctx, NC_ERR_ARG, "nc_snp_featurize_early: bad argument");
+    if (maxcov < 1 || maxcov > MAXCOV_CAP)
+        return nc_fail(ctx, NC_ERR_ARG, "nc_snp_featurize_early: maxcov %d outside [1,%d]", maxcov, MAXCOV_CAP);
+    if (pack->n_tiles != ctx->scan_n_tiles || pack->tile_size != ctx->scan_tile)
+        return nc_fail(ctx, NC_ERR_ARG, "nc_snp_featurize_early: not the pack of the open scan");
+    const int32_t rows = std::min(row_cap, (int32_t)ctx->scan_cap_cand);
+    NC_TRY(featurize_launch(ctx, "nc_snp_featurize_early", pack, ref_code_dev, ref_pos0, ref_len, seq_mode, maxcov, min_nbr_sites, x_dev,
+                            ref_code_out_dev, fwd_dp_dev, rev_dp_dev, site_depth_dev, valid_dev, ctx->scan_cap_nbr, rows, nc_scan_sites_early));
+    ctx->early_rows = rows;
     return NC_OK;
 }
 
diff --git a/nanocaller_amd/csrc/nc_scan.hip b/nanocaller_amd/csrc/nc_scan.hip
--- a/nanocaller_amd/csrc/nc_scan.hip
+++ b/nanocaller_amd/csrc/nc_scan.hip
@@ -287,13 +287,13 @@
     if (threadIdx.x == 0) { off[n] = carry; totals[2] = carry; }
 }
 
-__global__ void k_sites(int n_sites, int n_chunks, const int32_t *__restrict__ chunk_off, const int32_t *__restrict__ chunk_lo,
-                        const int32_t *__restrict__ cand_pos, const int32_t *__restrict__ cand_n,
+__global__ void k_sites(const int32_t *__restrict__ totals, int max_sites, int n_chunks, const int32_t *__restrict__ chunk_off,
+                        const int32_t *__restrict__ chunk_lo, const int32_t *__restrict__ cand_pos, const int32_t *__restrict__ cand_n,
                         const int32_t *__restrict__ cand_alt, int32_t *__restrict__ site_pos,
                         int32_t *__restrict__ site_chunk, int32_t *__restrict__ site_n, int32_t *__restrict__ site_alt)
 {
     const int s = blockIdx.x * blockDim.x + threadIdx.x;
-    if (s >= n_sites) return;
+    if (s >= min(totals[2], max_sites)) return;
     int lo = 0, hi = n_chunks;
     while (lo < hi) {
         const int mid = (lo + hi) >> 1;
@@ -386,6 +386,31 @@
 }
 static int cap_of(const DevBuf &b) { return (int)std::min<size_t>(b.cap / 4, (size_t)INT32_MAX); }
 
+static int ensure_sites(nc_ctx *ctx)
+{
+    const size_t ns = (size_t)ctx->scan_cap_cand + 1;
+    NC_TRY(nc_ensure(ctx, ctx->site_pos, ns * 4));
+    NC_TRY(nc_ensure(ctx, ctx->site_chunk, ns * 4));
+    NC_TRY(nc_ensure(ctx, ctx->site_n, ns * 4));
+    NC_TRY(nc_ensure(ctx, ctx->site_alt, ns * 4));
+    return NC_OK;
+}
+
+static int launch_sites(nc_ctx *ctx, int max_sites)
+{
+    if (max_sites > 0) {
+        hipLaunchKernelGGL(k_sites, dim3((max_sites + 255) / 256), dim3(256), 0, ctx->stream, (const int32_t *)ctx->totals.p, max_sites,
+                           ctx->scan_n_chunks, (const int32_t *)ctx->chunk_off.p, (const int32_t *)ctx->chunk_lo.p,
+                           (const int32_t *)ctx->cand_pos.p, (const int32_t *)ctx->cand_n.p, (const int32_t *)ctx->cand_alt.p,
+                           (int32_t *)ctx->site_pos.p, (int32_t *)ctx->site_chunk.p, (int32_t *)ctx->site_n.p,
+                           (int32_t *)ctx->site_alt.p);
+        NC_HIP(ctx, hipGetLastError());
+    }
+    if (!ctx->scan_ev) NC_HIP(ctx, hipEventCreateWithFlags(&ctx->scan_ev, hipEventDisableTiming));
+    NC_HIP(ctx, hipEventRecord(ctx->scan_ev, ctx->stream));
+    return NC_OK;
+}
+
 int nc_snp_scan_begin(nc_ctx *ctx, const nc_readpack *pack, const uint8_t *ref_code_dev, int32_t ref_pos0, int32_t ref_len,
                       int32_t scan_lo, int32_t scan_hi, const nc_scan_params *params, int32_t n_chunks,
                       const int32_t *chunk_start_host, const int32_t *chunk_end_host)
@@ -404,6 +429,8 @@
     NC_HIP(ctx, hipSetDevice(ctx->device));
     ctx->have_scan = false;
     ctx->scan_begun = false;
+    ctx->early_sites = ctx->early_ok = false;
+    ctx->early_rows = 0;
     const int64_t npos = (int64_t)pack->n_tiles * tile;
     NC_TRY(nc_ensure(ctx, ctx->stage_nbr, npos * 4));
     NC_TRY(nc_ensure(ctx, ctx->stage_cpos, npos * 4));
@@ -474,6 +501,8 @@
         ctx->scan_cap_nbr = cap_of(ctx->nbr_pos);
         ctx->scan_cap_cand = std::min(cap_of(ctx->cand_pos), std::min(cap_of(ctx->cand_n), cap_of(ctx->cand_alt)));
     }
+    NC_TRY(ensure_sites(ctx));
+    NC_TRY(nc_ensure(ctx, ctx->nbr_idx, (size_t)nc_nbr_index_len(pack) * 4));
     NC_TRY(scan_compact(ctx, ctx->scan_cap_nbr, ctx->scan_cap_cand));
     ctx->scan_begun = true;
     return NC_OK;
@@ -487,41 +516,52 @@
     NC_HIP(ctx, hipSetDevice(ctx->device));
     volatile int32_t *tot = ctx->mbox;
     NC_HIP(ctx, hipEventSynchronize(ctx->scan_tot_ev));
-    if (!(tot[0] <= ctx->scan_cap_nbr && tot[1] <= ctx->scan_cap_cand)) {
+    const bool fit = tot[0] <= ctx->scan_cap_nbr && tot[1] <= ctx->scan_cap_cand;
+    if (!fit) {
         NC_TRY(nc_ensure(ctx, ctx->nbr_pos, (size_t)(tot[0] + 1) * 4));
         NC_TRY(nc_ensure(ctx, ctx->cand_pos, (size_t)(tot[1] + 1) * 4));
         NC_TRY(nc_ensure(ctx, ctx->cand_n, (size_t)(tot[1] + 1) * 4));
         NC_TRY(nc_ensure(ctx, ctx->cand_alt, (size_t)(tot[1] + 1) * 4));
         ctx->scan_cap_nbr = cap_of(ctx->nbr_pos);
         ctx->scan_cap_cand = std::min(cap_of(ctx->cand_pos), std::min(cap_of(ctx->cand_n), cap_of(ctx->cand_alt)));
+        NC_TRY(ensure_sites(ctx));
         NC_TRY(scan_compact(ctx, ctx->scan_cap_nbr, ctx->scan_cap_cand));
         NC_HIP(ctx, hipEventSynchronize(ctx->scan_tot_ev));
         if (!(tot[0] <= ctx->scan_cap_nbr && tot[1] <= ctx->scan_cap_cand)) return nc_fail(ctx, NC_ERR_STATE, "nc_snp_scan: outputs still too small after regrowth");
     }
-    const int32_t n_chunks = ctx->scan_n_chunks;
     ctx->n_nbr = tot[0];
     ctx->n_cand = tot[1];
     ctx->n_sites = tot[2];
-    ctx->n_chunks = n_chunks;
-    const size_t ns = (size_t)tot[2] + 1;
-    NC_TRY(nc_ensure(ctx, ctx->site_pos, ns * 4));
-    NC_TRY(nc_ensure(ctx, ctx->site_chunk, ns * 4));
-    NC_TRY(nc_ensure(ctx, ctx->site_n, ns * 4));
-    NC_TRY(nc_ensure(ctx, ctx->site_alt, ns * 4));
-    if (tot[2] > 0) {
-        hipLaunchKernelGGL(k_sites, dim3((tot[2] + 255) / 256), dim3(256), 0, ctx->stream, tot[2], n_chunks,
-                           (const int32_t *)ctx->chunk_off.p, (const int32_t *)ctx->chunk_lo.p,
-                           (const int32_t *)ctx->cand_pos.p, (const int32_t *)ctx->cand_n.p, (const int32_t *)ctx->cand_alt.p,
-                           (int32_t *)ctx->site_pos.p, (int32_t *)ctx->site_chunk.p, (int32_t *)ctx->site_n.p,
-                           (int32_t *)ctx->site_alt.p);
-        NC_HIP(ctx, hipGetLastError());
-    }
-    if (!ctx->scan_ev) NC_HIP(ctx, hipEventCreateWithFlags(&ctx->scan_ev, hipEventDisableTiming));
-    NC_HIP(ctx, hipEventRecord(ctx->scan_ev, ctx->stream));
+    ctx->n_chunks = ctx->scan_n_chunks;
+    if (!(fit && ctx->early_sites)) NC_TRY(launch_sites(ctx, tot[2]));
+    ctx->early_ok = fit && ctx->early_sites && ctx->early_rows > 0 && tot[2] <= ctx->early_rows;
     ctx->have_scan = true;
     if (n_nbr) *n_nbr = tot[0];
     if (n_cand) *n_cand = tot[1];
     if (n_sites) *n_sites = tot[2];
+    return NC_OK;
+}
+
+int nc_scan_sites_early(nc_ctx *ctx)
+{
+    NC_TRY(launch_sites(ctx, ctx->scan_cap_cand));
+    ctx->early_sites = true;
+    return NC_OK;
+}
+
+int nc_snp_scan_caps(nc_ctx *ctx, int32_t *cap_nbr, int32_t *cap_cand)
+{
+    if (!ctx) return NC_ERR_ARG;
+    if (cap_nbr) *cap_nbr = cap_of(ctx->nbr_pos);
+    if (cap_cand) *cap_cand = std::min(cap_of(ctx->cand_pos), std::min(cap_of(ctx->cand_n), cap_of(ctx->cand_alt)));
+    return NC_OK;
+}
+
+int nc_snp_featurize_early_ok(nc_ctx *ctx, int32_t *ok)
+{
+    if (!ctx) return NC_ERR_ARG;
+    if (!ok) return nc_fail(ctx, NC_ERR_ARG, "nc_snp_featurize_early_ok: null argument");
+    *ok = ctx->have_scan && ctx->early_ok ? 1 : 0;
     return NC_OK;
 }
 
diff --git a/nanocaller_amd/engine.py b/nanocaller_amd/engine.py
--- a/nanocaller_amd/engine.py
+++ b/nanocaller_amd/engine.py
@@ -215,7 +215,7 @@
         self._loaded[kind] = w.path
 
     def snp_scan(self, dp: DevicePack, chunks, *, mincov, min_allele_freq, threshold, haploid=False, async_fetch=False, sites=None,
-                 sites_only=False, nbr_sites=None, nbr_only=False, sample=None) -> SnpSites:
+                 sites_only=False, nbr_sites=None, nbr_only=False, sample=None, featurize=None) -> SnpSites:
         def on_device(s):
             if isinstance(s, torch.Tensor):
                 d = s.to(device=self.device, dtype=torch.int32).contiguous()
@@ -251,6 +251,15 @@
         pc = dp.c_struct()
         listed = d_sites is not None and d_sites.numel() > 0
         listed_nbr = d_nbr is not None and d_nbr.numel() > 0
+        early = None
+        if featurize is not None:
+            cap_nbr, cap_cand = C.c_int32(), C.c_int32()
+            self._check(self.L.nc_snp_scan_caps(self.ctx, C.byref(cap_nbr), C.byref(cap_cand)), "nc_snp_scan_caps")
+            if cap_nbr.value > 0 and cap_cand.value > 0:
+                fz = dict(featurize)
+                want16 = self.x_int16 if fz.get("int16") is None else bool(fz["int16"])
+                i16 = want16 or dp.mates is not None
+                early = self._feat_outputs(cap_cand.value, i16)
         try:
             if listed:
                 self._check(self.L.nc_snp_scan_set_sites(self.ctx, int(d_sites.numel()), _ptr(d_sites), 1 if sites_only else 0), "nc_snp_scan_set_sites")
@@ -260,6 +269,9 @@
                 self._check(self.L.nc_snp_scan_set_sampling(self.ctx, seed, _lib.npp(keep6)), "nc_snp_scan_set_sampling")
             self._check(self.L.nc_snp_scan_begin(self.ctx, C.byref(pc), _ptr(dp.ref_code), dp.tile_pos0, dp.ref_code.numel(), scan_lo,
                                                  scan_hi, C.byref(params), len(chunks), _lib.npp(cs), _lib.npp(ce)), "nc_snp_scan_begin")
+            if early is not None:
+                self._featurize_call(dp, early, i16, seq=fz["seq"], maxcov=fz["maxcov"],
+                                     min_nbr_sites=int(fz.get("min_nbr_sites", 1)) + (1 if nbr_only else 0), row_cap=cap_cand.value)
         finally:
             if listed:
                 self.L.nc_snp_scan_set_sites(self.ctx, 0, None, 0)
@@ -277,7 +289,19 @@
                         "nc_snp_scan_fetch_async")
         else:
             self._check(self.L.nc_snp_scan_fetch(self.ctx, None, ptr[0], ptr[1], ptr[2], ptr[3]), "nc_snp_scan_fetch")
-        return SnpSites(n_sites=N, n_nbr=n_nbr.value, pos=h[0, :N], chunk=h[1, :N], dp=h[2, :N], alt=h[3, :N], nbr_only=bool(nbr_only))
+        res = SnpSites(n_sites=N, n_nbr=n_nbr.value, pos=h[0, :N], chunk=h[1, :N], dp=h[2, :N], alt=h[3, :N], nbr_only=bool(nbr_only))
+        if featurize is not None:
+            ok = C.c_int32(0)
+            if early is not None:
+                self._check(self.L.nc_snp_featurize_early_ok(self.ctx, C.byref(ok)), "nc_snp_featurize_early_ok")
+            if ok.value:
+                for k, v in early.items():
+                    setattr(res, k, v[:N])
+                if not want16 and i16:
+                    res.x = res.x.to(torch.float32)
+            elif N > 0:
+                self.snp_featurize(dp, res, **featurize)
+        return res
 
     def fetch_nbr_sites(self, n_nbr) -> np.ndarray:
         out = np.empty(n_nbr, np.int32)
@@ -342,35 +366,46 @@
         self._check(self.L.nc_refconf_text(*args, _ptr(text), int(nbytes.value), None), "nc_refconf_text")
         return text[:int(nbytes.value)].cpu().numpy(), off.cpu().numpy()
 
-    def snp_featurize(self, dp: DevicePack, sites: SnpSites, *, seq, maxcov, min_nbr_sites=1, int16=None) -> SnpSites:
-        if sites.nbr_only:
-            min_nbr_sites = int(min_nbr_sites) + 1
-        N = sites.n_sites
-        dev = self.device
-        want16 = self.x_int16 if int16 is None else bool(int16)
-        i16 = want16 or dp.mates is not None
+    def _feat_outputs(self, rows, i16):
+        N = int(rows)
         xb = N * 1025 * (2 if i16 else 4)
         a16 = lambda v: (v + 15) & ~15
         o_ref = a16(xb); o_fwd = a16(o_ref + 4 * N); o_rev = a16(o_fwd + 16 * N); o_dep = a16(o_rev + 16 * N); o_val = a16(o_dep + 4 * N)
-        buf = torch.empty(o_val + N + 16, dtype=torch.uint8, device=dev)
-        sites.x = buf[:xb].view(torch.int16 if i16 else torch.float32).view(N, 5, 41, 5)
-        sites.ref_code = buf[o_ref:o_ref + 4 * N].view(torch.int32)
-        sites.fwd_dp = buf[o_fwd:o_fwd + 16 * N].view(torch.int32).view(N, 4)
-        sites.rev_dp = buf[o_rev:o_rev + 16 * N].view(torch.int32).view(N, 4)
-        sites.depth = buf[o_dep:o_dep + 4 * N].view(torch.int32)
-        sites.valid = buf[o_val:o_val + N]
+        buf = torch.empty(o_val + N + 16, dtype=torch.uint8, device=self.device)
+        return dict(x=buf[:xb].view(torch.int16 if i16 else torch.float32).view(N, 5, 41, 5),
+                    ref_code=buf[o_ref:o_ref + 4 * N].view(torch.int32),
+                    fwd_dp=buf[o_fwd:o_fwd + 16 * N].view(torch.int32).view(N, 4),
+                    rev_dp=buf[o_rev:o_rev + 16 * N].view(torch.int32).view(N, 4),
+                    depth=buf[o_dep:o_dep + 4 * N].view(torch.int32),
+                    valid=buf[o_val:o_val + N])
+
+    def _featurize_call(self, dp, out, i16, *, seq, maxcov, min_nbr_sites, row_cap=None):
         pc = dp.c_struct()
         if dp.mates is not None:
             self._check(self.L.nc_snp_set_mates(self.ctx, int(dp.mates[0].numel()), _ptr(dp.mates[0]), _ptr(dp.mates[1])), "nc_snp_set_mates")
         try:
             with self._snp_state(int16=i16):
-                self._check(self.L.nc_snp_featurize(self.ctx, C.byref(pc), _ptr(dp.ref_code), dp.tile_pos0, dp.ref_code.numel(),
-                                                    _lib.SEQ_MODES[seq], int(maxcov), int(min_nbr_sites), _ptr(sites.x),
-                                                    _ptr(sites.ref_code), _ptr(sites.fwd_dp), _ptr(sites.rev_dp), _ptr(sites.depth),
-                                                    _ptr(sites.valid)), "nc_snp_featurize")
+                args = (self.ctx, C.byref(pc), _ptr(dp.ref_code), dp.tile_pos0, dp.ref_code.numel(), _lib.SEQ_MODES[seq], int(maxcov),
+                        int(min_nbr_sites), _ptr(out["x"]), _ptr(out["ref_code"]), _ptr(out["fwd_dp"]), _ptr(out["rev_dp"]), _ptr(out["depth"]),
+                        _ptr(out["valid"]))
+                if row_cap is None:
+                    self._check(self.L.nc_snp_featurize(*args), "nc_snp_featurize")
+                else:
+                    self._check(self.L.nc_snp_featurize_early(*args, int(row_cap)), "nc_snp_featurize_early")
         finally:
             if dp.mates is not None:
                 self.L.nc_snp_set_mates(self.ctx, 0, None, None)
+
+    def snp_featurize(self, dp: DevicePack, sites: SnpSites, *, seq, maxcov, min_nbr_sites=1, int16=None) -> SnpSites:
+        if sites.nbr_only:
+            min_nbr_sites = int(min_nbr_sites) + 1
+        N = sites.n_sites
+        want16 = self.x_int16 if int16 is None else bool(int16)
+        i16 = want16 or dp.mates is not None
+        out = self._feat_outputs(N, i16)
+        for k, v in out.items():
+            setattr(sites, k, v)
+        self._featurize_call(dp, out, i16, seq=seq, maxcov=maxcov, min_nbr_sites=min_nbr_sites)
         if not want16 and i16:
             sites.x = sites.x.to(torch.float32)
         return sites
diff --git a/nanocaller_amd/snpCaller.py b/nanocaller_amd/snpCaller.py
--- a/nanocaller_amd/snpCaller.py
+++ b/nanocaller_amd/snpCaller.py
@@ -191,10 +191,13 @@
     listed, only = sites_for(params, chrom)
     nbr_listed, nbr_only = neighbor_sites_for(params, chrom)
     spans = [(c['start'], c['end']) for c in chunks]
+    exact = eng.exact_fp32
+    feat = dict(seq=params['seq'], maxcov=params['maxcov'], min_nbr_sites=params['min_nbr_sites'], int16=not exact)
+    handover = os.environ.get('NC_SCAN_HANDOVER', '1') != '0'
     sites = eng.snp_scan(dpk, spans, mincov=params['mincov'],
                          min_allele_freq=params['min_allele_freq'], threshold=params['threshold'],
                          haploid=(ploidy == 'haploid'), async_fetch=True, sites=listed, sites_only=only,
-                         nbr_sites=nbr_listed, nbr_only=nbr_only)
+                         nbr_sites=nbr_listed, nbr_only=nbr_only, featurize=feat if handover else None)
     res = dict(chrom=chrom, ploidy=ploidy, n=0, genotype_listed=count_listed(listed, spans, ())[0], genotype_emitted=0)
     from . import gvcf
     if gvcf.enabled(params):
@@ -202,8 +205,8 @@
     if sites.n_sites == 0:
         eng.wait_copies()
         return PendingCall(lambda: res) if defer else res
-    exact = eng.exact_fp32
-    eng.snp_featurize(dpk, sites, seq=params['seq'], maxcov=params['maxcov'], min_nbr_sites=params['min_nbr_sites'], int16=not exact)
+    if not handover:
+        eng.snp_featurize(dpk, sites, **feat)
     all_valid = bool(sites.valid.all().item()) if params['min_nbr_sites'] > 1 or sites.nbr_only else True
     per_site = bool(params.get('disable_coverage_normalization'))
     scale, chunk_depth = eng.snp_scale(sites, len(chunks), train_cov, per_site=per_site, async_fetch=True)
```

Result: no change. 62.42 million (median of 2 runs) (-0.1%).
